# bdsaglam/torch-scae

Measured on AMD Instinct MI355X. Metric: images/sec SCAE fwd+bwd, MNIST 40x40 bs=128, 1/2/4/8 MI355X, higher is better.
Workload: dtype f32

## Files before the change

include/scae_hip.h:

```cpp
#ifndef SCAE_HIP_H
#define SCAE_HIP_H

#include <stdint.h>

#ifdef __cplusplus
extern "C" {
#endif

#define SCAE_ABI_VERSION 3

#define SCAE_OK 0
#define SCAE_ERR_BAD_ARG (-1)
#define SCAE_ERR_UNSUPPORTED (-2)

#define SCAE_MAX_CHANNELS 4
#define SCAE_ATTN_MAX_SET 64
#define SCAE_RENDER_MAX_TEMPLATE_ELEMS 4096

int scae_abi_version(void);
const char *scae_error_string(int code);

void *scae_launch_list_begin(void *stream);
int scae_launch_list_end(void *list);
int scae_launch_list_size(const void *list);
// ... 623 lines not shown
  float *loss;
  const float *g_loss;
  int defer_combine;
  float *out12;
  const scae_train_log_desc *train_log;
} scae_loss_extras;
int scae_loss_tail_supported(int B, int O, int ncls);
int64_t scae_loss_tail_workspace_floats(int B, int O, int ncls);
int scae_loss_tail_fwd_f32(const float *lpp, const float *posterior,
                           const float *caps_presence, const float *cls_w,
                           const float *cls_b, const int64_t *label,
                           const scae_loss_extras *extras, float *out12, float *workspace,
                           int B, int O, int M, int ncls, int n_classes_cfg, int prior_type,
                           int post_type, int sparsity_on, const float *weights5,
                           float within_const, void *stream);
int scae_loss_tail_defer_preferred(int B, int O);
int scae_loss_tail_combine_f32(const float *lpp, const float *posterior,
                               const float *caps_presence, const float *cls_w,
                               const float *cls_b, const int64_t *label,
                               const scae_loss_extras *extras, float *out12, float *workspace,
                               int B, int O, int M, int ncls, int n_classes_cfg, int prior_type,
                               int post_type, int sparsity_on, const float *weights5,
                               float within_const, void *stream);
int scae_loss_tail_fwd_class_probs_f32(
    const float *lpp, const float *posterior, const float *caps_presence, const float *cls_w,
    const float *cls_b, const int64_t *label, const scae_loss_extras *extras, float *out12,
    float *workspace, int B, int O, int M, int ncls, int n_classes_cfg, int prior_type,
    int post_type, int sparsity_on, const float *weights5, float within_const,
    const float *cp_caps_presence, const float *cp_posterior, const float *cp_w,
    const float *cp_bias, float *prior_prob, float *post_prob, int cp_B, int cp_O, int cp_M,
    int cp_ncls, const scae_scaled_sum *extra_sums, int n_extra, void *stream);
int scae_loss_tail_fwd_class_probs_sink_f32(
    const float *lpp, const float *posterior, const float *caps_presence, const float *cls_w,
    const float *cls_b, const int64_t *label, const scae_loss_extras *extras, float *out12,
    float *workspace, int B, int O, int M, int ncls, int n_classes_cfg, int prior_type,
    int post_type, int sparsity_on, const float *weights5, float within_const,
    const float *cp_caps_presence, const float *cp_posterior, const float *cp_w,
    const float *cp_bias, float *prior_prob, float *post_prob, int cp_B, int cp_O, int cp_M,
    int cp_ncls, const scae_scaled_sum *extra_sums, int n_extra, scae_eval_sink *sink,
    void *stream);
int scae_loss_tail_bwd_f32(const float *lpp, const float *posterior,
                           const float *caps_presence, const float *cls_w,
                           const float *cls_b, const int64_t *label,
                           const scae_loss_extras *extras, const float *gout12,
                           const float *workspace, float *g_lpp, float *g_posterior,
                           float *g_caps_presence, float *g_cls_w,
                           float *g_cls_b, int B, int O, int M, int ncls, int n_classes_cfg,
                           int prior_type, int post_type, int sparsity_on,
                           const float *weights5, float within_const, void *stream);

#define SCAE_EVAL_ACC_DOUBLES 17
int scae_eval_tail_f32(const float *lpp, const float *posterior, const float *caps_presence,
                       const float *cls_w, const float *cls_b, const int64_t *label,
                       const scae_loss_extras *extras, float *out12, float *workspace, int B,
                       int O, int M, int ncls, int n_classes_cfg, int prior_type,
                       int post_type, int sparsity_on, const float *weights5,
                       float within_const, const float *prior_prob, const float *post_prob,
                       double *acc, float *batch3, void *stream);
int scae_eval_tail_sink_f32(const float *lpp, const float *posterior, const float *caps_presence,
                            const float *cls_w, const float *cls_b, const int64_t *label,
                            const scae_loss_extras *extras, float *out12, float *workspace,
                            int B, int O, int M, int ncls, int n_classes_cfg, int prior_type,
                            int post_type, int sparsity_on, const float *weights5,
                            float within_const, const float *prior_prob, const float *post_prob,
                            double *acc, float *batch3, scae_eval_sink *sink, void *stream);
int scae_eval_tail_records_f32(const float *lpp, const float *posterior,
                               const float *caps_presence, const float *cls_w,
                               const float *cls_b, const int64_t *label,
                               const scae_loss_extras *extras, float *out12, float *workspace,
                               int B, int O, int M, int ncls, int n_classes_cfg, int prior_type,
                               int post_type, int sparsity_on, const float *weights5,
                               float within_const, const float *prior_prob,
                               const float *post_prob, double *acc, float *batch3,
                               scae_eval_sink *sink, scae_eval_records *records, void *stream);
int scae_eval_records_f32(const float *prior_prob, const float *post_prob, const int64_t *label,
                          const float *lpp, const float *rec_sums, const float *rec_pixels,
                          int B, int ncls, int M, int n_rec, scae_eval_records *records,
                          void *stream);
int scae_eval_accumulate_f32(const float *loss, const float *out12, const float *prior_prob,
                             const float *post_prob, const int64_t *label, int B, int ncls,
                             double *acc, float *batch3, void *stream);
int scae_eval_features_f32(const float *caps_presence, const float *posterior, int B, int O,
                           int M, scae_eval_sink *sink, void *stream);
int scae_train_log_f32(const float *loss, const float *out12, const float *extra2,
                       const scae_train_log_desc *log, int B, void *stream);

typedef struct scae_decoder_desc {
  const float *templates;
  const float *templates_alpha;
  const float *pose;
  const float *presence;
  const float *bg_image;
  const float *bg_value;
  const float *bg_mixing_logit;
  const float *temperature_logit;
  const float *out_scale;
  int B, M, C, th, tw, H, W;
  int template_repeat;
} scae_decoder_desc;

int scae_template_render_fwd_f32(const scae_decoder_desc *d,
                                 float *transformed_templates,
                                 float *mixing_logits, void *stream);

int scae_render_gmm_logprob_fwd_f32(const scae_decoder_desc *d, const float *x,
                                    float *log_prob, float *lse_post,
                                    float *lse_prior, void *stream);

int scae_render_gmm_bwd_f32(const scae_decoder_desc *d, const float *x,
                            const float *lse_post, const float *lse_prior,
                            const float *g_logprob, const float *g_tt,
                            const float *g_ml, float *g_templates,
                            float *g_alpha_partial, float *g_pose,
                            float *g_presence, float *g_bg_image,
                            float *g_scalar_partial, void *stream);
int scae_render_gmm_logprob_tiles(const scae_decoder_desc *d);
int scae_render_gmm_logprob_sums_fwd_f32(const scae_decoder_desc *d, const float *x,
                                         float *tile_sums, float *lse_post, float *lse_prior,
                                         void *stream);
int scae_render_gmm_sums_bwd_f32(const scae_decoder_desc *d, const float *x,
                                 const float *lse_post, const float *lse_prior,
                                 const float *g_tile_sums, float *g_templates,
                                 float *g_alpha_partial, float *g_pose, float *g_presence,
                                 float *g_bg_image, float *g_scalar_partial, void *stream);
#define SCAE_K1_FWD_WAVE 0
#define SCAE_K1_FWD_CLASSIC 1
#define SCAE_K1_RENDER_WAVE 0
#define SCAE_K1_RENDER_CLASSIC 1
#define SCAE_K1_BWD_CELL 0
#define SCAE_K1_BWD_SCATTER 1
#define SCAE_K1_BWD_GATHER 2
int scae_render_gmm_forms(const scae_decoder_desc *d, int fused, const void *tt,
                          const void *ml, int out[12]);


int scae_set_encoder_fwd_logprob_f32(int nseg, const float *const *seg_ptr,
                                     const int *seg_width, const int *seg_row_stride,
                                     const int64_t *seg_batch_stride, const float *presence,
                                     const float *params, float *z, float *hsave, int B, int N,
                                     int D, int Din, int Dout, int L, int layer_norm,
                                     const scae_decoder_desc *d, const float *x,
                                     float *tile_sums, float *lse_post, float *lse_prior,
                                     void *stream);

int scae_set_encoder_fwd_logprob_bf16(int nseg, const float *const *seg_ptr,
                                      const int *seg_width, const int *seg_row_stride,
                                      const int64_t *seg_batch_stride, const float *presence,
                                      const float *params, float *z, float *hsave, int B, int N,
                                      int D, int Din, int Dout, int L, int layer_norm,
                                      const scae_decoder_desc *d, const float *x,
                                      float *tile_sums, float *lse_post, float *lse_prior,
                                      void *stream);

typedef struct scae_likelihood_bwd_desc {
  const float *vote, *scale, *vote_presence, *dummy_vote, *x, *presence, *posterior;
  const int64_t *winner_idx;
  const float *g_lpp, *g_winner, *g_winner_presence, *g_soft_winner, *g_soft_winner_presence,
      *g_posterior, *g_mixing_log_prob, *g_mixing_logit;
  float *gvote, *gscale, *gvote_presence, *gx, *gpresence, *gdummy_partial;
  int B, O, M;
} scae_likelihood_bwd_desc;
int scae_render_gmm_sums_bwd_likelihood_f32(
    const scae_decoder_desc *d, const float *x, const float *lse_post, const float *lse_prior,
    const float *g_tile_sums, float *g_templates, float *g_alpha_partial, float *g_pose,
    float *g_presence, float *g_bg_image, float *g_scalar_partial,
    const scae_likelihood_bwd_desc *k, void *stream);

int scae_gmm_log_prob_fwd_f32(const float *loc, const float *mixing_logits,
                              const float *sigma, const float *x,
                              float *log_prob, int B, int K, int C, int Cm,
                              int64_t P, void *stream);
int scae_gmm_log_prob_bwd_f32(const float *loc, const float *mixing_logits,
                              const float *sigma, const float *x,
                              const float *g_logprob, float *g_loc,
                              float *g_ml, float *g_sigma_partial, float *g_x,
                              int B, int K, int C, int Cm, int64_t P,
                              void *stream);
int scae_gmm_mean_f32(const float *loc, const float *mixing_logits, float *out,
                      int B, int K, int C, int Cm, int64_t P, void *stream);
int scae_gmm_mode_f32(const float *loc, const float *mixing_logits,
                      const float *sigma, float *out, int maximum, int B,
                      int K, int C, int Cm, int64_t P, void *stream);

int scae_render_gmm_mode_f32(const scae_decoder_desc *d, float *out, int what, int first,
                             int count, void *stream);

int scae_render_gmm_parts_f32(const scae_decoder_desc *d, const float *x, const int *part_group,
                              const float *palette, int P, int *part, float *conf, float *mass,
                              float *mass_partial, int *group, float *rgb_part,
                              float *rgb_group, int first, int count, void *stream);
int scae_render_gmm_parts_geometry(const scae_decoder_desc *d, int count, int *out);

int scae_image_sheet_f32(int nsrc, const float *const *src, const int *n, int C, int H, int W,
                         int nrow, int padding, float pad_value, float *sheet, void *stream);

#define SCAE_KMEANS_MAX_K 256
#define SCAE_KMEANS_MAX_F 256
#define SCAE_KMEANS_MAX_KF 16384
#define SCAE_KMEANS_STATE_INTS 4
int scae_kmeans_supported(int k, int F);
int scae_kmeans_groups(int64_t N, int R);
typedef struct scae_kmeans_desc {
  const float *x;
  int64_t N;
  int F, k, R;
  int G;
  int max_iter;
  float *centroids;
  int64_t *labels;
  float *part_sum;
  int *part_count;
  int *part_changed;
  double *part_inertia;
  int *state;
  double *inertia;
} scae_kmeans_desc;
int scae_kmeans_lloyd_f32(const scae_kmeans_desc *d, int n_iters, void *stream);
int scae_kmeans_pp_f32(const float *x, int64_t N, int F, int k, int R, uint32_t seed,
                       float *centroids, float *d2, int64_t *chosen, void *stream);
int scae_kmeans_assign_f32(const float *x, int64_t N, int F, int k, const float *centroids,
                           int64_t *labels, void *stream);
int scae_kmeans_contingency(const int64_t *cluster_ids, const int64_t *labels, int64_t N, int k,
                            int ncls, int *table, int *outside, void *stream);

#define SCAE_PROBE_MAX_F 256
#define SCAE_PROBE_MAX_C 256
#define SCAE_PROBE_MAX_CF 16384
#define SCAE_PROBE_MAX_R 16
#define SCAE_PROBE_STATE_INTS 4
int scae_probe_supported(int F, int C, int R);
int scae_probe_groups(int64_t N, int F);
int scae_probe_predict_blocks(int64_t N);
int scae_probe_moments_f64(const float *x, const int64_t *y, int64_t N, int F, int C,
                           double *part, double *moments, int *outside, void *stream);
typedef struct scae_probe_desc {
  const float *x;
  const int64_t *y;
  int64_t N;
  int F, C, R;
  int G;
  int max_iter;
  const float *mean;
  const float *scale;
  const double *l2;
  const double *step;
  const double *tol;
  float *W, *V;
  float *grad;
  double *t;
  float *part_grad;
  double *part_loss;
  double *history;
  int *state;
} scae_probe_desc;
int scae_probe_fit_f32(const scae_probe_desc *d, int n_iters, void *stream);
int scae_probe_predict_f32(const float *x, int64_t N, int F, int C, const float *weight,
                           const float *bias, const int64_t *y, int64_t *pred, float *log_prob,
                           double *part_ce, double *mean_ce, void *stream);

#define SCAE_TSNE_MAX_N 32768
#define SCAE_TSNE_MAX_F 256
#define SCAE_TSNE_HISTORY_COLS 3
#define SCAE_TSNE_BLOCK_DOUBLES 640
int scae_tsne_supported(int N, int F);
int scae_tsne_groups(int N);
int scae_tsne_affinities_f32(const float *x, int N, int F, float perplexity, float *P,
                             float *beta, double *part, double *plogp, void *stream);
typedef struct scae_tsne_desc {
  int N;
  int G;
  int n_iter;
  int exaggeration_iter;
  int check_every;
  float early_exaggeration;
  float learning_rate;
  const float *P;
  float *Y, *velocity, *gains;
  float *part;
  float *rows;
  double *block;
  const double *plogp;
  double *history;
} scae_tsne_desc;
int scae_tsne_run_f32(const scae_tsne_desc *d, int first_iter, int n, void *stream);

#define SCAE_KNN_MAX_K 64
#define SCAE_KNN_MAX_F 256
#define SCAE_KNN_MAX_KS 8
int scae_knn_supported(int64_t Nq, int64_t Nb, int F, int k);
int scae_knn_groups(int64_t Nq, int64_t Nb);
int scae_knn_f32(const float *q, int64_t Nq, const float *base, int64_t Nb, int F, int k,
                 int self_mode, uint64_t *part, float *d2, int64_t *idx, void *stream);
int scae_knn_vote_f32(const int64_t *idx, const float *d2, int64_t Nq, int k,
                      const int64_t *base_labels, int64_t Nb, const int *ks, int n_ks,
                      int weighted, int64_t *pred, void *stream);
int scae_knn_ranks_f32(const float *x, int64_t N, int F, const int64_t *idx, int k, int *rank,
                       int *part_count, int64_t *part, int64_t *penalty, void *stream);

#define SCAE_TSNE_MAX_NEIGHBORS 128
#define SCAE_TSNE_SPARSE_MAX_N 262144
#define SCAE_TSNE_SPARSE_BLOCK_DOUBLES 5120
int scae_knn_wide_f32(const float *x, int64_t N, int F, int k, uint64_t *part, float *d2,
                      int64_t *idx, void *stream);
int scae_tsne_sparse_supported(int N, int F, int K);
int scae_tsne_sparse_groups(int N);
int scae_tsne_knn_bandwidths_f32(const float *d2, int N, int K, float perplexity, float *cond,
                                 float *beta, void *stream);
typedef struct scae_tsne_sparse_desc {
  int N;
  int G;
  int n_iter;
  int exaggeration_iter;
  int check_every;
// ... 31 lines not shown
```

torch_scae_amd/_lib.py:

```python
import ctypes
import os
from ctypes import (POINTER, Structure, c_char_p, c_double, c_float, c_int,
                    c_int64, c_uint32, c_uint64, c_void_p)

_HERE = os.path.dirname(os.path.abspath(__file__))
LIB_PATH = os.environ.get("SCAE_HIP_LIB") or os.path.join(_HERE, "lib",
                                                        "libscae_hip.so")

P = c_void_p


class DecoderDesc(Structure):
    _fields_ = [("templates", P), ("templates_alpha", P), ("pose", P),
                ("presence", P), ("bg_image", P), ("bg_value", P),
                ("bg_mixing_logit", P), ("temperature_logit", P),
                ("out_scale", P),
                ("B", c_int), ("M", c_int), ("C", c_int), ("th", c_int),
                ("tw", c_int), ("H", c_int), ("W", c_int),
                ("template_repeat", c_int)]


class LikelihoodBwdDesc(Structure):
    _fields_ = [(n, P) for n in (
        "vote", "scale", "vote_presence", "dummy_vote", "x", "presence",
        "posterior", "winner_idx", "g_lpp", "g_winner", "g_winner_presence",
        "g_soft_winner", "g_soft_winner_presence", "g_posterior",
        "g_mixing_log_prob", "g_mixing_logit", "gvote", "gscale",
        "gvote_presence", "gx", "gpresence", "gdummy_partial")] + [
        ("B", c_int), ("O", c_int), ("M", c_int)]


class GemmDesc(Structure):
    _fields_ = [("A", P), ("B", P), ("C", P), ("bias", P), ("mask", P),
                ("asum", P), ("batch", c_int), ("M", c_int), ("N", c_int),
                ("K", c_int), ("a_kcontig", c_int), ("lda", c_int),
                ("a_batch", c_int64), ("b_kcontig", c_int), ("ldb", c_int),
                ("b_batch", c_int64), ("ldc", c_int), ("c_batch", c_int64),
                ("bias_ld", c_int), ("bias_batch", c_int64), ("ldmask", c_int),
                ("mask_batch", c_int64), ("asum_batch", c_int64),
                ("relu", c_int), ("asum_ld", c_int), ("c_nomask", P)]


class MlpChainLayer(Structure):
    _fields_ = [("w", P), ("w_gs", c_int64), ("ldw", c_int), ("K", c_int),
                ("N", c_int), ("bias", P), ("bias_gs", c_int64),
                ("bias_ld", c_int), ("gate", P), ("gate_gs", c_int64),
                ("gate_bs", c_int64), ("out", P), ("out_gs", c_int64),
                ("out_bs", c_int64), ("relu", c_int)]


class MlpChainDesc(Structure):
    _fields_ = [("layer", MlpChainLayer * 4), ("n_layers", c_int), ("in_", P),
                ("in_gs", c_int64), ("in_bs", c_int64), ("in_dim", c_int),
                ("B", c_int), ("G", c_int), ("row_tile", c_int),
                ("bf16", c_int)]


class VotesDesc(Structure):
    _fields_ = [(n, P) for n in ("all_param", "cpr_static", "bias_cvr",
                                 "bias_caps", "bias_vote", "bias_scale",
                                 "noise_caps", "noise_vote")] + \
        [("noise_scale", c_float), ("V", c_int), ("ld_param", c_int),
         ("similarity", c_int), ("learn_vote_scale", c_int),
         ("allow_deformations", c_int)] + \
        [(n, P) for n in ("vote", "scale", "vote_presence", "logit_caps",
                          "logit_vote", "reg_partial", "caps_presence",
                          "caps_arg", "gvote", "gscale", "gvote_presence",
                          "glogit_caps", "glogit_vote", "greg", "gcaps_presence",
                          "gall_param", "gcpr_in", "gall_param_gated")]


class SumSegment(Structure):
    _fields_ = [("dst", P), ("begin", c_int64), ("end", c_int64),
                ("period", c_int64)]


class SumJob(Structure):
    _fields_ = [("src", P), ("rows", c_int64), ("cols", c_int64),
                ("segments", POINTER(SumSegment)), ("n_segments", c_int)]


class ScaledSum(Structure):
    _fields_ = [("src", P), ("n", c_int64), ("scale", c_float), ("dst", P)]


class TrainLogDesc(Structure):
    _fields_ = [("rows", P), ("step", P), ("capacity", c_int), ("acc", P),
                ("prior_prob", P), ("post_prob", P), ("label", P), ("ncls", c_int),
                ("lr", P)]


class LossExtras(Structure):
    _fields_ = [("rec_sums", P), ("n_rec", c_int), ("reg", P),
                ("w_reg", c_float), ("g_rec_sums", P), ("g_reg", P),
                ("loss", P), ("g_loss", P), ("defer_combine", c_int),
                ("out12", P), ("train_log", POINTER(TrainLogDesc))]


class KMeansDesc(Structure):
    _fields_ = [("x", P), ("N", c_int64), ("F", c_int), ("k", c_int), ("R", c_int),
                ("G", c_int), ("max_iter", c_int), ("centroids", P), ("labels", P),
                ("part_sum", P), ("part_count", P), ("part_changed", P),
                ("part_inertia", P), ("state", P), ("inertia", P)]


class ProbeDesc(Structure):
    _fields_ = [("x", P), ("y", P), ("N", c_int64), ("F", c_int), ("C", c_int), ("R", c_int),
                ("G", c_int), ("max_iter", c_int), ("mean", P), ("scale", P), ("l2", P),
                ("step", P), ("tol", P), ("W", P), ("V", P), ("grad", P), ("t", P),
                ("part_grad", P), ("part_loss", P), ("history", P), ("state", P)]


class TsneDesc(Structure):
    _fields_ = [("N", c_int), ("G", c_int), ("n_iter", c_int), ("exaggeration_iter", c_int),
                ("check_every", c_int), ("early_exaggeration", c_float),
                ("learning_rate", c_float), ("P", P), ("Y", P), ("velocity", P), ("gains", P),
                ("part", P), ("rows", P), ("block", P), ("plogp", P), ("history", P)]


class TsneSparseDesc(Structure):
    _fields_ = [("N", c_int), ("G", c_int), ("n_iter", c_int), ("exaggeration_iter", c_int),
                ("check_every", c_int), ("early_exaggeration", c_float),
                ("learning_rate", c_float), ("indptr", P), ("cols", P), ("vals", P),
                ("nnz", c_int64), ("Y", P), ("velocity", P), ("gains", P), ("part", P),
                ("rows", P), ("block", P), ("plogp", P), ("history", P)]


class SeedFoldDesc(Structure):
    _fields_ = [(n, P) for n in (
        "seeds", "wq", "bq", "wk", "bk", "wv", "bv", "wo", "bo", "w2", "b2",
        "q", "wkf", "bkf", "wvf", "bvf", "wv2e", "wowv")] + \
        [("O", c_int), ("C", c_int), ("D", c_int)]


class FirstLayerDesc(Structure):
    _fields_ = [("img", P), ("w", P), ("bias", P), ("out", P)] + \
        [(n, c_int) for n in ("B", "Cin", "IH", "IW", "Cout", "stride",
                              "n_layers")] + \
        [("rw", P * 8), ("rwf", P * 8), ("rwd", P * 8),
         ("rCout", c_int * 8), ("rCin", c_int * 8),
         ("out_h", P), ("rwfh", P * 8), ("rwdh", P * 8)]


class BatchSourceDesc(Structure):
    _fields_ = [("images", P), ("labels", P), ("index", P), ("rows", c_int64),
                ("n", c_int64)] + \
        [(n, c_int) for n in ("image_u8", "label_u8", "C", "h", "w", "H", "W",
                              "shuffle", "translate")] + \
        [("seed", c_uint64), ("epoch", c_int64), ("position", c_int64),
         ("rank", c_int), ("world", c_int), ("wrap", c_int),
         ("affine", P), ("affine_rows", c_int64)]


class SeedFoldGrads(Structure):
    _fields_ = [(n, P) for n in (
        "g_q", "g_wkf", "g_bkf", "g_wvf", "g_bvf", "d_seeds", "d_wq", "d_bq",
        "d_wk", "d_bk", "d_wv", "d_bv", "d_wo", "d_bo", "d_w2", "d_b2",
        "gv2e", "t1")]


SIGNATURES = {
    "scae_abi_version": [],
    "scae_error_string": [c_int],
    "scae_uniform_f32": [P, c_int64, P, P],
    "scae_geometric_transform_fwd_f32": [P, P, c_int64, c_int, c_int, c_int, P],
    "scae_geometric_transform_bwd_f32": [P, P, P, c_int64, c_int, c_int, c_int,
                                         P],
    "scae_mat3_mul_fwd_f32": [P, P, P, c_int64, c_int, P],
    "scae_mat3_mul_bwd_f32": [P, P, P, P, P, c_int64, c_int, P],
    "scae_qkv_attention_fwd_f32": [P, P, P, P, P, P, c_int, c_int, c_int,
                                   c_int, c_int, c_float, P],
    "scae_qkv_attention_fwd_bf16": [P, P, P, P, P, P, c_int, c_int, c_int,
                                    c_int, c_int, c_float, P],
    "scae_qkv_attention_bwd_f32": [P, P, P, P, P, P, P, P, P, c_int, c_int,
                                   c_int, c_int, c_int, c_float, P],
    "scae_set_encoder_param_count": [c_int] * 5,
    "scae_set_encoder_grid": [c_int],
    "scae_set_encoder_supported": [c_int] * 6,
    "scae_set_encoder_fwd_f32": [c_int, P, P, P, P, P, P, P, P] + [c_int] * 7 + [P],
    "scae_set_encoder_bwd_f32": [c_int, P, P, P, P, P, P, P, P, P, P]
                                + [c_int] * 7 + [P],
    "scae_render_gmm_sums_bwd_likelihood_f32": [P] * 13,
    "scae_set_encoder_fwd_logprob_f32": [c_int, P, P, P, P, P, P, P, P] + [c_int] * 7
                                        + [P] * 6,
    "scae_set_encoder_fwd_logprob_bf16": [c_int, P, P, P, P, P, P, P, P] + [c_int] * 7
                                         + [P] * 6,
    "scae_set_encoder_bf16_supported": [c_int] * 6,
    "scae_set_encoder_fwd_bf16": [c_int, P, P, P, P, P, P, P, P] + [c_int] * 7 + [P],
    "scae_set_encoder_bwd_bf16": [c_int, P, P, P, P, P, P, P, P, P, P]
                                 + [c_int] * 7 + [P],
    "scae_seed_attention_splits": [c_int] * 2,
    "scae_seed_attention_grid": [c_int] * 2,
    "scae_seed_attention_supported": [c_int] * 4,
    "scae_seed_attention_fwd_f32": [P] * 9 + [c_int] * 5 + [P],
    "scae_seed_attention_bwd_f32": [P] * 10 + [c_int] * 5 + [P],
    "scae_seed_attention_mfma_supported": [c_int] * 4,
    "scae_seed_attention_mfma_rows": [c_int],
    "scae_seed_attention_mfma_fwd_f32": [P] * 7 + [c_int] * 4 + [P],
    "scae_seed_attention_mfma_bwd_f32": [P] * 8 + [c_int] * 4 + [P],
    "scae_seed_attention_mfma_fwd_bf16": [P] * 7 + [c_int] * 4 + [P],
    "scae_seed_attention_mfma_bwd_bf16": [P] * 8 + [c_int] * 4 + [P],
    "scae_seed_attention_mfma_bwd_gemm_f32": [P] * 8 + [c_int] * 4
    + [POINTER(GemmDesc), c_int, P],
    "scae_seed_attention_mfma_bwd_gemm_bf16": [P] * 8 + [c_int] * 4
    + [POINTER(GemmDesc), c_int, P],
    "scae_object_encoder_bwd_supported": [c_int] * 9,
    "scae_object_encoder_bwd_gemm_f32": [P] * 8 + [c_int] * 4
    + [POINTER(GemmDesc), c_int] + [c_int, P, P, P, P, P, P, P, P, P] + [c_int] * 7 + [P],
    "scae_object_encoder_bwd_gemm_bf16": [P] * 8 + [c_int] * 4
    + [POINTER(GemmDesc), c_int] + [c_int, P, P, P, P, P, P, P, P, P] + [c_int] * 7 + [P],
    "scae_seed_attention_mfma_reduce_f32": [P, c_int] + [P] * 7 + [c_int] * 2 + [P],
    "scae_seed_fold_supported": [c_int] * 3,
    "scae_seed_fold_fwd_f32": [POINTER(SeedFoldDesc), P],
    "scae_seed_fold_bwd_f32": [POINTER(SeedFoldDesc), POINTER(SeedFoldGrads), P],
    "scae_layer_norm_rows": [c_int64],
    "scae_layer_norm_fwd_f32": [P] * 6 + [c_int64, c_int, c_float, P],
    "scae_layer_norm_bwd_f32": [P] * 7 + [c_int64, c_int, P],
    "scae_gemm_f32": [P] * 6 + [c_int] * 6 + [c_int64, c_int, c_int, c_int64,
                                              c_int, c_int64, c_int, c_int64,
                                              c_int, c_int64, c_int64, c_int, c_int,
                                              P],
    "scae_gemm_bf16": [P] * 6 + [c_int] * 6 + [c_int64, c_int, c_int, c_int64,
                                              c_int, c_int64, c_int, c_int64,
                                              c_int, c_int64, c_int64, c_int, c_int,
                                              P],
    "scae_gemm_pair_f32": [POINTER(GemmDesc), POINTER(GemmDesc), P],
    "scae_launch_list_begin": [P],
    "scae_launch_list_end": [P],
    "scae_launch_list_size": [P],
    "scae_launch_list_run": [P, P],
    "scae_launch_list_lane": [P, c_int],
    "scae_launch_list_timeline": [P, P, P, POINTER(c_float), c_int],
    "scae_launch_list_free": [P],
    "scae_gemm_multi_f32": [POINTER(GemmDesc), c_int, P],
    "scae_gemm_multi_bf16": [POINTER(GemmDesc), c_int, P],
    "scae_mlp_chain_max_width": [],
    "scae_mlp_chain_fwd_f32": [POINTER(MlpChainDesc), P],
    "scae_mlp_chain_bwd_f32": [POINTER(MlpChainDesc), P],
    "scae_mlp_chain_votes_fwd_f32": [POINTER(MlpChainDesc), POINTER(VotesDesc), P],
    "scae_mlp_chain_votes_bwd_f32": [POINTER(MlpChainDesc), POINTER(VotesDesc), P],
    "scae_gemm_pair_bf16": [POINTER(GemmDesc), POINTER(GemmDesc), P],
    "scae_conv3x3_wf_floats": [c_int, c_int],
    "scae_conv3x3_relayout_f32": [P, P, P, c_int, c_int, P],
    "scae_conv3x3_bf16r_supported": [c_int] * 6,
    "scae_conv3x3_first_fwd_relayout_bf16": [P] * 4 + [c_int] * 7 + [P] * 8,
    "scae_cvt_bf16_batch": [c_int, P, P, P, P],
    "scae_conv3x3_fwd_bf16r": [P] * 7 + [c_int] * 6 + [P],
    "scae_conv3x3_dgrad_bf16r": [P] * 5 + [c_int] * 6 + [P],
    "scae_conv3x3_wgrad_bf16r_splits": [c_int] * 5,
# ... 291 lines not shown
```

torch_scae_amd/csrc/loss_tail.hip:

```cpp
#include "class_probs_dev.h"
#include "common.h"
#include "loss_tail_dev.h"

namespace {
using namespace scae_tail;
constexpr int MAXCLS = 32;

__device__ __forceinline__ float ent_term_grad(float p, float k) {
  const float q = p * k;
  return q < scae::kLogSafeEps ? 1e8f : -(logf(q) + 1.f);
}

__device__ __forceinline__ float within_term(const float *x, float r, int O, int type,
                                             float cw, int lane) {
  if (type == 0) return (r - cw) * (r - cw);
  const float k = type == 2 ? (float)O : 1.f;
  float w = 0.f;
  for (int o = lane; o < O; o += NTI) w += ent_term(x[o] / (r + 1e-8f), k);
  return scae::wave_sum(w);
}

__device__ __forceinline__ float cls_xe(const TailArgs &a, const float *x, int label, int lane,
                                        float &gl) {
  const bool on = lane < a.ncls;
  float z = -INFINITY;
  if (on) {
    const float *wr = a.cls_w + (size_t)lane * a.O;
    float z0 = a.cls_b[lane], z1 = 0.f, z2 = 0.f, z3 = 0.f;
    int o = 0;
    for (; o + 4 <= a.O; o += 4) {
      const float w0 = wr[o], w1 = wr[o + 1], w2 = wr[o + 2], w3 = wr[o + 3];
      z0 = fmaf(x[o], w0, z0), z1 = fmaf(x[o + 1], w1, z1);
      z2 = fmaf(x[o + 2], w2, z2), z3 = fmaf(x[o + 3], w3, z3);
    }
    for (; o < a.O; ++o) z0 = fmaf(x[o], wr[o], z0);
    z = (z0 + z1) + (z2 + z3);
  }
  const float mx = scae::wave_max(z);
  float p = on ? expf(z - mx) : 0.f;
  p /= scae::wave_sum(p);
  const float mx2 = scae::wave_max(on ? p : -INFINITY);
  const float q = on ? expf(p - mx2) : 0.f;
  const float sum2 = scae::wave_sum(q);
  const float plabel = scae::wave_sum(lane == label ? p : 0.f);
  const float dq = on ? q / sum2 - (lane == label ? 1.f : 0.f) : 0.f;
  const float dot = scae::wave_sum(p * dq);
  gl = p * (dq - dot);
  return mx2 + logf(sum2) - plabel;
}

__global__ __launch_bounds__(NTI) void tail_image_kernel(TailArgs a, Ws ws, scae_cp::Args cpa,
                                                        int n_cp) {
  extern __shared__ __attribute__((aligned(16))) float smem[];
  const int B = a.B, O = a.O, M = a.M, b = blockIdx.x, lane = threadIdx.x;
  if (b >= B) {
    __shared__ scae_cp::Lds s_cpl;
    scae_cp::body(cpa, s_cpl, b - B, lane);
    return;
  }
  float *s_cp = smem, *s_mass = smem + O, *s_raw = smem + 2 * O;
  float rc = 0.f, rm = 0.f;
  for (int o = lane; o < O; o += NTI) {
    const float xc = a.cp[(size_t)b * O + o];
    const float *pr = a.posterior + ((size_t)b * (O + 1) + o) * M;
    float t = 0.f;
    if ((M & 3) == 0) {
      const float4 *p4 = reinterpret_cast<const float4 *>(pr);
      for (int m = 0; m < M / 4; ++m) {
        const float4 v = p4[m];
        t += (v.x + v.y) + (v.z + v.w);
      }
    } else {
      for (int m = 0; m < M; ++m) t += pr[m];
    }
    s_cp[o] = xc;
    s_raw[o] = t;
    s_mass[o] = t / M;
    ws.mass[(size_t)b * O + o] = t;
    rc += xc;
    rm += t / M;
  }
  rc = scae::wave_sum(rc);
  rm = scae::wave_sum(rm);
  float lp = 0.f;
  for (int m = lane; m < M; m += NTI) lp += a.lpp[(size_t)b * M + m];
  lp = scae::wave_sum(lp);
  __syncthreads();
  float wc = 0.f, wm = 0.f;
  if (a.sparsity_on) {
    wc = within_term(s_cp, rc, O, a.prior_type, a.l2_within_const, lane);
    wm = within_term(s_mass, rm, O, a.post_type, a.l2_within_const_post, lane);
  }
  float xe_c = 0.f, xe_m = 0.f;
  if (a.label) {
    const int label = (int)a.label[b];
    float g0, g1;
    xe_c = cls_xe(a, s_cp, label, lane, g0);
    xe_m = cls_xe(a, s_raw, label, lane, g1);
    if (lane < a.ncls) {
      ws.gl[((size_t)b * 2 + 0) * a.ncls + lane] = g0;
      ws.gl[((size_t)b * 2 + 1) * a.ncls + lane] = g1;
    }
  }
  if (lane == 0) {
    float *p = ws.part + (size_t)b * 8;
    p[0] = lp, p[1] = wc, p[2] = wm, p[3] = xe_c, p[4] = xe_m, p[5] = rc, p[6] = rm, p[7] = 0.f;
  }
}

template <int NTC>
__global__ __launch_bounds__(NTC) void tail_combine_kernel(TailArgs a, scae_loss_extras x, Ws ws,
                                                          float *out) {
  extern __shared__ __attribute__((aligned(16))) float smem[];
  combine_body<NTC>(a, x, ws, out, smem);
}

template <int NTC>
__global__ __launch_bounds__(NTC) void tail_combine_log_kernel(TailArgs a, scae_loss_extras x,
                                                              Ws ws, float *out,
                                                              TrainLogArgs g) {
  extern __shared__ __attribute__((aligned(16))) float smem[];
  combine_body<NTC>(a, x, ws, out, smem);
  __syncthreads();
  train_log_epilogue<NTC>(g, out, out, nullptr);
}

__device__ __forceinline__ void sparsity_grad(const float *x, const float *col, float r, int B,
                                              int O, int type, float cw, float cb, float gw,
                                              float gb, float *g, int lane) {
  if (type == 0) {
    for (int o = lane; o < O; o += 64)
      g[o] = gw * 2.f * (r - cw) / B + gb * 2.f * (col[o] - cb) / O;
    return;
  }
  const float k = type == 2 ? (float)O : 1.f;
  float tot = 0.f;
  for (int o = 0; o < O; ++o) tot += col[o];
  const float tinv = 1.f / (tot + 1e-8f), rinv = 1.f / (r + 1e-8f);
  float dot_b = 0.f, dot_w = 0.f;
  for (int o = lane; o < O; o += 64) {
    dot_b += ent_term_grad(col[o] * tinv, k) * col[o] * tinv;
    dot_w += ent_term_grad(x[o] * rinv, k) * x[o] * rinv;
  }
  dot_b = scae::wave_sum(dot_b);
  dot_w = scae::wave_sum(dot_w);
  for (int o = lane; o < O; o += 64) {
    const float dw = (ent_term_grad(x[o] * rinv, k) - dot_w) * rinv / B;
    const float db = -(ent_term_grad(col[o] * tinv, k) - dot_b) * tinv;
    g[o] = gw * dw + gb * db;
  }
}

template <int NT>
__device__ __forceinline__ void tail_bwd_body(const TailArgs &a, const scae_loss_extras &x,
                                              const Ws &ws, const float *gout ,
                                              float *g_lpp, float *g_post, float *g_cp,
                                              float *g_w, float *g_b, float *smem) {
  const int B = a.B, O = a.O, M = a.M, tid = threadIdx.x;
  float go[12];
#pragma unroll
  for (int i = 0; i < 12; ++i) go[i] = gout ? gout[i] : 0.f;
  if (x.g_loss) go[0] += x.g_loss[0];
  const float g0 = go[0];
  if ((int)blockIdx.x >= B) {
    if (!(a.label && g_w)) return;
    const float g_x1 = (g0 + go[6]) / B, g_x2 = (g0 + go[7]) / B;
    const int nout = a.ncls * O + a.ncls;
    const int out = ((int)blockIdx.x - B) * (NT / 4) + (tid >> 2), part = tid & 3;
    float t = 0.f;
    if (out < a.ncls * O) {
      const int cc = out / O, o = out - cc * O;
      float t0 = 0.f, t1 = 0.f, t2 = 0.f, t3 = 0.f;
      int b = part;
      for (; b + 12 < B; b += 16) {
#define SCAE_TERM(bb)                                                                  \
  (ws.gl[((size_t)(bb) * 2) * a.ncls + cc] * g_x1 * a.cp[(size_t)(bb) * O + o] +      \
   ws.gl[((size_t)(bb) * 2 + 1) * a.ncls + cc] * g_x2 * ws.mass[(size_t)(bb) * O + o])
        const float u0 = SCAE_TERM(b), u1 = SCAE_TERM(b + 4), u2 = SCAE_TERM(b + 8),
                    u3 = SCAE_TERM(b + 12);
        t0 += u0, t1 += u1, t2 += u2, t3 += u3;
      }
      for (; b < B; b += 4) t0 += SCAE_TERM(b);
#undef SCAE_TERM
      t = (t0 + t1) + (t2 + t3);
    } else if (out < nout) {
      const int cc = out - a.ncls * O;
#pragma unroll 4
      for (int b = part; b < B; b += 4)
        t += ws.gl[((size_t)b * 2) * a.ncls + cc] * g_x1 +
             ws.gl[((size_t)b * 2 + 1) * a.ncls + cc] * g_x2;
    }
    t += scae::xor1_f(t);
    t += scae::xor2_f(t);
    if (part == 0 && out < nout) {
      if (out < a.ncls * O)
        g_w[out] = t;
      else
        g_b[out - a.ncls * O] = t;
    }
    return;
  }
  const int b = blockIdx.x;
  const float g_lp = (-a.w_ll * g0 + go[1] - go[10]) / B;
  for (int m = tid; m < M; m += NT) g_lpp[(size_t)b * M + m] = g_lp;
  if (x.g_rec_sums) {
    const float gr = (-g0 + go[8] - go[9]) / B;
    const int per = (x.n_rec + B - 1) / B, i1 = min(x.n_rec, (b + 1) * per);
    for (int i = b * per + tid; i < i1; i += NT) x.g_rec_sums[i] = gr;
  }
  if (x.g_reg && b == 0 && tid == 0) x.g_reg[0] = x.w_reg * g0 + go[11];
  float *s_cp = smem, *s_mass = s_cp + O, *col = s_mass + O, *gc = col + 2 * O, *gm = gc + O;
  for (int o = tid; o < O; o += NT) {
    s_cp[o] = a.cp[(size_t)b * O + o];
    s_mass[o] = ws.mass[(size_t)b * O + o] / M;
    if (!x.defer_combine) {
      col[o] = ws.col[o];
      col[O + o] = ws.col[O + o];
    }
    gc[o] = gm[o] = 0.f;
  }
  if (x.defer_combine) column_sums<NT>(a, ws, col, tid, false);
  __syncthreads();
  if (a.sparsity_on && tid < 64) {
    const float *p = ws.part + (size_t)b * 8;
    sparsity_grad(s_cp, col, p[5], B, O, a.prior_type, a.l2_within_const, a.l2_between_const,
                  a.w_pw * g0 + go[2], a.w_pb * g0 + go[3], gc, tid);
    sparsity_grad(s_mass, col + O, p[6], B, O, a.post_type, a.l2_within_const_post,
                  a.l2_between_const_post, a.w_qw * g0 + go[4], a.w_qb * g0 + go[5], gm, tid);
  }
  __syncthreads();
  for (int o = tid; o < O; o += NT) g_cp[(size_t)b * O + o] = gc[o];
  float *gp = g_post + (size_t)b * (O + 1) * M;
  if ((M & 3) == 0) {
    const int M4 = M / 4;
    for (int e = tid; e < (O + 1) * M4; e += NT) {
      const int o = e / M4;
      const float v = o < O ? gm[o] / M : 0.f;
      reinterpret_cast<float4 *>(gp)[e] = make_float4(v, v, v, v);
    }
  } else {
    for (int e = tid; e < (O + 1) * M; e += NT) {
      const int o = e / M;
      gp[e] = o < O ? gm[o] / M : 0.f;
    }
  }
}

template <int NT>
__global__ __launch_bounds__(NT) void tail_bwd_kernel(TailArgs a, scae_loss_extras x, Ws ws,
                                                      const float *gout , float *g_lpp,
                                                      float *g_post, float *g_cp, float *g_w,
                                                      float *g_b) {
  extern __shared__ __attribute__((aligned(16))) float smem[];
  if (x.defer_combine && blockIdx.x + 1 == gridDim.x) {
    combine_body<NT>(a, x, ws, x.out12, smem);
    return;
  }
  tail_bwd_body<NT>(a, x, ws, gout, g_lpp, g_post, g_cp, g_w, g_b, smem);
}

template <int NT>
__global__ __launch_bounds__(NT) void tail_bwd_log_kernel(TailArgs a, scae_loss_extras x, Ws ws,
                                                          const float *gout ,
                                                          float *g_lpp, float *g_post,
                                                          float *g_cp, float *g_w, float *g_b,
                                                          TrainLogArgs g) {
  extern __shared__ __attribute__((aligned(16))) float smem[];
  if (blockIdx.x + 1 == gridDim.x) {
    combine_body<NT>(a, x, ws, x.out12, smem);
    __syncthreads();
    train_log_epilogue<NT>(g, x.out12, x.out12, nullptr);
    return;
  }
  tail_bwd_body<NT>(a, x, ws, gout, g_lpp, g_post, g_cp, g_w, g_b, smem);
}
}

extern "C" int scae_loss_tail_supported(int B, int O, int ncls) {
  return (B > 0 && O > 0 && O <= 4096 && ncls <= MAXCLS) ? 1 : 0;
}

extern "C" int64_t scae_loss_tail_workspace_floats(int B, int O, int ncls) {
  if (B <= 0 || O <= 0 || ncls < 0) return 0;
  return (int64_t)ws_floats(B, O, ncls);
}

int scae_tail::fill_train_log(TrainLogArgs &g, const scae_train_log_desc &d, int B) {
  if (!d.rows || !d.step || d.capacity <= 0 || B <= 0 || d.ncls < 0) return SCAE_ERR_BAD_ARG;
  if (d.label && (d.ncls <= 0 || !d.prior_prob || !d.post_prob)) return SCAE_ERR_BAD_ARG;
  g = TrainLogArgs{d.rows, d.step, d.acc, d.prior_prob, d.post_prob, d.label, d.lr,
                   d.capacity, B, d.ncls};
  return SCAE_OK;
}

static int launch_combine(const TailArgs &a, const scae_loss_extras &x, const Ws &ws,
                          float *out12, hipStream_t st) {
  const bool small = scae_loss_tail_defer_preferred(a.B, a.O);
  if (x.train_log) {
    TrainLogArgs g;
    const int rc = fill_train_log(g, *x.train_log, a.B);
    if (rc) return rc;
    if (small)
      scae::launch(tail_combine_log_kernel<NT_SMALL>, dim3(1), dim3(NT_SMALL), combine_lds(a.O),
                   st, a, x, ws, out12, g);
    else
      scae::launch(tail_combine_log_kernel<NTC_LARGE>, dim3(1), dim3(NTC_LARGE),
                   combine_lds(a.O), st, a, x, ws, out12, g);
    return SCAE_OK;
  }
  if (small)
    scae::launch(tail_combine_kernel<NT_SMALL>, dim3(1), dim3(NT_SMALL), combine_lds(a.O), st,
                       a, x, ws, out12);
  else
    scae::launch(tail_combine_kernel<NTC_LARGE>, dim3(1), dim3(NTC_LARGE), combine_lds(a.O),
                       st, a, x, ws, out12);
  return SCAE_OK;
}

int scae_tail::fill_tail(TailArgs &a, const float *lpp, const float *posterior, const float *cp,
                          const float *cls_w, const float *cls_b, const int64_t *label, int B,
                          int O, int M, int ncls, int n_classes_cfg, int prior_type,
                          int post_type, int sparsity_on, const float *weights ,
                          float within_const) {
  if (!lpp || !posterior || !cp || !weights || B <= 0 || O <= 0 || M <= 0)
    return SCAE_ERR_BAD_ARG;
  if (label && (!cls_w || !cls_b || ncls <= 0)) return SCAE_ERR_BAD_ARG;
  if (prior_type < 0 || prior_type > 2 || post_type < 0 || post_type > 2) return SCAE_ERR_BAD_ARG;
  if (!scae_loss_tail_supported(B, O, ncls)) return SCAE_ERR_UNSUPPORTED;
  a = TailArgs{lpp, posterior, cp, cls_w, cls_b, label, B, O, M, ncls, prior_type, post_type,
               sparsity_on, weights[0], weights[1], weights[2], weights[3], weights[4],
               0.f, 0.f, 0.f, 0.f};
  const float nc = n_classes_cfg > 0 ? (float)n_classes_cfg : 1.f;
  a.l2_within_const = within_const == within_const ? within_const : (float)O / nc;
  a.l2_between_const = (float)B / nc;
  a.l2_within_const_post = (float)O / nc;
  a.l2_between_const_post = (float)B / nc;
  return SCAE_OK;
}

static int tail_fwd(const float *lpp, const float *posterior, const float *caps_presence,
                    const float *cls_w, const float *cls_b, const int64_t *label,
                    const scae_loss_extras *extras, float *out12, float *workspace, int B, int O,
                    int M, int ncls, int n_classes_cfg, int prior_type, int post_type,
                    int sparsity_on, const float *weights5, float within_const,
                    const scae_cp::Args *cpa, void *stream) {
  TailArgs a;
  int rc = fill_tail(a, lpp, posterior, caps_presence, cls_w, cls_b, label, B, O, M, ncls,
                     n_classes_cfg, prior_type, post_type, sparsity_on, weights5, within_const);
  if (rc) return rc;
  SCAE_REQUIRE(out12 && workspace);
  scae_loss_extras x{};
  if (extras) x = *extras;
  if (x.rec_sums && x.n_rec <= 0) return SCAE_ERR_BAD_ARG;
  const Ws ws = carve_ws(workspace, B, O, ncls);
  hipStream_t st = (hipStream_t)stream;
  const int n_cp = cpa ? cpa->B + cpa->extra.n : 0;
  scae::launch(tail_image_kernel, dim3(B + n_cp), dim3(NTI), 3 * O * sizeof(float), st, a,
                     ws, cpa ? *cpa : scae_cp::Args{}, n_cp);
  if (!x.defer_combine) {
    rc = launch_combine(a, x, ws, out12, st);
    if (rc) return rc;
  }
  return scae_launch_status();
}

extern "C" int scae_loss_tail_defer_preferred(int B, int O) {
  return B > 0 && O > 0 && (long)B * B * 2 * O * (long)sizeof(float) <= (8l << 20);
}

extern "C" int scae_loss_tail_combine_f32(const float *lpp, const float *posterior,
                                          const float *caps_presence, const float *cls_w,
                                          const float *cls_b, const int64_t *label,
                                          const scae_loss_extras *extras, float *out12,
                                          float *workspace, int B, int O, int M, int ncls,
                                          int n_classes_cfg, int prior_type, int post_type,
                                          int sparsity_on, const float *weights5,
                                          float within_const, void *stream) {
  TailArgs a;
  int rc = fill_tail(a, lpp, posterior, caps_presence, cls_w, cls_b, label, B, O, M, ncls,
                     n_classes_cfg, prior_type, post_type, sparsity_on, weights5, within_const);
  if (rc) return rc;
  SCAE_REQUIRE(out12 && workspace);
  scae_loss_extras x{};
  if (extras) x = *extras;
  if (x.rec_sums && x.n_rec <= 0) return SCAE_ERR_BAD_ARG;
  rc = launch_combine(a, x, carve_ws(workspace, B, O, ncls), out12, (hipStream_t)stream);
  if (rc) return rc;
  return scae_launch_status();
}

extern "C" int scae_loss_tail_fwd_f32(const float *lpp, const float *posterior,
                                      const float *caps_presence, const float *cls_w,
                                      const float *cls_b, const int64_t *label,
                                      const scae_loss_extras *extras, float *out12,
                                      float *workspace, int B, int O, int M, int ncls,
                                      int n_classes_cfg, int prior_type, int post_type,
                                      int sparsity_on, const float *weights5,
                                      float within_const, void *stream) {
  return tail_fwd(lpp, posterior, caps_presence, cls_w, cls_b, label, extras, out12, workspace,
                  B, O, M, ncls, n_classes_cfg, prior_type, post_type, sparsity_on, weights5,
                  within_const, nullptr, stream);
}

extern "C" int scae_loss_tail_fwd_class_probs_sink_f32(
    const float *lpp, const float *posterior, const float *caps_presence, const float *cls_w,
    const float *cls_b, const int64_t *label, const scae_loss_extras *extras, float *out12,
    float *workspace, int B, int O, int M, int ncls, int n_classes_cfg, int prior_type,
    int post_type, int sparsity_on, const float *weights5, float within_const,
    const float *cp_caps_presence, const float *cp_posterior, const float *cp_w,
    const float *cp_bias, float *prior_prob, float *post_prob, int cp_B, int cp_O, int cp_M,
    int cp_ncls, const scae_scaled_sum *extra_sums, int n_extra, scae_eval_sink *sink,
    void *stream) {
  scae_cp::Args cpa;
  int rc = scae_cp::fill(cpa, cp_caps_presence, cp_posterior, cp_w, cp_bias, prior_prob,
                         post_prob, cp_B, cp_O, cp_M, cp_ncls, extra_sums, n_extra);
  if (rc) return rc;
  cpa.sink = sink;
  return tail_fwd(lpp, posterior, caps_presence, cls_w, cls_b, label, extras, out12, workspace,
                  B, O, M, ncls, n_classes_cfg, prior_type, post_type, sparsity_on, weights5,
                  within_const, &cpa, stream);
}

extern "C" int scae_loss_tail_fwd_class_probs_f32(
    const float *lpp, const float *posterior, const float *caps_presence, const float *cls_w,
    const float *cls_b, const int64_t *label, const scae_loss_extras *extras, float *out12,
    float *workspace, int B, int O, int M, int ncls, int n_classes_cfg, int prior_type,
    int post_type, int sparsity_on, const float *weights5, float within_const,
    const float *cp_caps_presence, const float *cp_posterior, const float *cp_w,
    const float *cp_bias, float *prior_prob, float *post_prob, int cp_B, int cp_O, int cp_M,
    int cp_ncls, const scae_scaled_sum *extra_sums, int n_extra, void *stream) {
  return scae_loss_tail_fwd_class_probs_sink_f32(
      lpp, posterior, caps_presence, cls_w, cls_b, label, extras, out12, workspace, B, O, M,
      ncls, n_classes_cfg, prior_type, post_type, sparsity_on, weights5, within_const,
      cp_caps_presence, cp_posterior, cp_w, cp_bias, prior_prob, post_prob, cp_B, cp_O, cp_M,
      cp_ncls, extra_sums, n_extra, nullptr, stream);
}

extern "C" int scae_loss_tail_bwd_f32(const float *lpp, const float *posterior,
                                      const float *caps_presence, const float *cls_w,
                                      const float *cls_b, const int64_t *label,
                                      const scae_loss_extras *extras, const float *gout12,
                                      const float *workspace, float *g_lpp, float *g_posterior,
                                      float *g_caps_presence, float *g_cls_w, float *g_cls_b,
                                      int B, int O, int M, int ncls, int n_classes_cfg,
                                      int prior_type, int post_type, int sparsity_on,
                                      const float *weights5, float within_const, void *stream) {
  TailArgs a;
  int rc = fill_tail(a, lpp, posterior, caps_presence, cls_w, cls_b, label, B, O, M, ncls,
                     n_classes_cfg, prior_type, post_type, sparsity_on, weights5, within_const);
  if (rc) return rc;
  SCAE_REQUIRE(g_lpp && g_posterior && g_caps_presence && workspace);
  if (!gout12 && !(extras && extras->g_loss)) return SCAE_ERR_BAD_ARG;
  scae_loss_extras x{};
  if (extras) x = *extras;
  if (x.rec_sums && (x.n_rec <= 0 || !x.g_rec_sums)) return SCAE_ERR_BAD_ARG;
  if (x.reg && !x.g_reg) return SCAE_ERR_BAD_ARG;
  if (label) SCAE_REQUIRE(g_cls_w && g_cls_b);
  const Ws ws = carve_ws(const_cast<float *>(workspace), B, O, ncls);
  if (x.defer_combine) SCAE_REQUIRE(x.out12);
  const size_t lds = 6 * O * sizeof(float) > combine_lds(O) ? 6 * O * sizeof(float) : combine_lds(O);
  if (x.defer_combine && x.train_log) {
    TrainLogArgs g;
    rc = fill_train_log(g, *x.train_log, B);
    if (rc) return rc;
    const int cls_blocks = label ? (ncls * O + ncls + NT_SMALL / 4 - 1) / (NT_SMALL / 4) : 0;
    scae::launch(tail_bwd_log_kernel<NT_SMALL>, dim3(B + cls_blocks + 1), dim3(NT_SMALL), lds,
                 (hipStream_t)stream, a, x, ws, gout12, g_lpp, g_posterior, g_caps_presence,
                 g_cls_w, g_cls_b, g);
    return scae_launch_status();
  }
#define SCAE_TAIL_BWD(NTH)                                                                       \
  do {                                                                                           \
    const int cls_blocks = label ? (ncls * O + ncls + NTH / 4 - 1) / (NTH / 4) : 0;              \
    scae::launch(tail_bwd_kernel<NTH>, dim3(B + cls_blocks + (x.defer_combine ? 1 : 0)),   \
                       dim3(NTH), lds, (hipStream_t)stream, a, x, ws, gout12, g_lpp, g_posterior, \
                       g_caps_presence, g_cls_w, g_cls_b);                                       \
  } while (0)
  if (x.defer_combine || scae_loss_tail_defer_preferred(B, O))
    SCAE_TAIL_BWD(NT_SMALL);
  else
    SCAE_TAIL_BWD(NTB_LARGE);
#undef SCAE_TAIL_BWD
  return scae_launch_status();
}
```

torch_scae_amd/csrc/loss_tail_dev.h:

```cpp
#pragma once
#include "common.h"

namespace scae_tail {
constexpr int NTI = 64;
constexpr int NT_SMALL = 512, NTC_LARGE = 1024, NTB_LARGE = 256;

struct TailArgs {
  const float *lpp;
  const float *posterior;
  const float *cp;
  const float *cls_w;
  const float *cls_b;
  const int64_t *label;
  int B, O, M, ncls;
  int prior_type, post_type;
  int sparsity_on;
  float w_ll, w_pw, w_pb, w_qw, w_qb;
  float l2_within_const, l2_between_const, l2_within_const_post, l2_between_const_post;
};

struct Ws {
  float *part, *mass, *gl, *col;
};
__host__ __device__ inline Ws carve_ws(float *w, int B, int O, int ncls) {
  Ws s;
  s.part = w;
  s.mass = s.part + (size_t)B * 8;
  s.gl = s.mass + (size_t)B * O;
  s.col = s.gl + (size_t)B * 2 * (ncls > 0 ? ncls : 1);
  return s;
}
inline size_t ws_floats(int B, int O, int ncls) {
  return (size_t)B * 8 + (size_t)B * O + (size_t)B * 2 * (ncls > 0 ? ncls : 1) + 2 * (size_t)O;
}

__device__ __forceinline__ float ent_term(float p, float k) {
  return -p * scae::log_safe(p * k);
}
__device__ __forceinline__ float between_term(const float *col, int O, int type, float cb,
                                              int lane) {
  float t = 0.f;
  if (type == 0) {
    for (int o = lane; o < O; o += 64) t += (col[o] - cb) * (col[o] - cb);
    return scae::wave_sum(t) / O;
  }
  const float k = type == 2 ? (float)O : 1.f;
  float tot = 0.f;
  for (int o = 0; o < O; ++o) tot += col[o];
  for (int o = lane; o < O; o += 64) t += ent_term(col[o] / (tot + 1e-8f), k);
  return -scae::wave_sum(t);
}

template <int NTC>
__device__ __forceinline__ void column_sums(const TailArgs &a, const Ws &ws, float *col, int tid,
                                            bool publish) {
  const int B = a.B, O = a.O;
  for (int e = tid; e < ((2 * O * 16 + NTC - 1) / NTC) * NTC; e += NTC) {
    const int c = e >> 4, l = e & 15, which = c / O, o = c - which * O;
    float t = 0.f;
    if (c < 2 * O) {
      auto at = [&](int b) {
        return which == 0 ? a.cp[(size_t)b * O + o] : ws.mass[(size_t)b * O + o] / a.M;
      };
      float t0 = 0.f, t1 = 0.f, t2 = 0.f, t3 = 0.f;
      int b = l;
      for (; b + 48 < B; b += 64) {
        const float u0 = at(b), u1 = at(b + 16), u2 = at(b + 32), u3 = at(b + 48);
        t0 += u0, t1 += u1, t2 += u2, t3 += u3;
      }
      for (; b < B; b += 16) t0 += at(b);
      t = (t0 + t1) + (t2 + t3);
    }
    t = scae::row_sum16(t);
    if (c < 2 * O && l == 0) {
      col[c] = t;
      if (publish) ws.col[c] = t;
    }
  }
}

template <int NTC>
__device__ __forceinline__ void combine_body(const TailArgs &a, const scae_loss_extras &x,
                                             const Ws &ws, float *out, float *smem) {
  const int B = a.B, O = a.O, tid = threadIdx.x;
  float *col = smem, *red = smem + 2 * O;
  float v[6] = {0.f, 0.f, 0.f, 0.f, 0.f, 0.f};
  for (int b = tid; b < B; b += NTC) {
    const float4 p = *reinterpret_cast<const float4 *>(ws.part + (size_t)b * 8);
    v[0] += p.x, v[1] += p.y, v[2] += p.z, v[3] += p.w;
    v[4] += ws.part[(size_t)b * 8 + 4];
  }
  if (x.rec_sums)
    for (int i = tid; i < x.n_rec; i += NTC) v[5] += x.rec_sums[i];
  column_sums<NTC>(a, ws, col, tid, true);
  scae::block_sum<6, NTC>(v, red);
  if (tid >= 64) return;
  float pb = 0.f, qb = 0.f;
  if (a.sparsity_on) {
    pb = between_term(col, O, a.prior_type, a.l2_between_const, tid);
    qb = between_term(col + O, O, a.post_type, a.l2_between_const_post, tid);
  }
  if (tid != 0) return;
  const float log_prob = v[0] / B, pw = v[1] / B, qw = v[2] / B, xe1 = v[3] / B, xe2 = v[4] / B;
  const float rec = x.rec_sums ? v[5] / B : 0.f, reg = x.reg ? x.reg[0] : 0.f;
  out[1] = log_prob, out[2] = pw, out[3] = pb, out[4] = qw, out[5] = qb;
  out[6] = xe1, out[7] = xe2, out[8] = rec, out[9] = -rec, out[10] = -log_prob, out[11] = reg;
  const float loss = -a.w_ll * log_prob + a.w_pw * pw + a.w_pb * pb + a.w_qw * qw +
                     a.w_qb * qb + xe1 + xe2 - rec + x.w_reg * reg;
  out[0] = loss;
  if (x.loss) x.loss[0] = loss;
}


__device__ __forceinline__ int row_argmax(const float *p, int n) {
  float v = 0.f;
  int best = 0;
  for (int c0 = 0; c0 < n; c0 += 16) {
    float x[16];
#pragma unroll
    for (int j = 0; j < 16; ++j) x[j] = c0 + j < n ? p[c0 + j] : 0.f;
#pragma unroll
    for (int j = 0; j < 16; ++j) {
      const int c = c0 + j;
      if (c >= n) break;
      if (x[j] != x[j]) return c;
      if (c == 0 || x[j] > v) v = x[j], best = c;
    }
  }
  return best;
}

template <int NT>
__device__ __forceinline__ void accuracy_counts(const float *prior_prob, const float *post_prob,
                                                const int64_t *label, int B, int ncls,
                                                float &n_prior, float &n_post) {
  __shared__ float red[2][NT / 64];
  float cp = 0.f, cq = 0.f;
  if (label && ncls > 0) {
    for (int b = threadIdx.x; b < B; b += NT) {
      const int64_t l = label[b];
      cp += row_argmax(prior_prob + (size_t)b * ncls, ncls) == l ? 1.f : 0.f;
      cq += row_argmax(post_prob + (size_t)b * ncls, ncls) == l ? 1.f : 0.f;
    }
  }
  cp = scae::wave_sum(cp);
  cq = scae::wave_sum(cq);
  const int w = threadIdx.x / 64;
  if ((threadIdx.x & 63) == 0) red[0][w] = cp, red[1][w] = cq;
  __syncthreads();
  n_prior = n_post = 0.f;
  if (threadIdx.x == 0)
    for (int i = 0; i < NT / 64; ++i) n_prior += red[0][i], n_post += red[1][i];
}

__device__ __forceinline__ void batch_accuracies(bool labelled, int B, float n_prior,
                                                 float n_post, float acc3[3]) {
  float pa = 0.f, qa = 0.f;
  if (labelled) pa = n_prior / (float)B, qa = n_post / (float)B;
  acc3[0] = qa > pa ? qa : pa, acc3[1] = pa, acc3[2] = qa;
}

__device__ __forceinline__ void accumulate_batch(double *A, float loss, const float *out12,
                                                 const float acc3[3]) {
  A[0] += 1.0;
  A[1] += (double)loss;
  A[2] += (double)acc3[0];
  A[3] += (double)acc3[1];
  A[4] += (double)acc3[2];
  if (out12)
    for (int i = 0; i < 12; ++i) A[5 + i] += (double)out12[i];
}

struct TrainLogArgs {
  float *rows;
  int64_t *step;
  double *acc;
  const float *prior_prob, *post_prob;
  const int64_t *label;
  const float *lr;
  int capacity, B, ncls;
};

template <int NT>
__device__ __forceinline__ void train_log_epilogue(const TrainLogArgs &g, const float *loss,
                                                   const float *out12, const float *extra) {
  float n_prior, n_post;
  accuracy_counts<NT>(g.prior_prob, g.post_prob, g.label, g.B, g.ncls, n_prior, n_post);
  if (threadIdx.x >= 64) return;
  const int lane = threadIdx.x;
  n_prior = __shfl(n_prior, 0), n_post = __shfl(n_post, 0);
  float acc3[3];
  batch_accuracies(g.label && g.ncls > 0, g.B, n_prior, n_post, acc3);
  const int64_t s = g.step[0];
  const float l = loss[0];
  const float o = out12 && lane >= 4 && lane < 16 ? out12[lane - 4] : 0.f;
  const float lr = g.lr ? g.lr[0] : __builtin_nanf("");
  const float e = extra && lane >= 17 && lane < 19 ? extra[lane - 17] : 0.f;
  const double a = g.acc && lane < SCAE_EVAL_ACC_DOUBLES ? g.acc[lane] : 0.0;
  const float v = lane == 0 ? l : lane == 1 ? acc3[0] : lane == 2 ? acc3[1]
                : lane == 3 ? acc3[2] : lane < 16 ? o : lane == 16 ? lr : e;
  float *r = g.rows + (size_t)((uint64_t)s % (uint64_t)g.capacity) * SCAE_TRAIN_LOG_ROW;
  if (lane < SCAE_TRAIN_LOG_ROW) r[lane] = v;
  const float u = __shfl(v, lane > 0 ? lane - 1 : 0);
  if (g.acc && lane < SCAE_EVAL_ACC_DOUBLES && (lane < 5 || out12))
    g.acc[lane] = a + (lane == 0 ? 1.0 : (double)u);
  if (lane == 0) g.step[0] = s + 1;
}

inline size_t combine_lds(int O) { return (2 * O + 6 * (NTC_LARGE / 64)) * sizeof(float); }

int fill_tail(TailArgs &a, const float *lpp, const float *posterior, const float *cp,
              const float *cls_w, const float *cls_b, const int64_t *label, int B, int O, int M,
              int ncls, int n_classes_cfg, int prior_type, int post_type, int sparsity_on,
              const float *weights , float within_const);
int fill_train_log(TrainLogArgs &g, const scae_train_log_desc &d, int B);
}
```

torch_scae_amd/csrc/render_bwd_likelihood.hip:

```cpp
#include "common.h"
#include "capsule_likelihood_dev.h"
#include "render_gmm_wave_dev.h"

namespace {
struct LkBwd {
  scae_lk::LkArgs a;
  const int64_t *winner_idx;
  const float *g_lpp, *g_winner, *g_winner_presence, *g_soft_winner, *g_soft_winner_presence,
      *g_posterior, *g_mlp, *g_mlogit;
  float *gvote, *gscale, *gvp, *gx, *gpresence, *gdummy;
};

template <int C>
__global__ __launch_bounds__(256, 5) void bwd_cell_likelihood_kernel(
    scae_decoder_desc d, const float *__restrict__ x, const float *__restrict__ lse_post,
    const float *__restrict__ lse_prior, const float *__restrict__ g_tile, int lp_tiles,
    int lp_ppb, float *__restrict__ g_templates, float *__restrict__ g_alpha_partial,
    float *__restrict__ g_pose, float *__restrict__ g_presence, float *__restrict__ g_bg_image,
    float *__restrict__ g_scalar_partial, int chunk_rows, int max_items, int item_budget,
    LkBwd lk, int n_lk) {
  extern __shared__ __attribute__((aligned(16))) float smem[];
  if ((int)blockIdx.x < n_lk) {
    scae_lk::likelihood_bwd_body<false, 256>(
        lk.a, lk.winner_idx, lk.g_lpp, lk.g_winner, lk.g_winner_presence, lk.g_soft_winner,
        lk.g_soft_winner_presence, lk.g_posterior, lk.g_mlp, lk.g_mlogit, lk.gvote, lk.gscale,
        lk.gvp, lk.gx, lk.gpresence, lk.gdummy, smem, blockIdx.x, n_lk);
    return;
  }
  const int id = (int)blockIdx.x - n_lk, K = d.M + 1, b = id / K, k = id - b * K;
  scae_k1::bwd_cell_body<C, 256>(d, x, lse_post, lse_prior, nullptr, g_tile, lp_tiles, lp_ppb,
                                 g_templates, g_alpha_partial, g_pose, g_presence, g_bg_image,
                                 g_scalar_partial, chunk_rows, max_items, item_budget, smem, k, b);
}

template <int C>
int launch(const scae_decoder_desc *d, const scae_k1::CellGeom &g, const scae_k1::LpTiling &lt,
           const float *x, const float *lse_post, const float *lse_prior, const float *g_tile,
           float *g_templates, float *g_alpha_partial, float *g_pose, float *g_presence,
           float *g_bg_image, float *g_scalar_partial, const LkBwd &lk, hipStream_t st) {
  const size_t lds_k = scae_lk::lk_lds(lk.a.O, lk.a.M, true);
  const size_t lds = g.lds > lds_k ? g.lds : lds_k;
  if (lds > 48 * 1024) {
    hipError_t e =
        hipFuncSetAttribute(reinterpret_cast<const void *>(bwd_cell_likelihood_kernel<C>),
                            hipFuncAttributeMaxDynamicSharedMemorySize, (int)lds);
    if (e != hipSuccess) return (int)e;
  }
  const int n_lk = lk.a.B < 1024 ? lk.a.B : 1024;
  scae::launch((bwd_cell_likelihood_kernel<C>), dim3(n_lk + (d->M + 1) * d->B), dim3(256),
                     lds, st, *d, x, lse_post, lse_prior, g_tile, lt.tiles, lt.ppb, g_templates,
                     g_alpha_partial, g_pose, g_presence, g_bg_image, g_scalar_partial,
                     g.chunk_rows, g.max_items, g.item_budget, lk, n_lk);
  return scae_launch_status();
}
}

extern "C" int scae_render_gmm_sums_bwd_likelihood_f32(
    const scae_decoder_desc *d, const float *x, const float *lse_post, const float *lse_prior,
    const float *g_tile_sums, float *g_templates, float *g_alpha_partial, float *g_pose,
    float *g_presence, float *g_bg_image, float *g_scalar_partial,
    const scae_likelihood_bwd_desc *k, void *stream) {
  SCAE_REQUIRE(d && k);
  const char *e = getenv("SCAE_FUSE_K1_K4_BWD");
  const scae_k1::CellGeom g = scae_k1::cell_geom(d);
  const bool fits = !(e && *e == '0') && g.lds && (d->C == 1 || d->C == 3) && k->O <= 64 &&
                    scae_lk::lk_lds(k->O, k->M, true) <= g.lds && k->B > 0 && k->O > 0 &&
                    k->M > 0 && d->template_repeat <= 1;
  if (!fits) {
    int rc = scae_render_gmm_sums_bwd_f32(d, x, lse_post, lse_prior, g_tile_sums, g_templates,
                                          g_alpha_partial, g_pose, g_presence, g_bg_image,
                                          g_scalar_partial, stream);
    if (rc) return rc;
    return scae_capsule_likelihood_bwd_f32(
        k->vote, k->scale, k->vote_presence, k->dummy_vote, k->x, k->presence, k->posterior,
        k->winner_idx, k->g_lpp, k->g_winner, k->g_winner_presence, k->g_soft_winner,
        k->g_soft_winner_presence, k->g_posterior, k->g_mixing_log_prob, k->g_mixing_logit,
        k->gvote, k->gscale, k->gvote_presence, k->gx, k->gpresence, k->gdummy_partial, k->B,
        k->O, k->M, stream);
  }
  SCAE_REQUIRE(x && lse_post && lse_prior && g_tile_sums && g_templates && g_alpha_partial &&
               g_pose && g_scalar_partial);
  SCAE_REQUIRE(k->vote && k->scale && k->vote_presence && k->dummy_vote && k->x &&
               k->posterior && k->winner_idx && k->gvote && k->gscale && k->gvote_presence &&
               k->gx && k->gdummy_partial);
  const scae_k1::LpTiling lt = scae_k1::lp_tiling(d);
  LkBwd lk{{k->vote, k->scale, k->vote_presence, k->dummy_vote, k->x, k->presence, k->B, k->O,
            k->M},
           k->winner_idx,
           k->g_lpp,
           k->g_winner,
           k->g_winner_presence,
           k->g_soft_winner,
           k->g_soft_winner_presence,
           k->g_posterior,
           k->g_mixing_log_prob,
           k->g_mixing_logit,
           k->gvote,
           k->gscale,
           k->gvote_presence,
           k->gx,
           k->gpresence,
           k->gdummy_partial};
  hipStream_t st = (hipStream_t)stream;
  return d->C == 1 ? launch<1>(d, g, lt, x, lse_post, lse_prior, g_tile_sums, g_templates,
                               g_alpha_partial, g_pose, g_presence, g_bg_image, g_scalar_partial,
                               lk, st)
                   : launch<3>(d, g, lt, x, lse_post, lse_prior, g_tile_sums, g_templates,
                               g_alpha_partial, g_pose, g_presence, g_bg_image, g_scalar_partial,
                               lk, st);
}
```

torch_scae_amd/csrc/render_gmm_wave_dev.h:

```cpp
#pragma once
#include "common.h"
#include "render_gmm_dev.h"

namespace scae_k1 {
namespace {
constexpr float kLog2e = 1.44269504088896340736f, kLn2 = 0.69314718055994530942f;
constexpr int KC = 8;
constexpr float kMasked = -3.0e38f;

constexpr int kLogprobPadLow = 1;
template <int C> struct TexelOf { static constexpr int TX = C == 1 ? 2 : (C <= 3 ? 4 : 8); };

__device__ __forceinline__ float ex2(float v) { return __builtin_amdgcn_exp2f(v); }
__device__ __forceinline__ float lg2(float v) { return __builtin_amdgcn_logf(v); }

__host__ __device__ inline int plane_w(int tw, int PL) { return tw + PL + 2; }
__host__ __device__ inline int plane_elems(int th, int tw, int PL) {
  return (th + PL + 2) * (tw + PL + 2);
}
template <int C, int PL = 2>
__device__ __forceinline__ void stage_planes(float *s_pl, const scae_decoder_desc &d, int b, int k0,
                                             int nk, float alpha_scale, int tid, int nthr) {
  constexpr int TX = TexelOf<C>::TX;
  const int M = d.M, th = d.th, tw = d.tw, tsz = th * tw;
// ... 51 lines not shown
        const float *a = d.pose + ((size_t)b * M + k) * 6;
        const float hx = 0.5f * (float)tw, hy = 0.5f * (float)th;
        co[0] = hx * a[0], co[1] = hx * a[1], co[2] = hx * (a[2] + 1.f) - 0.5f;
        co[3] = hy * a[3], co[4] = hy * a[4], co[5] = hy * (a[5] + 1.f) - 0.5f;
        co[6] = d.presence ? kLog2e * log_safe(d.presence[b * M + k]) : 0.f;
      }
#pragma unroll
      for (int i = 0; i < 8; ++i) s_coef[k * 8 + i] = co[i];
    }
  }
  __syncthreads();

  const int p = tile * ppb + tid;
  const bool live = p < HW && tid < ppb;
  const int pc = live ? p : HW - 1;
  const float inv_w = 1.f / (float)W;
  const int pi = (int)(((float)pc + 0.5f) * inv_w), pj = pc - pi * W;
  const float xn = (float)(2 * pj + 1) * inv_w - 1.f;
  const float yn = (float)(2 * pi + 1) * (1.f / (float)d.H) - 1.f;
  const float txf = (float)tw, tyf = (float)th, pwf = (float)pw;
  const float c2 = kLog2e * 0.5f * sc.inv_var;

  float xv[C], mpost[C], spost[C];
  const float u_bg = kLog2e * sc.bg_ml;
  float mprior = u_bg, sprior = 1.f;
#pragma unroll
  for (int c = 0; c < C; ++c) {
    xv[c] = x[((size_t)b * C + c) * HW + pc];
    const float bgv = d.bg_image ? d.bg_image[((size_t)b * C + c) * HW + pc] : sc.bg_val;
    const float df = xv[c] - bgv;
    mpost[c] = fmaf(df * df, -c2, u_bg);
    spost[c] = 1.f;
  }

  const float *s_tap = s_pl + (size_t)(PL * pw + PL) * TX;
  for (int k0 = 0; k0 < M; k0 += KC) {
    float uv[KC], pv[KC][C];
#pragma unroll
    for (int q = 0; q < KC; ++q) {
      const int k = k0 + q, kp = k < M ? k : M - 1;
      const float4 ca = *reinterpret_cast<const float4 *>(s_coef + k * 8);
      const float4 cb = *reinterpret_cast<const float4 *>(s_coef + k * 8 + 4);
      float ix = fmaf(ca.x, xn, fmaf(ca.y, yn, ca.z));
      float iy = fmaf(ca.w, xn, fmaf(cb.x, yn, cb.y));
      ix = fminf(fmaxf(ix, -(float)PL), txf);
      iy = fminf(fmaxf(iy, -(float)PL), tyf);
      const float x0f = floorf(ix), y0f = floorf(iy);
      const float fx = ix - x0f, fy = iy - y0f;
      const int idx = (int)fmaf(y0f, pwf, x0f);
      const float *q0 = s_tap + ((size_t)kp * psz + idx) * TX;
      const float *q1 = q0 + pw * TX;
      float v[TX];
      if (TX == 2) {
        const float2 v00 = *reinterpret_cast<const float2 *>(q0);
        const float2 v01 = *reinterpret_cast<const float2 *>(q0 + 2);
        const float2 v10 = *reinterpret_cast<const float2 *>(q1);
        const float2 v11 = *reinterpret_cast<const float2 *>(q1 + 2);
        const float t0 = fmaf(fx, v01.x - v00.x, v00.x), a0 = fmaf(fx, v01.y - v00.y, v00.y);
        const float t1 = fmaf(fx, v11.x - v10.x, v10.x), a1 = fmaf(fx, v11.y - v10.y, v10.y);
        v[0] = fmaf(fy, t1 - t0, t0);
        v[1] = fmaf(fy, a1 - a0, a0);
      } else {
#pragma unroll
        for (int c4 = 0; c4 < TX; c4 += 4) {
          const float4 v00 = *reinterpret_cast<const float4 *>(q0 + c4);
          const float4 v01 = *reinterpret_cast<const float4 *>(q0 + TX + c4);
          const float4 v10 = *reinterpret_cast<const float4 *>(q1 + c4);
          const float4 v11 = *reinterpret_cast<const float4 *>(q1 + TX + c4);
          const float e00[4] = {v00.x, v00.y, v00.z, v00.w}, e01[4] = {v01.x, v01.y, v01.z, v01.w};
          const float e10[4] = {v10.x, v10.y, v10.z, v10.w}, e11[4] = {v11.x, v11.y, v11.z, v11.w};
#pragma unroll
          for (int e = 0; e < 4; ++e) {
            if (c4 + e > C) continue;
            const float t0 = fmaf(fx, e01[e] - e00[e], e00[e]);
            const float t1 = fmaf(fx, e11[e] - e10[e], e10[e]);
            v[c4 + e] = fmaf(fy, t1 - t0, t0);
          }
        }
      }
      const float u = v[C] + cb.z;
      uv[q] = u;
#pragma unroll
      for (int c = 0; c < C; ++c) {
        const float df = xv[c] - v[c];
        pv[q][c] = fmaf(df * df, -c2, u);
      }
    }
    {
      float cm = uv[0];
#pragma unroll
      for (int q = 1; q < KC; ++q) cm = fmaxf(cm, uv[q]);
      const float mn = fmaxf(mprior, cm);
      float s = sprior * ex2(mprior - mn);
#pragma unroll
      for (int q = 0; q < KC; ++q) s += ex2(uv[q] - mn);
      mprior = mn, sprior = s;
    }
#pragma unroll
    for (int c = 0; c < C; ++c) {
      float cm = pv[0][c];
#pragma unroll
      for (int q = 1; q < KC; ++q) cm = fmaxf(cm, pv[q][c]);
      const float mn = fmaxf(mpost[c], cm);
      float s = spost[c] * ex2(mpost[c] - mn);
#pragma unroll
      for (int q = 0; q < KC; ++q) s += ex2(pv[q][c] - mn);
      mpost[c] = mn, spost[c] = s;
    }
  }

  const float knorm = -sc.log_sigma - scae::kHalfLog2Pi;
  const float lprior = kLn2 * (mprior + lg2(sprior));
  float lp_sum = 0.f;
#pragma unroll
  for (int c = 0; c < C; ++c) {
    const float lpost = fmaf(kLn2, mpost[c] + lg2(spost[c]), knorm);
    if (live) {
      const size_t o = ((size_t)b * C + c) * HW + p;
      if (log_prob) log_prob[o] = lpost - lprior;
      lse_post[o] = lpost;
      lp_sum += lpost - lprior;
    }
  }
  if (live) lse_prior[(size_t)b * HW + p] = lprior;

  if (block_sums) {
    const float ws = scae::wave_sum(lp_sum);
    const int wid = tid >> 6, nw = nthr >> 6;
    if ((tid & 63) == 0) s_red[wid] = ws;
    __syncthreads();
    if (tid == 0) {
      float s = 0.f;
      for (int w = 0; w < nw; ++w) s += s_red[w];
      block_sums[(size_t)b * n_tiles + tile] = s;
    }
  }
}
#ifndef SCAE_CELL_ABL
#define SCAE_CELL_ABL 0
#endif
#ifndef SCAE_CELL_NT320
#define SCAE_CELL_NT320 0
#endif
#ifndef SCAE_CELL_REC_KB
#define SCAE_CELL_REC_KB 16
#endif
#ifndef SCAE_CELL_ITEMS
#define SCAE_CELL_ITEMS 256
#endif
template <int C> struct RecOf { static constexpr int RS = C == 1 ? 4 : ((C + 4) & ~1); };

__device__ __forceinline__ int fdiv(int n, float inv) { return (int)(((float)n + 0.5f) * inv); }

template <int C, int NTB>
__device__ __forceinline__ void bwd_cell_body(
    const scae_decoder_desc &d, const float *__restrict__ x, const float *__restrict__ lse_post,
    const float *__restrict__ lse_prior, const float *__restrict__ g_logprob,
    const float *__restrict__ g_tile, int lp_tiles, int lp_ppb,
    float *__restrict__ g_templates, float *__restrict__ g_alpha_partial,
    float *__restrict__ g_pose, float *__restrict__ g_presence,
    float *__restrict__ g_bg_image, float *__restrict__ g_scalar_partial, int chunk_rows,
    int max_items, int item_budget, float *smem, int k, int b) {
  constexpr int TX = TexelOf<C>::TX, NV = C + 1, RS = RecOf<C>::RS, NM = 4 * NV;
  const int tid = threadIdx.x;
  const int M = d.M, K = M + 1, W = d.W, H = d.H, HW = H * W, tw = d.tw, th = d.th;
  const int tsz = th * tw, psz = pad_elems(th, tw), pw = pad_w(tw);
  const bool has_scale = d.out_scale != nullptr;
  const float sigma = has_scale ? softplusf_(d.out_scale[0]) + 1e-4f : 1.f;
  const float inv_sigma = has_scale ? 1.f / sigma : 1.f, inv_var = inv_sigma * inv_sigma;
  const float knorm = (has_scale ? -logf(sigma) : 0.f) - scae::kHalfLog2Pi, hvar = 0.5f * inv_var;
  const float inv_wf = 1.f / (float)W, inv_hf = 1.f / (float)H;
  const float inv_ppb = __builtin_amdgcn_rcpf((float)lp_ppb);
  const int chunk_px = chunk_rows * W;

  float *s_pl = smem;
  float *s_rec = s_pl + ((psz * TX + 3) & ~3);
  int *s_id = reinterpret_cast<int *>(s_rec + (((size_t)chunk_px * RS + 3) & ~(size_t)3));
  float *s_part = reinterpret_cast<float *>(s_id + ((chunk_px + 3) & ~3));
  float *s_tex = s_part + (size_t)max_items * NM;
  float *s_red = s_tex + ((NV * tsz + 3) & ~3);

  if (k == M) {
    struct { float bg_ml, bg_val, inv_var; } sc = {softplusf_(d.bg_mixing_logit[0]),
                                                  d.bg_image ? 0.f : sigmoidf_(d.bg_value[0]), inv_var};
    float acc[3] = {0.f, 0.f, 0.f};
    for (int p = tid; p < HW; p += NTB) {
      const float sp = __expf(sc.bg_ml - lse_prior[(size_t)b * HW + p]);
      float gml = 0.f;
#pragma unroll
      for (int c = 0; c < C; ++c) {
        const size_t o = ((size_t)b * C + c) * HW + p;
        const float gc = g_tile ? g_tile[b * lp_tiles + fdiv(p, inv_ppb)] : g_logprob[o];
        const float tv = d.bg_image ? d.bg_image[o] : sc.bg_val;
        const float diff = x[o] - tv;
        const float w = __expf(fmaf(diff * diff, -hvar, knorm) + sc.bg_ml - lse_post[o]);
        const float gtt = gc * w * diff * sc.inv_var;
        gml += gc * (w - sp);
        acc[2] += gc * w * (diff * diff * sc.inv_var - 1.f) * inv_sigma;
        if (d.bg_image) {
          if (g_bg_image) g_bg_image[o] = gtt;
        } else {
          acc[0] += gtt;
        }
      }
      acc[1] += gml;
    }
    scae::block_sum<3, NTB>(acc, s_red);
    if (tid == 0) {
      float *sp = g_scalar_partial + ((size_t)b * K + k) * 4;
      sp[0] = d.bg_image ? 0.f : acc[0] * sc.bg_val * (1.f - sc.bg_val);
      sp[1] = acc[1] * scae::softplus_grad(d.bg_mixing_logit[0]);
      sp[2] = 0.f;
      sp[3] = has_scale ? acc[2] * scae::softplus_grad(d.out_scale[0]) : 0.f;
    }
    return;
  }

  if (d.presence && d.presence[b * M + k] < scae::kLogSafeEps) {
    float *o_t = g_templates + ((size_t)b * M + k) * C * tsz;
    for (int e = tid; e < C * tsz; e += NTB) o_t[e] = 0.f;
    float *o_a = g_alpha_partial + ((size_t)b * M + k) * tsz;
    for (int e = tid; e < tsz; e += NTB) o_a[e] = 0.f;
    if (tid < 6) g_pose[((size_t)b * M + k) * 6 + tid] = 0.f;
    if (tid == 0) {
      if (g_presence) g_presence[b * M + k] = 0.f;
      float *sp = g_scalar_partial + ((size_t)b * K + k) * 4;
      sp[0] = sp[1] = sp[2] = sp[3] = 0.f;
    }
    return;
  }
  {
    const float *ts = d.templates + ((size_t)tb(d, b) * M + k) * C * tsz;
    const float *as = d.templates_alpha + (size_t)k * tsz;
    const float inv_pw = __builtin_amdgcn_rcpf((float)pw);
    for (int e = tid; e < psz; e += NTB) {
      const int yp = fdiv(e, inv_pw), y = yp - 2, xx = e - yp * pw - 2;
      const bool in = y >= 0 && y < th && xx >= 0 && xx < tw;
#pragma unroll
      for (int c = 0; c < TX; ++c)
        s_pl[e * TX + c] = !in || c > C ? 0.f : (c < C ? ts[c * tsz + y * tw + xx] : as[y * tw + xx]);
    }
    for (int e = tid; e < NV * tsz; e += NTB) s_tex[e] = 0.f;
  }
  const float *pa = d.pose + ((size_t)b * M + k) * 6;
  const float pa6[6] = {pa[0], pa[1], pa[2], pa[3], pa[4], pa[5]};
  const float hx = 0.5f * (float)tw, hy = 0.5f * (float)th;
  const float A0 = hx * pa[0], A1 = hx * pa[1], A2 = hx * (pa[2] + 1.f) - 0.5f;
  const float A3 = hy * pa[3], A4 = hy * pa[4], A5 = hy * (pa[5] + 1.f) - 0.5f;
  const float lsp = d.presence ? log_safe(d.presence[b * M + k]) : 0.f;
  const float txf = (float)tw, tyf = (float)th, pwf = (float)pw;
  const float *s_tap = s_pl + (size_t)(2 * pw + 2) * TX;
  const float ax = A0 * 2.f * inv_wf, bx = A1 * 2.f * inv_hf;
  const float c0x = fmaf(A0, inv_wf - 1.f, fmaf(A1, inv_hf - 1.f, A2));
  const float ay = A3 * 2.f * inv_wf, by = A4 * 2.f * inv_hf;
  const float c0y = fmaf(A3, inv_wf - 1.f, fmaf(A4, inv_hf - 1.f, A5));
  const float det = ax * by - bx * ay;
  const float span = fabsf(ax) + fabsf(ay) + fabsf(bx) + fabsf(by);
  const bool det_ok = fabsf(det) > 1e-3f * span && fabsf(det) < 1e30f;
  const float inv_det = det_ok ? __builtin_amdgcn_rcpf(det) : 0.f;
  const bool ax_ok = fabsf(ax) > 1e-3f && fabsf(ax) < 1e30f, ay_ok = fabsf(ay) > 1e-3f && fabsf(ay) < 1e30f;
  constexpr float kSlack = 0.02f;
  const float inv_ax = ax_ok ? __builtin_amdgcn_rcpf(ax) : 0.f, inv_ay = ay_ok ? __builtin_amdgcn_rcpf(ay) : 0.f;
  const float dix = -ay * inv_det, diy = ax * inv_det;
  const float hvar2 = kLog2e * hvar, knorm2 = kLog2e * knorm;
  __syncthreads();

  float acc[8];
#pragma unroll
  for (int i = 0; i < 8; ++i) acc[i] = 0.f;

  for (int r0 = 0; r0 < H; r0 += chunk_rows) {
    const int r1 = min(H, r0 + chunk_rows), p0 = r0 * W, np = (r1 - r0) * W;
    for (int pl = tid; pl < np; pl += NTB) {
      const int p = p0 + pl;
      const int pi = fdiv(p, inv_wf), pj = p - pi * W;
      const float xn = (float)(2 * pj + 1) * inv_wf - 1.f, yn = (float)(2 * pi + 1) * inv_hf - 1.f;
      float ix, iy;
      tex_pos(pa6, xn, yn, tw, th, ix, iy);
      ix = fminf(fmaxf(ix, -2.f), txf);
      iy = fminf(fmaxf(iy, -2.f), tyf);
      const float x0f = floorf(ix), y0f = floorf(iy), fx = ix - x0f, fy = iy - y0f;
      const int idx = (int)fmaf(y0f, pwf, x0f);
      const float *q0 = s_tap + (size_t)idx * TX, *q1 = q0 + pw * TX;
      float v[NV], vdx[NV], vdy[NV];
#pragma unroll
      for (int e = 0; e < NV; ++e) {
        const float v00 = q0[e], v01 = q0[TX + e], v10 = q1[e], v11 = q1[TX + e];
        const float d0 = v01 - v00, d1 = v11 - v10;
        const float t0 = fmaf(fx, d0, v00), t1 = fmaf(fx, d1, v10);
        vdy[e] = t1 - t0;
        v[e] = fmaf(fy, vdy[e], t0);
        vdx[e] = fmaf(fy, d1 - d0, d0);
      }
      const float mlv2 = kLog2e * (v[C] + lsp);
      const float sp = ex2(fmaf(-kLog2e, lse_prior[(size_t)b * HW + p], mlv2));
      const float gct = g_tile ? g_tile[b * lp_tiles + fdiv(p, inv_ppb)] : 0.f;
      float gtt[C], gml = 0.f;
#pragma unroll
      for (int c = 0; c < C; ++c) {
        const size_t o = ((size_t)b * C + c) * HW + p;
        const float gc = g_tile ? gct : g_logprob[o];
        const float diff = x[o] - v[c];
        const float w = ex2(fmaf(diff * diff, -hvar2, fmaf(-kLog2e, lse_post[o], mlv2 + knorm2)));
        const float gw = gc * w;
        gtt[c] = gw * diff * inv_var;
        gml += gc * (w - sp);
        if (has_scale) acc[7] += gw * (diff * diff * inv_var - 1.f) * inv_sigma;
      }
      float gix = gml * vdx[C], giy = gml * vdy[C];
#pragma unroll
      for (int c = 0; c < C; ++c) {
        gix = fmaf(gtt[c], vdx[c], gix);
        giy = fmaf(gtt[c], vdy[c], giy);
      }
      acc[0] = fmaf(gix, xn, acc[0]);
      acc[1] = fmaf(gix, yn, acc[1]);
      acc[2] += gix;
      acc[3] = fmaf(giy, xn, acc[3]);
      acc[4] = fmaf(giy, yn, acc[4]);
      acc[5] += giy;
      acc[6] += gml;
      float *rec = s_rec + (size_t)pl * RS;
      if (C == 1) {
        *reinterpret_cast<float4 *>(rec) = make_float4(gtt[0], gml, fx, fy);
      } else {
#pragma unroll
        for (int c = 0; c < C; ++c) rec[c] = gtt[c];
        rec[C] = gml, rec[C + 1] = fx, rec[C + 2] = fy;
      }
      s_id[pl] = idx;
    }
    __syncthreads();

#if SCAE_CELL_ABL != 1
    int cxlo, cylo, ncx, ncy;
    {
      const float jx = ax * (float)(W - 1), jy = ay * (float)(W - 1);
      const float xa = fmaf(bx, (float)r0, c0x), xb = fmaf(bx, (float)(r1 - 1), c0x);
      const float ya = fmaf(by, (float)r0, c0y), yb = fmaf(by, (float)(r1 - 1), c0y);
      const float xmin = fminf(xa, xb) + fminf(jx, 0.f), xmax = fmaxf(xa, xb) + fmaxf(jx, 0.f);
      const float ymin = fminf(ya, yb) + fminf(jy, 0.f), ymax = fmaxf(ya, yb) + fmaxf(jy, 0.f);
      cxlo = (int)fminf(fmaxf(floorf(xmin - 0.01f), -1.f), txf);
      cylo = (int)fminf(fmaxf(floorf(ymin - 0.01f), -1.f), tyf);
      const int cxhi = (int)fmaxf(fminf(floorf(xmax + 0.01f), txf - 1.f), -2.f);
      const int cyhi = (int)fmaxf(fminf(floorf(ymax + 0.01f), tyf - 1.f), -2.f);
      ncx = max(cxhi - cxlo + 1, 0), ncy = max(cyhi - cylo + 1, 0);
    }
    const int ncells = ncx * ncy;
    int S = 1, G = 1;
    if (ncells > 0) {
      const int L = max(item_budget / ncells, 1);
      const int rows_cell = det_ok ? min(r1 - r0, (int)fminf(fabsf(dix) + fabsf(diy), 1e4f) + 2)
                                   : r1 - r0;
      S = min(min(L, rows_cell), 64);
      const float run = fminf(ax_ok ? fabsf(inv_ax) : 1e4f, ay_ok ? fabsf(inv_ay) : 1e4f);
      const int jspan = min(W, (int)fminf(run, 1e4f) + 2);
      G = max(1, min(L / S, jspan >> 2));
      const int nparts = S * G, nitems = ncells * nparts;
      const float inv_nc = __builtin_amdgcn_rcpf((float)ncells), inv_ncx = __builtin_amdgcn_rcpf((float)ncx);
      const float inv_G = __builtin_amdgcn_rcpf((float)G);
      for (int item = tid; item < nitems; item += NTB) {
        const int part = fdiv(item, inv_nc), cell = item - part * ncells;
        const int sl = fdiv(part, inv_G), seg = part - sl * G;
        const int cyi = fdiv(cell, inv_ncx), cxi = cell - cyi * ncx;
        const float cxf = (float)(cxlo + cxi), cyf = (float)(cylo + cyi);
        const int myid = (int)fmaf(cyf, pwf, cxf);
        const float ux = cxf - c0x, uy = cyf - c0y;
        int ilo = r0, ihi = r1 - 1;
        if (det_ok) {
          const float i00 = (ax * uy - ay * ux) * inv_det;
          const float imin = i00 + fminf(dix, 0.f) + fminf(diy, 0.f);
          const float imax = i00 + fmaxf(dix, 0.f) + fmaxf(diy, 0.f);
          ilo = max(ilo, (int)fminf(fmaxf(ceilf(imin - kSlack), -1.f), (float)H));
          ihi = min(ihi, (int)fmaxf(fminf(floorf(imax + kSlack), (float)H), -1.f));
        }
        float m[NM];
#pragma unroll
        for (int q = 0; q < NM; ++q) m[q] = 0.f;
        for (int i = ilo + sl; i <= ihi; i += S) {
          const float rx = fmaf(-bx, (float)i, ux), ry = fmaf(-by, (float)i, uy);
          float lo = 0.f, hi = (float)(W - 1);
          if (ax_ok) {
            const float t0 = rx * inv_ax, t1 = t0 + inv_ax;
            lo = fmaxf(lo, ceilf(fminf(t0, t1) - kSlack));
            hi = fminf(hi, floorf(fmaxf(t0, t1) + kSlack));
          }
          if (ay_ok) {
            const float t0 = ry * inv_ay, t1 = t0 + inv_ay;
            lo = fmaxf(lo, ceilf(fminf(t0, t1) - kSlack));
            hi = fminf(hi, floorf(fmaxf(t0, t1) + kSlack));
          }
          if (!(lo <= hi)) continue;
          int jl = (int)lo, jh = (int)hi;
          if (G > 1) {
            const int len = fdiv(jh - jl + G, inv_G);
            jl += seg * len;
            jh = min(jh, jl + len - 1);
          }
          const int base = (i - r0) * W;
#if SCAE_CELL_ABL == 2
          if (jl > 10000)
#endif
          for (int pl = base + jl; pl <= base + jh; ++pl) {
            if (s_id[pl] != myid) continue;
            const float *rec = s_rec + (size_t)pl * RS;
            float g[NV], fx, fy;
            if (C == 1) {
              const float4 r4 = *reinterpret_cast<const float4 *>(rec);
              g[0] = r4.x, g[1] = r4.y, fx = r4.z, fy = r4.w;
            } else {
#pragma unroll
              for (int e = 0; e < NV; ++e) g[e] = rec[e];
              fx = rec[NV], fy = rec[NV + 1];
            }
            const float fxy = fx * fy;
#pragma unroll
            for (int e = 0; e < NV; ++e) {
              m[4 * e] += g[e];
              m[4 * e + 1] = fmaf(g[e], fx, m[4 * e + 1]);
              m[4 * e + 2] = fmaf(g[e], fy, m[4 * e + 2]);
              m[4 * e + 3] = fmaf(g[e], fxy, m[4 * e + 3]);
            }
          }
        }
        float *mp = s_part + (size_t)item * NM;
#pragma unroll
        for (int q = 0; q < NM; q += 4)
          *reinterpret_cast<float4 *>(mp + q) = make_float4(m[q], m[q + 1], m[q + 2], m[q + 3]);
      }
    }
    __syncthreads();
    int P = S * G;
    while (P > 6) {
      const int q = (P + 3) >> 2, stride = q * ncells * (NM / 4);
      float4 *dst = reinterpret_cast<float4 *>(s_part);
      for (int t = tid; t < stride; t += NTB) {
        float4 a4 = dst[t];
#pragma unroll
        for (int j = 1; j < 4; ++j)
          if (t + j * stride < P * ncells * (NM / 4)) {
            const float4 b4 = dst[t + j * stride];
            a4 = make_float4(a4.x + b4.x, a4.y + b4.y, a4.z + b4.z, a4.w + b4.w);
          }
        dst[t] = a4;
      }
      __syncthreads();
      P = q;
    }

    if (ncells > 0) {
      const float inv_tw = __builtin_amdgcn_rcpf((float)tw);
      for (int e = tid; e < tsz; e += NTB) {
        const int ty = fdiv(e, inv_tw), tx = e - ty * tw;
        float g[NV];
// ... 71 lines not shown
```

torch_scae_amd/ops.py:

```python
import collections
import ctypes
import functools

import numpy as np
import torch

from . import _lib, step_plan
from ._lib import DecoderDesc, ScaeHipError
from .step_plan import StepPlan, current as _plan

__all__ = ["geometric_transform", "qkv_attention", "set_encoder", "grouped_mlp", "seed_attention", "seed_attention_supported", "seed_fold", "seed_fold_supported", "loss_tail", "loss_tail_scalar", "loss_tail_supported", "capsule_votes",
           "capsule_likelihood", "colored_templates", "template_color_supported", "attention_conv_pool", "attention_pool_supported", "capsule_head", "part_encoder", "conv_stack", "conv_stack_supported",
           "uniform", "reset_noise", "pack_params", "render_templates", "render_gmm_log_prob", "render_gmm_log_prob_sums",
           "gmm_log_prob", "gmm_mean", "gmm_mode", "render_gmm_mode", "render_gmm_parts", "GmmParts", "image_sheet", "ScaeHipError"]


def _need_hip(*tensors):
    for t in tensors:
        if t is None:
            continue
        if not t.is_cuda:
            raise ScaeHipError(
                "torch_scae_amd ops run only on a HIP device (got a "
                f"{t.device} tensor); there is no CPU path.")
        if t.dtype != torch.float32:
            raise ScaeHipError(f"float32 expected, got {t.dtype}")


def _c(t):
    return None if t is None else t.contiguous()


def _p(t):
    return None if t is None else ctypes.c_void_p(t.data_ptr())


def _stream(ref):
    return ctypes.c_void_p(torch.cuda.current_stream(ref.device).cuda_stream)


def _detached(t):
    return None if t is None else t.detach()


def _fwd(f):
    node = f.__qualname__

    @functools.wraps(f)
    def forward(ctx, *args):
        ctx.plan = plan = _plan()
        plan.enter(node)
        return f(ctx, *args)
    return staticmethod(forward)


def _bwd(f):
    node = f.__qualname__

    @functools.wraps(f)
    def backward(ctx, *grads):
        with step_plan.running(ctx.plan, node):
            return f(ctx, *grads)
    return staticmethod(backward)


def _slot(t, ctx=None):
    return getattr(t, "_scae_grad_slot", None) if t is not None else None


def _grad_out(slot, like, shape=None):
    shape = tuple(like.shape if shape is None else shape)
    if slot is not None and tuple(slot.shape) == shape:
        v = slot.take()
        if v is not None:
            v._scae_in_slot = True
            return v
        flush_param_sums()
        flush_pending_backward()
    return torch.empty(shape, device=like.device, dtype=like.dtype)


def _in_slot(t):
    return t is not None and getattr(t, "_scae_in_slot", False)


def _sum_jobs(jobs):
    arr = (_lib.ScaledSum * max(1, len(jobs)))()
    for a, (src, scale, dst) in zip(arr, jobs):
        assert src.is_contiguous() and dst.numel() == 1
        a.src, a.n, a.scale, a.dst = src.data_ptr(), src.numel(), scale, \
            dst.data_ptr()
    return arr


def scaled_sums(jobs):
    _lib.call("scae_scaled_sums_f32", _sum_jobs(jobs), len(jobs),
              _stream(jobs[0][0]))


def mfma_bf16(enabled=True):
    return _plan().precision(enabled)


def _bf16():
    return _plan().bf16


def _prec(name):
    return name.replace("_f32", "_bf16") if _plan().bf16 else name


_FOLD_RIDES = __import__("os").environ.get("SCAE_FOLD_RIDES", "conv")


class StepPrologue:

    def __init__(self):
        self.noise = self.noise_state = None
        self.fold_inputs = self.fold_outs = self.fold_dims = None
        self.first_inputs = self.first_outs = None
        self.first_half = None
        self.noise_fresh = self.fold_fresh = self.first_fresh = False
        self.fold_rides_conv = False
        self.fold_conv_ok = False if _FOLD_RIDES == "prologue" else None

    def _first_desc(self, image):
        _, weights, biases, strides = self.first_inputs
        act, wfs, wds = self.first_outs
        d = _lib.FirstLayerDesc()
        d.img, d.w, d.bias, d.out = image.data_ptr(), weights[0].data_ptr(), \
            biases[0].data_ptr(), act.data_ptr()
        d.B, d.Cin, d.IH, d.IW = image.shape
        d.Cout, d.stride, d.n_layers = weights[0].shape[0], strides[0], len(wfs)
        for i, (w, wf, wd) in enumerate(zip(weights[1:], wfs, wds)):
            d.rw[i], d.rwf[i], d.rwd[i] = w.data_ptr(), wf.data_ptr(), \
                wd.data_ptr()
            d.rCout[i], d.rCin[i] = w.shape[0], w.shape[1]
        if self.first_half is not None:
            act_h, wfh, wdh = self.first_half
            d.out_h = act_h.data_ptr()
            for i, (a, b) in enumerate(zip(wfh, wdh)):
                d.rwfh[i], d.rwdh[i] = a.data_ptr(), b.data_ptr()
        return d

    def launch(self, dst_image=None, src_image=None, dst_label=None,
               src_label=None, stream_ref=None, source=None):
        stage = dst_image is not None
        n_noise = 0 if self.noise is None else self.noise.numel()
        first = self.first_outs is not None and (
            not stage or (dst_image.data_ptr() == self.first_inputs[0].data_ptr()
                          and dst_image.shape == self.first_inputs[0].shape))
        if not (stage or n_noise or self.fold_outs is not None or first):
            return
        ref = dst_image if stage else (
            self.noise if n_noise else (self.fold_outs[0] if self.fold_outs
                                        is not None else self.first_outs[0]))
        _need_hip(ref)
        P = ctypes.c_void_p
        desc = fdesc = None
        fold_here = self.fold_outs is not None and not self.fold_rides_conv
        if fold_here:
            desc = ctypes.byref(_fold_desc(self.fold_inputs, self.fold_outs,
                                           *self.fold_dims))
        if first:
            fdesc = ctypes.byref(self._first_desc(
                src_image if stage and source is None else
                dst_image if stage else self.first_inputs[0]))
        if source is not None:
            _lib.call("scae_step_prologue_source_f32", _p(dst_image),
                      _p(dst_label), dst_image.shape[0], ctypes.byref(source),
                      _p(self.noise), n_noise, _p(self.noise_state), desc, fdesc,
                      _stream(ref))
        else:
            _lib.call("scae_step_prologue_first_f32",
                      _p(dst_image), _p(src_image),
                      dst_image.numel() if stage else 0,
                      P(dst_label.data_ptr()) if stage else None,
                      P(src_label.data_ptr()) if stage else None,
                      dst_label.numel() if stage else 0,
                      _p(self.noise), n_noise, _p(self.noise_state), desc, fdesc,
                      _stream(ref))
        self.noise_fresh = self.noise is not None
        self.fold_fresh = fold_here
        self.first_fresh = first


def step_prologue(pro):
    return _plan().with_prologue(pro)


def reset_noise():
    for plan in step_plan.live_plans():
        for key, (seed, state) in list(plan.noise.items()):
            fresh = (int(torch.initial_seed()) ^ plan.noise_salt) & ((1 << 63) - 1)
            state.copy_(torch.tensor([fresh, 0, 0], dtype=torch.int64))
            plan.noise[key] = (fresh, state)


def uniform(n, ref):
    _need_hip(ref)
    plan = _plan()
    seed = (int(torch.initial_seed()) ^ plan.noise_salt) & ((1 << 63) - 1)
    key = (ref.device, torch.cuda.current_stream(ref.device).cuda_stream)
    state = plan.noise.get(key)
    if state is None or (state[0] != seed and
                         not torch.cuda.is_current_stream_capturing()):
        state = plan.noise[key] = (seed, torch.tensor(
            [seed, 0, 0], dtype=torch.int64).to(ref.device))
    pro = plan.prologue
    if pro is not None:
        if pro.noise is not None and pro.noise.numel() == int(n) \
                and pro.noise_state is state[1] and pro.noise_fresh:
            pro.noise_fresh = False
            return pro.noise
        pro.noise = torch.empty(int(n), device=ref.device, dtype=torch.float32)
        pro.noise_state, pro.noise_fresh = state[1], False
# ... 127 lines not shown
                  V, _stream(right))
        ctx.save_for_backward(left, right)
        return out

    @_bwd
    def backward(ctx, gout):
        left, right = ctx.saved_tensors
        V = right.shape[-3]
        n_caps = right.numel() // (9 * V)
        gright = torch.empty_like(right)
        gleft = torch.empty_like(left) if ctx.needs_input_grad[0] else None
        _lib.call("scae_mat3_mul_bwd_f32", _p(left), _p(right),
                  _p(gout.contiguous()), _p(gleft), _p(gright), n_caps, V,
                  _stream(right))
        return gleft, gright


def mat3_mul(left, right):
    return _Mat3Mul.apply(left, right)


class _QKVAttention(torch.autograd.Function):

    @_fwd
    def forward(ctx, q, k, v, presence):
        bf16 = q.dtype == torch.bfloat16
        if bf16:
            if not (k.dtype == v.dtype == torch.bfloat16 and q.is_cuda):
                raise ScaeHipError("bf16 attention wants q, k and v in bf16 "
                                   "on a HIP device")
            presence = None if presence is None else presence.float()
            _need_hip(presence)
        else:
            _need_hip(q, k, v, presence)
        q, k, v, presence = _c(q), _c(k), _c(v), _c(presence)
        HB, N, dk = q.shape
        M, dv = v.shape[1], v.shape[2]
        out = torch.empty(HB, N, dv, device=q.device, dtype=q.dtype)
        probs = torch.empty(HB, N, M, device=q.device, dtype=torch.float32)
        sqrt_dk = float(np.float32(np.sqrt(dk)))
        if bf16 and (N > 64 or M > 64):
            q32, k32, v32 = q.float(), k.float(), v.float()
            out32 = torch.empty(HB, N, dv, device=q.device, dtype=torch.float32)
            _lib.call("scae_qkv_attention_fwd_f32", _p(q32), _p(k32), _p(v32),
                      _p(presence), _p(out32), _p(probs), HB, N, M, dk, dv,
                      sqrt_dk, _stream(q))
            out.copy_(out32)
        else:
            _lib.call("scae_qkv_attention_fwd_bf16" if bf16 else
                      "scae_qkv_attention_fwd_f32", _p(q), _p(k), _p(v),
                      _p(presence), _p(out), _p(probs), HB, N, M, dk, dv,
                      sqrt_dk, _stream(q))
        ctx.save_for_backward(q, k, v, probs)
        ctx.has_presence = presence is not None
        ctx.sqrt_dk = sqrt_dk
        return out

    @_bwd
    def backward(ctx, gout):
        q, k, v, probs = ctx.saved_tensors
        dtype = q.dtype
        if dtype != torch.float32:
            q, k, v = q.float(), k.float(), v.float()
        HB, N, dk = q.shape
        M, dv = v.shape[1], v.shape[2]
        gout = gout.float().contiguous()
        gq, gk, gv = torch.empty_like(q), torch.empty_like(k), torch.empty_like(v)
        gp = None
        if ctx.has_presence and ctx.needs_input_grad[3]:
            gp = torch.empty(HB, M, device=q.device, dtype=q.dtype)
        _lib.call("scae_qkv_attention_bwd_f32", _p(q), _p(k), _p(v), _p(probs),
                  _p(gout), _p(gq), _p(gk), _p(gv), _p(gp), HB, N, M, dk, dv,
                  ctx.sqrt_dk, _stream(q))
        if dtype != torch.float32:
            gq, gk, gv = gq.to(dtype), gk.to(dtype), gv.to(dtype)
        return gq, gk, gv, gp


def qkv_attention(queries, keys, values, presence=None):
    return _QKVAttention.apply(queries, keys, values, presence)


def _seg_arrays(segs):
    n = len(segs)
    ptrs = (ctypes.c_void_p * n)(*[t.data_ptr() for t in segs])
    widths = (ctypes.c_int * n)(*[t.shape[2] for t in segs])
    rs = (ctypes.c_int * n)(*[t.stride(1) for t in segs])
    bs = (ctypes.c_int64 * n)(*[t.stride(0) for t in segs])
    return ptrs, widths, rs, bs


def step_fusion(target):
    return _plan().fusing(target)


def fusion_target():
    return _plan().target


class LogProbRider:

    def __init__(self, inputs, x):
        t = _prep_decoder(inputs.tensors())
        _need_hip(x)
        self.x = x.detach().contiguous()
        self.desc, (B, M, C, th, tw, H, W) = _make_desc(t, inputs.output_size)
        self._keep = t
        dev, dt = t[0].device, t[0].dtype
        tiles = _lib.load().scae_render_gmm_logprob_tiles(ctypes.byref(self.desc))
        self.sums = torch.empty(B, tiles, device=dev, dtype=dt)
        self.lse_post = torch.empty(B, C, H, W, device=dev, dtype=dt)
        self.lse_prior = torch.empty(B, 1 if t[1] is not None else C, H, W,
                                     device=dev, dtype=dt)
        self.key = self.key_of(inputs, x)
        self.launched = False

    @staticmethod
    def key_of(inputs, x):
        return (x.data_ptr(), tuple(x.shape), tuple(inputs.output_size)) + tuple(
            None if v is None else (v.data_ptr(), tuple(v.shape))
            for v in inputs.tensors())


def offer_log_prob_rider(inputs, x):
    plan = _plan()
    plan.rider = LogProbRider(inputs, x)
    return plan.rider


def evaluating():
    return _plan().evaluation is not None


def withdraw_log_prob_rider():
    plan = _plan()
    if plan.rider is not None and not plan.rider.launched:
        plan.rider = None


class _PendingK1Backward:

    def __init__(self, desc, keep, inputs, outputs, stream_ref):
        self.desc, self.keep, self.ref = desc, (keep, inputs), stream_ref
        self.ptrs = [ctypes.c_void_p(t.data_ptr()) if t is not None else None
                     for t in inputs] + \
                    [None if t is None else ctypes.c_void_p(
                        t if isinstance(t, int) else t.data_ptr())
                     for t in outputs]
        self.keep_out = [t for t in outputs if not isinstance(t, int)]

    def launch_alone(self):
        _lib.call("scae_render_gmm_sums_bwd_f32", ctypes.byref(self.desc),
                  *self.ptrs, _stream(self.ref))


class _PendingWeightGemms:

    def __init__(self, descs, n, keep, stream_ref):
        self.descs, self.n, self.keep, self.ref = descs, n, keep, stream_ref

    def launch_alone(self):
        _lib.call("scae_gemm_multi_f32", self.descs, self.n, _stream(self.ref))


class _PendingTcBackward:

    def __init__(self, ptrs, bm, dims, keep, gf_ptr, stream_ref):
        self.ptrs, self.bm, self.dims = ptrs, bm, dims
        self.keep, self.gf_ptr, self.ref = keep, gf_ptr, stream_ref

    def launch_alone(self):
        _lib.call("scae_template_color_bwd_f32", *self.ptrs, *self.bm,
                  *self.dims, _stream(self.ref))


class _PendingReduce:

    def __init__(self, args, keep, stream_ref):
        self.args, self.keep, self.ref = args, keep, stream_ref

    def launch_alone(self):
        _lib.call("scae_seed_attention_mfma_reduce_f32", *self.args,
                  _stream(self.ref))


class _PendingFoldBackward:

    def __init__(self, desc, grads, keep, stream_ref):
        self.desc, self.grads, self.keep, self.ref = desc, grads, keep, stream_ref

    def launch_alone(self):
        _lib.call("scae_seed_fold_bwd_f32", ctypes.byref(self.desc),
                  ctypes.byref(self.grads), _stream(self.ref))


class _TrunkBackwardOffer:

    def __init__(self, node, z):
        self.node, self.z_ptr, self.shape = node, z.data_ptr(), tuple(z.shape)

    def carry(self, plan, lib, h, args, O, C, parked, gh):
        t = self.node
        B, N, D, Din, Dout, L, ln = t.dims
        if not (plan.parking and plan.carry_trunk_bwd
                and h.data_ptr() == self.z_ptr and tuple(h.shape) == self.shape
                and t.bf16 == plan.bf16
                and lib.scae_object_encoder_bwd_supported(B, N, O, C, D, Din,
                                                          Dout, L, ln)):
            return False
        packed, hsave = t.saved_tensors[:2]
        segs = list(t.saved_tensors[2:2 + t.nseg])
        presence = t.saved_tensors[2 + t.nseg] if t.has_presence else None
        partial, gsegs, gptrs = _trunk_bwd_outputs(t, packed, segs)
        ptrs, widths, rs, bs = _seg_arrays(segs)
        rc = getattr(lib, _prec("scae_object_encoder_bwd_gemm_f32"))(
            *args, parked.descs, parked.n, len(segs), ptrs, widths, rs, bs,
            gptrs, _p(presence), _p(packed), _p(hsave), _p(partial), B, N, D,
            Din, Dout, L, ln, _stream(h))
        if rc == _lib.ERR_UNSUPPORTED:
            return False
        _lib.check(rc, "scae_object_encoder_bwd_gemm")
        t.carried = (gh, partial, gsegs)
        return True


def _trunk_bwd_outputs(ctx, packed, segs):
    B, N = ctx.dims[:2]
    grid = _lib.load().scae_set_encoder_grid(B)
    partial = torch.empty(grid, packed.numel(), device=packed.device,
                          dtype=packed.dtype)
    gsegs = [torch.empty(B, N, t.shape[2], device=t.device, dtype=t.dtype)
             if ctx.needs_input_grad[3 + i] else None
             for i, t in enumerate(segs)]
    gptrs = (ctypes.c_void_p * len(segs))(
        *[None if g is None else g.data_ptr() for g in gsegs])
    return partial, gsegs, gptrs


def flush_pending_backward():
    _plan().flush_scope("deferring")


class _SetEncoder(torch.autograd.Function):
    @_fwd
    def forward(ctx, presence, packed, meta, *segs):
        D, Dout, L, layer_norm = meta
        _need_hip(presence, packed, *segs)
        segs = [t if t.stride(2) == 1 else t.contiguous() for t in segs]
        presence, packed = _c(presence), packed.contiguous()
        B, N = segs[0].shape[:2]
        Din = sum(t.shape[2] for t in segs)
        lib = _lib.load()
        assert packed.numel() == lib.scae_set_encoder_param_count(
            D, Din, Dout, L, int(layer_norm))
        z = torch.empty(B, N, Dout if Dout else D, device=packed.device,
                        dtype=packed.dtype)
        hsave = torch.empty(B, L + 1, N, D, device=packed.device,
                            dtype=packed.dtype)
        ptrs, widths, rs, bs = _seg_arrays(segs)
        ctx.bf16 = bool(_bf16() and lib.scae_set_encoder_bf16_supported(
            N, D, Din, Dout, L, int(layer_norm)))
        rider = ctx.plan.rider
        if rider is not None and not rider.launched \
                and rider.x.device == packed.device:
            _lib.call("scae_set_encoder_fwd_logprob_bf16" if ctx.bf16 else
                      "scae_set_encoder_fwd_logprob_f32", len(segs), ptrs,
                      widths, rs, bs, _p(presence), _p(packed), _p(z),
                      _p(hsave), B, N, D, Din, Dout, L, int(layer_norm),
                      ctypes.byref(rider.desc), _p(rider.x), _p(rider.sums),
                      _p(rider.lse_post), _p(rider.lse_prior), _stream(packed))
            rider.launched = True
        else:
            _lib.call("scae_set_encoder_fwd_bf16" if ctx.bf16 else
                      "scae_set_encoder_fwd_f32", len(segs), ptrs, widths, rs,
                      bs, _p(presence), _p(packed), _p(z), _p(hsave), B, N, D,
                      Din, Dout, L, int(layer_norm), _stream(packed))
        ctx.save_for_backward(packed, hsave, *segs,
                              *([presence] if presence is not None else []))
        ctx.has_presence = presence is not None
        ctx.nseg = len(segs)
        ctx.dims = (B, N, D, Din, Dout, L, int(layer_norm))
        ctx.slot = _slot(packed, ctx)
        ctx.carried = None
        if ctx.plan.fused and ctx.plan.carry_trunk_bwd and Dout == 0 and \
                any(ctx.needs_input_grad) and \
                lib.scae_set_encoder_bf16_supported(N, D, Din, Dout, L,
                                                    int(layer_norm)):
            ctx.plan.offer("trunk_bwd", _TrunkBackwardOffer(ctx, z))
        return z

    @_bwd
    def backward(ctx, gz):
        packed, hsave = ctx.saved_tensors[:2]
        segs = list(ctx.saved_tensors[2:2 + ctx.nseg])
        presence = ctx.saved_tensors[2 + ctx.nseg] if ctx.has_presence else None
        B, N, D, Din, Dout, L, ln = ctx.dims
        gz = gz.contiguous()
        carried, ctx.carried = ctx.carried, None
        if carried is not None and carried[0].data_ptr() == gz.data_ptr():
            _, partial, gsegs = carried
        else:
            partial, gsegs, gptrs = _trunk_bwd_outputs(ctx, packed, segs)
            ptrs, widths, rs, bs = _seg_arrays(segs)
            _lib.call("scae_set_encoder_bwd_bf16" if ctx.bf16 else
                      "scae_set_encoder_bwd_f32", len(segs), ptrs, widths, rs,
                      bs, gptrs, _p(presence), _p(packed), _p(hsave), _p(gz),
# ... 1529 lines not shown
        x, tuple(bool(o) for _, _, o in layers),
        (bool(similarity), bool(learn_vote_scale), bool(allow_deformations),
         bool(defer_reg)), float(noise_scale), cpr_static, bias_cvr, bias_caps,
        bias_vote, bias_scale, noise_caps, noise_vote, *ws, *bs)


def mlp_chain(x, layers, x_is_relu=False):
    ws = [w for w, _, _ in layers]
    bs = [b for _, b, _ in layers]
    return _MLPChain.apply(x, tuple(bool(o) for _, _, o in layers),
                           bool(x_is_relu), *ws, *bs)


def grouped_mlp(x, weights, biases, ones_input=False, grad_pregated=False,
                x_is_relu=False, pad_out=False):
    biases = list(biases) if biases is not None else [None] * len(weights)
    return _GroupedMLP.apply(x, ones_input, len(weights), grad_pregated,
                             x_is_relu, pad_out, *weights, *biases)


class _CapsuleVotes(torch.autograd.Function):
    @_fwd
    def forward(ctx, all_param, cpr_static, b_cvr, b_caps, b_vote, b_scale,
                noise_caps, noise_vote, noise_scale, similarity,
                learn_vote_scale, allow_deformations, param_is_relu,
                defer_reg):
        _need_hip(all_param, cpr_static, b_cvr, b_caps, b_vote, b_scale,
                  noise_caps, noise_vote)
        B, O, A = all_param.shape
        V = (A - 7) // 8
        ldp = all_param.stride(1)
        if not (all_param.stride(2) == 1 and ldp >= A
                and all_param.stride(0) == O * ldp):
            all_param, ldp = all_param.contiguous(), A
        args = [all_param] + [_c(t) for t in (cpr_static, b_cvr, b_caps, b_vote,
                                              b_scale, noise_caps, noise_vote)]
        dev, dt = all_param.device, all_param.dtype
        vote = torch.empty(B, O, V, 6, device=dev, dtype=dt)
        scale = torch.empty(B, O, V, device=dev, dtype=dt)
        vp = torch.empty(B, O, V, device=dev, dtype=dt)
        lc = torch.empty(B, O, 1, device=dev, dtype=dt)
        lv = torch.empty(B, O, V, device=dev, dtype=dt)
        reg = torch.empty(B, O, device=dev, dtype=dt)
        reg_loss = torch.empty((), device=dev, dtype=dt)
        caps_presence = torch.empty(B, O, device=dev, dtype=dt)
        caps_arg = torch.empty(B, O, device=dev, dtype=torch.int32)
        flags = (B, O, V, ldp, int(similarity), int(learn_vote_scale),
                 int(allow_deformations))
        _lib.call("scae_capsule_votes_fwd_f32", *[_p(t) for t in args],
                  float(noise_scale), _p(vote), _p(scale), _p(vp), _p(lc),
                  _p(lv), _p(reg), _p(caps_presence), _p(caps_arg), *flags,
                  _stream(all_param))
        if not defer_reg:
            scaled_sums([(reg, 0.5 / B, reg_loss)])
        ctx.save_for_backward(caps_arg, *[t for t in args if t is not None])
        ctx.has_noise = (args[6] is not None, args[7] is not None)
        ctx.noise_scale = float(noise_scale)
        ctx.flags = flags
        ctx.param_is_relu = bool(param_is_relu)
        ctx.slots = [_slot(t, ctx) for t in (cpr_static, b_cvr, b_caps, b_vote,
                                        b_scale)]
        ctx.set_materialize_grads(False)
        ctx.mark_non_differentiable(reg)
        return vote, scale, vp, lc, lv, reg_loss, caps_presence, reg

    @_bwd
    def backward(ctx, gvote, gscale, gvp, glc, glv, greg, gcp, _greg_partial):
        saved = list(ctx.saved_tensors)
        caps_arg = saved.pop(0)
        args = saved[:6]
        args.append(saved.pop(6) if ctx.has_noise[0] else None)
        args.append(saved[6] if ctx.has_noise[1] else None)
        all_param = args[0]
        B, O, V, ldp = ctx.flags[:4]
        A = all_param.shape[2]
        padded = lambda: torch.empty(B, O, ldp, device=all_param.device,
                                     dtype=all_param.dtype)[:, :, :A]
        gall = padded()
        ggated = padded() if ctx.param_is_relu else None
        gin = torch.empty(B, O, V, 6, device=all_param.device,
                          dtype=all_param.dtype)
        grads = [_c(g) for g in (gvote, gscale, gvp, glc, glv, greg, gcp)]
        _lib.call("scae_capsule_votes_bwd_f32", *[_p(t) for t in args],
                  ctx.noise_scale, *[_p(g) for g in grads], _p(caps_arg),
                  _p(gall), _p(gin), _p(ggated), *ctx.flags,
                  _stream(all_param))
        outs = [_grad_out(sl, t) for sl, t in zip(ctx.slots, args[1:6])]
        gall_rows = torch.as_strided(gall, (B, O * ldp), (O * ldp, 1))
        (g_static,), (g_cvr, g_caps, g_vote, g_scale) = _sum_rows_multi([
            dict(partial=gin.view(B, -1), shapes=[args[1].shape],
                 outs=outs[:1], defer=ctx.slots[0] is not None),
            dict(partial=gall_rows,
                 shapes=[t.shape for t in args[2:6]],
                 starts=[6 * V, 6 * V + 6, 6 * V + 7, 7 * V + 7], period=ldp,
                 outs=outs[1:],
                 defer=all(sl is not None for sl in ctx.slots[1:5]))])
        return (gall if ggated is None else ggated, g_static, g_cvr, g_caps,
                g_vote, g_scale, None, None, None, None, None, None, None, None)


def capsule_votes(all_param, cpr_static, bias_cvr, bias_caps, bias_vote,
                  bias_scale, noise_caps=None, noise_vote=None, noise_scale=0.,
                  similarity=False, learn_vote_scale=True,
                  allow_deformations=True, param_is_relu=False,
                  defer_reg=False):
    return _CapsuleVotes.apply(all_param, cpr_static, bias_cvr, bias_caps,
                               bias_vote, bias_scale, noise_caps, noise_vote,
                               noise_scale, similarity, learn_vote_scale,
                               allow_deformations, param_is_relu, defer_reg)


class _CapsuleLikelihood(torch.autograd.Function):
    @_fwd
    def forward(ctx, vote, scale, vp, dummy_vote, x, presence, defer_sum):
        _need_hip(vote, scale, vp, dummy_vote, x, presence)
        vote, scale, vp, dummy_vote, x, presence = (
            _c(t) for t in (vote, scale, vp, dummy_vote, x, presence))
        B, O, M, _ = vote.shape
        dev, dt = vote.device, vote.dtype
        f = lambda *s: torch.empty(*s, device=dev, dtype=dt)
        lpp, binary = f(B, M), f(B, O, M)
        winner, winner_p = f(B, M, 6), f(B, M)
        widx = torch.empty(B, M, device=dev, dtype=torch.int64)
        from_caps = torch.empty(B, M, device=dev, dtype=torch.int64)
        soft, soft_p = f(B, M, 6), f(B, M)
        post, mlp, mlogit = f(B, O + 1, M), f(B, O + 1, M), f(B, O + 1, M)
        log_prob = torch.empty((), device=dev, dtype=dt)
        _lib.call("scae_capsule_likelihood_fwd_f32", _p(vote), _p(scale),
                  _p(vp), _p(dummy_vote), _p(x), _p(presence), _p(lpp),
                  _p(binary), _p(winner), _p(winner_p), _p(widx),
                  _p(from_caps), _p(soft), _p(soft_p), _p(post), _p(mlp),
                  _p(mlogit), B, O, M, _stream(vote))
        if not defer_sum:
            scaled_sums([(lpp, 1.0 / B, log_prob)])
        saved = [vote, scale, vp, dummy_vote, x, post, widx]
        if presence is not None:
            saved.append(presence)
        ctx.save_for_backward(*saved)
        ctx.has_presence = presence is not None
        ctx.dims = (B, O, M)
        ctx.dummy_shape = dummy_vote.shape
        ctx.mark_non_differentiable(binary, widx, from_caps)
        ctx.set_materialize_grads(False)
        return (lpp, binary, winner, winner_p, widx, from_caps, soft, soft_p,
                post, mlp, mlogit, log_prob)

    @_bwd
    def backward(ctx, g_lpp, _gb, g_w, g_wp, _gi, _gf, g_s, g_sp, g_post,
                 g_mlp, g_mlogit, g_log_prob):
        saved = ctx.saved_tensors
        vote, scale, vp, dummy_vote, x, post, widx = saved[:7]
        presence = saved[7] if ctx.has_presence else None
        B, O, M = ctx.dims
        if g_log_prob is not None:
            spread = (g_log_prob / B).expand(B, M)
            g_lpp = spread if g_lpp is None else g_lpp + spread
        gvote, gscale, gvp = (torch.empty_like(t) for t in (vote, scale, vp))
        gx = torch.empty_like(x)
        gpres = torch.empty(B, M, device=x.device, dtype=x.dtype) \
            if presence is not None else None
        gdummy = torch.empty(B, M, 6, device=x.device, dtype=x.dtype)
        gin = [_c(g) for g in (g_lpp, g_w, g_wp, g_s, g_sp, g_post, g_mlp,
                               g_mlogit)]
        pending = ctx.plan.take("k1_bwd")
        if pending is not None and any(
                g is not None for g in (g_w, g_wp, g_s, g_sp)):
            pending.launch_alone()
            pending = None
        if pending is not None and pending.ref.device == vote.device:
            k = _lib.LikelihoodBwdDesc()
            for name, t in zip(
                    ("vote", "scale", "vote_presence", "dummy_vote", "x",
                     "presence", "posterior", "winner_idx", "g_lpp",
                     "g_winner", "g_winner_presence", "g_soft_winner",
                     "g_soft_winner_presence", "g_posterior",
                     "g_mixing_log_prob", "g_mixing_logit", "gvote", "gscale",
                     "gvote_presence", "gx", "gpresence", "gdummy_partial"),
                    (vote, scale, vp, dummy_vote, x, presence, post, widx,
                     *gin, gvote, gscale, gvp, gx, gpres, gdummy)):
                setattr(k, name, None if t is None else t.data_ptr())
            k.B, k.O, k.M = B, O, M
            _lib.call("scae_render_gmm_sums_bwd_likelihood_f32",
                      ctypes.byref(pending.desc), *pending.ptrs,
                      ctypes.byref(k), _stream(vote))
        else:
            if pending is not None:
                pending.launch_alone()
            _lib.call("scae_capsule_likelihood_bwd_f32", _p(vote), _p(scale),
                      _p(vp), _p(dummy_vote), _p(x), _p(presence), _p(post),
                      _p(widx), *[_p(g) for g in gin], _p(gvote), _p(gscale),
                      _p(gvp), _p(gx), _p(gpres), _p(gdummy), B, O, M,
                      _stream(vote))
        g_dummy = None
        if g_w is not None or g_s is not None:
            g_dummy = _sum_rows(gdummy.view(B, -1), [ctx.dummy_shape])[0]
        return gvote, gscale, gvp, g_dummy, gx, gpres, None


def capsule_likelihood(vote, scale, vote_presence, dummy_vote, x,
                       presence=None, defer_sum=False):
    return _CapsuleLikelihood.apply(vote, scale, vote_presence, dummy_vote, x,
                                    presence, defer_sum)


_SPARSITY_TYPES = {"l2": 0, "entropy": 1, "kl": 2}


def loss_tail_supported(B, O, n_classes):
    return bool(_lib.load().scae_loss_tail_supported(B, O, n_classes or 0))


class _LossTail(torch.autograd.Function):
    @_fwd
    def forward(ctx, lpp, posterior, caps_presence, cls_w, cls_b, label,
                rec_sums, reg, cfg):
        _need_hip(lpp, posterior, caps_presence, cls_w, cls_b, rec_sums, reg)
        ctx.slots = (_slot(cls_w, ctx), _slot(cls_b, ctx))
        lpp, posterior, caps_presence = _c(lpp), _c(posterior), _c(caps_presence)
        cls_w, cls_b, label = _c(cls_w), _c(cls_b), _c(label)
        rec_sums, reg = _c(rec_sums), _c(reg)
        B, O1, M = posterior.shape
        O = O1 - 1
        ncls = 0 if cls_w is None else cls_w.shape[0]
        (n_classes_cfg, prior_type, post_type, sparsity_on, weights,
         within_const, w_reg) = cfg
        w5 = (ctypes.c_float * 5)(*weights)
        ints = (B, O, M, ncls, int(n_classes_cfg or 0), prior_type, post_type,
                int(sparsity_on))
        both = torch.empty(16, device=lpp.device, dtype=lpp.dtype)
        out = both[:12]
        wc = float("nan") if within_const is None else float(within_const)
        lab = None if label is None else ctypes.c_void_p(label.data_ptr())
        ex = _lib.LossExtras()
        if rec_sums is not None:
            ex.rec_sums, ex.n_rec = rec_sums.data_ptr(), rec_sums.numel()
        if reg is not None:
            ex.reg, ex.w_reg = reg.data_ptr(), float(w_reg)
        loss = both[12]
        ex.loss = loss.data_ptr()
        defer = ctx.plan.fused and rec_sums is not None and \
            any(ctx.needs_input_grad) and \
            bool(_lib.load().scae_loss_tail_defer_preferred(B, O))
        ev = ctx.plan.evaluation if ctx.plan.fused and rec_sums is not None else None
        if ev is not None and label is not None and not ctx.plan.holds("class_probs"):
            ev = None
        defer = defer and ev is None
        tl = ctx.plan.train_log if ctx.plan.fused and rec_sums is not None and ev is None \
            else None
        if tl is not None and label is not None and not ctx.plan.holds("class_probs"):
            tl = None
        ex.defer_combine = int(defer or ev is not None)
        ws = torch.empty(_lib.load().scae_loss_tail_workspace_floats(
            ints[0], ints[1], ints[3]), device=lpp.device, dtype=lpp.dtype)
        tail = (_p(lpp), _p(posterior), _p(caps_presence), _p(cls_w), _p(cls_b),
                lab, ctypes.byref(ex), _p(out), _p(ws), *ints, w5, wc)
        parked = ctx.plan.take("class_probs")
        if tl is not None:
            probs = (None, None) if label is None else parked.keep[4:6]
            ex.train_log = ctypes.pointer(tl.fused_desc(*probs, label))
        if ev is not None and parked is not None and ev.sink is not None:
            ev.sink_written = True
            _lib.call("scae_loss_tail_fwd_class_probs_sink_f32", *tail, *parked.args,
                      ctypes.c_void_p(ev.sink.ptr), _stream(lpp))
        elif parked is not None:
            _lib.call("scae_loss_tail_fwd_class_probs_f32", *tail, *parked.args,
                      _stream(lpp))
        else:
            _lib.call("scae_loss_tail_fwd_f32", *tail, _stream(lpp))
        if ev is not None:
            probs = (None, None) if label is None else parked.keep[4:6]
            ev.fused_launch(tail, *probs, keep=(ws, both, ex, w5), stream_ref=lpp)
        ctx.save_for_backward(lpp, posterior, caps_presence, ws,
                              *([cls_w, cls_b, label] if label is not None
                                else []),
                              *([rec_sums] if rec_sums is not None else []),
                              *([reg] if reg is not None else []))
        ctx.has = (label is not None, rec_sums is not None, reg is not None)
        ctx.call = (ints, tuple(weights), wc, float(w_reg))
        ctx.set_materialize_grads(False)
        ctx.deferred = None
        if defer:
            ctx.deferred = _PendingCombine(
                tail, (lpp, posterior, caps_presence, cls_w, cls_b, label,
                       rec_sums, reg, ws, w5, both, ex), loss.data_ptr(),
                out.data_ptr(), lpp)
            ctx.plan.park("combine", ctx.deferred)
        return loss, out

    @_bwd
    def backward(ctx, g_loss, gout):
        saved = list(ctx.saved_tensors)
        lpp, posterior, cp, ws = saved[:4]
        rest = saved[4:]
        has_label, has_rec, has_reg = ctx.has
        cls_w = cls_b = label = rec_sums = reg = None
        if has_label:
            cls_w, cls_b, label = rest[:3]
            rest = rest[3:]
        if has_rec:
            rec_sums, rest = rest[0], rest[1:]
        if has_reg:
            reg = rest[0]
        ints, weights, wc, w_reg = ctx.call
        g_lpp, g_post, g_cp = (torch.empty_like(t) for t in (lpp, posterior, cp))
        g_w = _grad_out(ctx.slots[0], cls_w) if cls_w is not None else None
        g_b = _grad_out(ctx.slots[1], cls_b) if cls_b is not None else None
        g_rec = torch.empty_like(rec_sums) if has_rec else None
        g_reg = torch.empty_like(reg) if has_reg else None
        ex = _lib.LossExtras()
        if has_rec:
            ex.rec_sums, ex.n_rec = rec_sums.data_ptr(), rec_sums.numel()
            ex.g_rec_sums = g_rec.data_ptr()
        if has_reg:
            ex.reg, ex.w_reg, ex.g_reg = reg.data_ptr(), w_reg, g_reg.data_ptr()
        if g_loss is None and gout is None:
            gout = torch.zeros(12, device=lpp.device, dtype=lpp.dtype)
        if g_loss is not None:
            g_loss = g_loss.contiguous()
            ex.g_loss = g_loss.data_ptr()
        pend = ctx.deferred
        if pend is not None and ctx.plan.holds("combine", pend):
            ctx.plan.take("combine")
            ex.defer_combine, ex.loss, ex.out12 = 1, pend.loss_ptr, pend.out_ptr
            ex.train_log = pend.keep[-1].train_log
        w5 = (ctypes.c_float * 5)(*weights)
        lab = None if label is None else ctypes.c_void_p(label.data_ptr())
        _lib.call("scae_loss_tail_bwd_f32", _p(lpp), _p(posterior), _p(cp),
                  _p(cls_w), _p(cls_b), lab, ctypes.byref(ex),
                  _p(_c(gout)), _p(ws), _p(g_lpp), _p(g_post), _p(g_cp),
                  _p(g_w), _p(g_b), *ints, w5, wc, _stream(lpp))
        return g_lpp, g_post, g_cp, g_w, g_b, None, g_rec, g_reg, None


def loss_tail_scalar(lpp, posterior, caps_presence, cls_w, cls_b, label,
                     n_classes, prior_type, post_type, sparsity_on, weights,
                     within_const=None, rec_sums=None, reg=None, w_reg=0.):
    if label is None:
        cls_w = cls_b = None
    cfg = (n_classes, _SPARSITY_TYPES[prior_type], _SPARSITY_TYPES[post_type],
           bool(sparsity_on), [float(w) for w in weights], within_const,
           float(w_reg))
    return _LossTail.apply(lpp, posterior, caps_presence, cls_w, cls_b, label,
                           rec_sums, reg, cfg)


class EvalEpilogue:

    def __init__(self, device):
        self.acc = torch.zeros(_lib.EVAL_ACC_DOUBLES, device=device, dtype=torch.float64)
        self.batch3 = torch.zeros(3, device=device, dtype=torch.float32)
        self.fused = False
        self._keep = None
        self.sink = None
        self.sink_written = False
        self.records = None
        self.records_alone = False

    def fused_launch(self, tail, prior, post, keep, stream_ref):
        _need_hip(prior, post)
        if self.records is not None:
            sink = ctypes.c_void_p(self.sink.ptr) if self.sink_written else None
            _lib.call("scae_eval_tail_records_f32", *tail, _p(prior), _p(post), _p(self.acc),
                      _p(self.batch3), sink, ctypes.c_void_p(self.records.ptr),
                      _stream(stream_ref))
            self.records_alone = False
        elif self.sink_written:
            _lib.call("scae_eval_tail_sink_f32", *tail, _p(prior), _p(post), _p(self.acc),
                      _p(self.batch3), ctypes.c_void_p(self.sink.ptr), _stream(stream_ref))
        else:
            _lib.call("scae_eval_tail_f32", *tail, _p(prior), _p(post), _p(self.acc),
                      _p(self.batch3), _stream(stream_ref))
        self.fused, self._keep = True, (keep, prior, post)

    def accumulate(self, loss, out12, prior, post, label):
        _need_hip(loss, out12, prior, post)
        B = 1 if label is None else label.shape[0]
        ncls = 0 if prior is None else prior.shape[-1]
        loss, out12, prior, post = _c(loss), _c(out12), _c(prior), _c(post)
        lab = None if label is None else ctypes.c_void_p(_c(label).data_ptr())
        _lib.call("scae_eval_accumulate_f32", _p(loss), _p(out12), _p(prior), _p(post), lab,
                  B, ncls, _p(self.acc), _p(self.batch3), _stream(loss))
        self._keep = (loss, out12, prior, post, label)


class EvalSink:

    def __init__(self, device):
        self.desc = torch.zeros(_lib.EVAL_SINK_INT64S, device=device, dtype=torch.int64)
        self.ptr = self.desc.data_ptr()
        self.rows = None

    def point(self, rows):
        if rows is not None:
            if rows.dtype != torch.float32 or rows.dim() != 3 or rows.shape[1] != 2 \
                    or not rows.is_contiguous() or rows.device != self.desc.device:
                raise ValueError("sink rows must be a contiguous (N, 2, O) fp32 tensor on "
                                 "the sink's device")
        self.rows = rows
        n = 0 if rows is None else rows.shape[0]
        self.desc.copy_(torch.tensor([0 if rows is None else rows.data_ptr(), n, 0, 0],
                                     dtype=torch.int64))

    def off(self):
        self.point(None)

    def status(self):
        v = self.desc[2:4].cpu()
        return int(v[0]), bool(v[1])

    def launch_alone(self, caps_presence, posterior):
        _need_hip(caps_presence, posterior)
        cp, post = _c(caps_presence.detach()), _c(posterior.detach())
        B, O1, M = post.shape
        _lib.call("scae_eval_features_f32", _p(cp), _p(post), B, O1 - 1, M,
                  ctypes.c_void_p(self.ptr), _stream(cp))
        self._keep = (cp, post)


class EvalRecords:

    def __init__(self, device):
        self.desc = torch.zeros(_lib.EVAL_RECORDS_INT64S, device=device, dtype=torch.int64)
        self.ptr = self.desc.data_ptr()
        self.rows = self.confusion = None

    def point(self, rows, confusion=None, labelled=True):
        R = _lib.EVAL_RECORD_FLOATS
        dev = self.desc.device
        if rows is not None:
            if rows.dtype != torch.float32 or rows.dim() != 2 or rows.shape[1] != R \
                    or not rows.is_contiguous() or rows.device != dev:
                raise ValueError(f"records rows must be a contiguous (N, {R}) fp32 tensor on "
                                 "the records' device")
            if confusion is not None and (
                    confusion.dtype != torch.int64 or confusion.dim() != 3
                    or confusion.shape[0] != 2 or confusion.shape[1] != confusion.shape[2]
                    or not confusion.is_contiguous() or confusion.device != dev):
                raise ValueError("confusion must be a contiguous (2, ncls, ncls) int64 tensor "
                                 "on the records' device")
        else:
            confusion = None
        self.rows, self.confusion = rows, confusion
        self.desc.copy_(torch.tensor(
            [0 if rows is None else rows.data_ptr(), 0 if rows is None else rows.shape[0], 0, 0,
             0 if confusion is None else confusion.data_ptr(),
             0 if confusion is None else confusion.shape[1], int(bool(labelled))],
            dtype=torch.int64))

    def off(self):
        self.point(None)

    def status(self):
        v = self.desc[2:4].cpu()
        return int(v[0]), bool(v[1])

    def launch_alone(self, prior, post, label, lpp, rec_sums=None, rec_pixels=None):
        _need_hip(prior, post, lpp, rec_sums, rec_pixels)
        prior, post, label, lpp = (_c(t.detach()) if t is not None else None
                                   for t in (prior, post, label, lpp))
        rec = rec_sums if rec_sums is not None else rec_pixels
        rec = _c(rec.detach()).flatten(1) if rec is not None else None
        B, M = lpp.shape
        ncls = 0 if prior is None else prior.shape[-1]
        lab = None if label is None else ctypes.c_void_p(label.data_ptr())
        _lib.call("scae_eval_records_f32", _p(prior), _p(post), lab, _p(lpp),
                  _p(rec if rec_sums is not None else None),
                  _p(rec if rec_sums is None else None), B, ncls, M,
                  0 if rec is None else rec.shape[1], ctypes.c_void_p(self.ptr), _stream(lpp))
        self._keep = (prior, post, label, lpp, rec)


TRAIN_LOG_INDEX = {"loss": 0, "accuracy": 1, "prior_accuracy": 2, "posterior_accuracy": 3,
                   "log_prob": 5, "prior_within_sparsity_loss": 6,
                   "prior_between_sparsity_loss": 7, "posterior_within_sparsity_loss": 8,
                   "posterior_between_sparsity_loss": 9, "prior_cls_xe": 10,
                   "posterior_cls_xe": 11, "rec_ll": 12, "rec_ll_loss": 13,
                   "log_prob_loss": 14, "cpr_dynamic_reg_loss": 15, "learning_rate": 16,
                   "mse": 17, "part_caps_loss": 18}


def ring_order(count, capacity):
    k = min(count, capacity)
    steps = list(range(count - k, count))
    return [s % capacity for s in steps], steps


class TrainLog:

    def __init__(self, capacity, device, lr=None):
        self.capacity = int(capacity)
        self.rows = torch.zeros(self.capacity, _lib.TRAIN_LOG_ROW, device=device,
                                dtype=torch.float32)
        self.step = torch.zeros(1, device=device, dtype=torch.int64)
        self.acc = torch.zeros(_lib.EVAL_ACC_DOUBLES, device=device, dtype=torch.float64)
        self.lr = lr
        self.count = 0
        self.fused = False
        self._keep = None

    def _desc(self, prior, post, label):
        d = _lib.TrainLogDesc()
        d.rows, d.step, d.acc = self.rows.data_ptr(), self.step.data_ptr(), \
            self.acc.data_ptr()
        d.capacity = self.capacity
        d.lr = None if self.lr is None else self.lr.data_ptr()
        if label is not None:
            d.prior_prob, d.post_prob, d.label = prior.data_ptr(), post.data_ptr(), \
                label.data_ptr()
            d.ncls = prior.shape[-1]
        return d

    def fused_desc(self, prior, post, label):
        _need_hip(prior, post)
        d = self._desc(prior, post, label)
        self.fused, self._keep = True, (d, prior, post, label)
        return d

    def log_alone(self, loss, out12, extra2, prior, post, label):
        _need_hip(loss, out12, extra2, prior, post)
        loss, out12, extra2 = _c(loss), _c(out12), _c(extra2)
        prior, post, label = _c(prior), _c(post), _c(label)
        B = 1 if label is None else label.shape[0]
        d = self._desc(prior, post, label)
        _lib.call("scae_train_log_f32", _p(loss), _p(out12), _p(extra2), ctypes.byref(d), B,
                  _stream(loss))
        self._keep = (d, loss, out12, extra2, prior, post, label)

    def reset(self):
        self.rows.zero_()
        self.step.zero_()
        self.acc.zero_()
        self.count = 0


def loss_tail(*args, **kwargs):
    return loss_tail_scalar(*args, **kwargs)[1]


class DecoderInputs:

    FIELDS = ("templates", "templates_alpha", "pose", "presence", "bg_image",
              "bg_value", "bg_mixing_logit", "temperature_logit", "out_scale")

    def __init__(self, output_size, **tensors):
        self.output_size = tuple(output_size)
        for f in self.FIELDS:
            setattr(self, f, tensors.get(f))

    def tensors(self):
        return [getattr(self, f) for f in self.FIELDS]


def _make_desc(tensors, output_size):
    (templates, alpha, pose, presence, bg_image, bg_value, bg_ml, temp,
     out_scale) = tensors
    B0, M, C, th, tw = templates.shape
    B = pose.shape[0]
    if B % B0:
        raise ValueError(f"{B} poses cannot share {B0} template sets")
    H, W = output_size
    d = DecoderDesc(_p(templates), _p(alpha), _p(pose), _p(presence),
                    _p(bg_image), _p(bg_value), _p(bg_ml), _p(temp),
                    _p(out_scale), B, M, C, th, tw, H, W, B // B0)
    return d, (B, M, C, th, tw, H, W)


def _decoder_backward(ctx_tensors, output_size, needs, x, lse_post, lse_prior,
                      g_lp, g_tt, g_ml, g_tile=None, slots=None,
                      alpha_shape=None, park=False):
    (templates, alpha, pose, presence, bg_image, bg_value, bg_ml, temp,
     out_scale) = ctx_tensors
    d, (B, M, C, th, tw, H, W) = _make_desc(ctx_tensors, output_size)
    dev, dt = templates.device, templates.dtype
    g_templates = torch.empty_like(templates)
    g_alpha_p = torch.empty(B, M, th, tw, device=dev, dtype=dt) \
        if alpha is not None else None
    g_pose = torch.empty_like(pose)
    g_presence = torch.empty_like(presence) if presence is not None else None
    g_bg_image = torch.empty_like(bg_image) if bg_image is not None else None
    g_scal = torch.empty(B, M + 1, 4, device=dev, dtype=dt)
    slots = slots or [None] * 9
    jobs, g_alpha, gs = [], None, [None] * 4
    if alpha is not None:
        ashape = tuple(alpha_shape or alpha.shape)
        jobs.append(dict(partial=g_alpha_p.view(B, -1), shapes=[ashape],
                         outs=[_grad_out(slots[1], alpha, ashape)],
                         defer=slots[1] is not None))
    scal = [(i, t) for i, t in enumerate((bg_value, bg_ml, temp, out_scale))
            if t is not None]
    if scal:
        jobs.append(dict(partial=g_scal.view(-1, 4),
                         shapes=[t.shape for _, t in scal],
                         starts=[i for i, _ in scal],
                         outs=[_grad_out(slots[5 + i], t) for i, t in scal],
                         defer=all(slots[5 + i] is not None
                                   for i, _ in scal)))
    if park:
        plan = _plan()
        park = plan.deferred is not None and all(
            job["defer"] and all(_in_slot(o) for o in job["outs"])
            for job in jobs)
    if g_tile is not None and park:
        plan.flush_scope("deferring")
        addr = lambda t: None if t is None else t.data_ptr()
        plan.park("k1_bwd", _PendingK1Backward(
            d, ctx_tensors, (x, lse_post, lse_prior, g_tile),
            (addr(g_templates), g_alpha_p, addr(g_pose), addr(g_presence),
             addr(g_bg_image), g_scal), templates))
    elif g_tile is not None:
        _lib.call("scae_render_gmm_sums_bwd_f32", ctypes.byref(d), _p(x),
                  _p(lse_post), _p(lse_prior), _p(g_tile), _p(g_templates),
                  _p(g_alpha_p), _p(g_pose), _p(g_presence), _p(g_bg_image),
                  _p(g_scal), _stream(templates))
    else:
        _lib.call("scae_render_gmm_bwd_f32", ctypes.byref(d), _p(x),
                  _p(lse_post), _p(lse_prior), _p(g_lp), _p(g_tt), _p(g_ml),
                  _p(g_templates), _p(g_alpha_p), _p(g_pose), _p(g_presence),
                  _p(g_bg_image), _p(g_scal), _stream(templates))
    res = _sum_rows_multi(jobs) if jobs else []
    if alpha is not None:
        g_alpha = res[0][0]
    if scal:
        for (i, _), o in zip(scal, res[-1]):
            gs[i] = o
    return (g_templates, g_alpha, g_pose, g_presence, g_bg_image, *gs)


def _prep_decoder(tensors):
    _need_hip(*tensors)
    tensors = [_c(_detached(t)) for t in tensors]
    if tensors[1] is not None:
        tensors[1] = tensors[1].reshape(-1, *tensors[1].shape[-2:])
    return tensors


class _RenderTemplates(torch.autograd.Function):

    @_fwd
    def forward(ctx, output_size, *tensors):
        t = _prep_decoder(tensors)
        d, (B, M, C, th, tw, H, W) = _make_desc(t, output_size)
        dev, dt = t[0].device, t[0].dtype
        Cm = 1 if t[1] is not None else C
        tt = torch.empty(B, M + 1, C, H, W, device=dev, dtype=dt)
        ml = torch.empty(B, M + 1, Cm, H, W, device=dev, dtype=dt)
        _lib.call("scae_template_render_fwd_f32", ctypes.byref(d), _p(tt),
                  _p(ml), _stream(t[0]))
        ctx.save_for_backward(*[x for x in t if x is not None])
        ctx.present = [x is not None for x in t]
        ctx.output_size = output_size
        ctx.alpha_shape = None if tensors[1] is None else tensors[1].shape
        ctx.slots = [_slot(v, ctx) for v in tensors]
        ctx.set_materialize_grads(False)
        return tt, ml

    @_bwd
    def backward(ctx, g_tt, g_ml):
        if g_tt is None and g_ml is None:
            return (None,) * 10
        it = iter(ctx.saved_tensors)
        t = [next(it) if p else None for p in ctx.present]
        grads = _decoder_backward(t, ctx.output_size, ctx.needs_input_grad,
                                  None, None, None, None, _c(g_tt), _c(g_ml),
                                  slots=ctx.slots, alpha_shape=ctx.alpha_shape)
        grads = list(grads)
        if grads[1] is not None:
            grads[1] = grads[1].view(ctx.alpha_shape)
        return (None, *grads)


class _RenderGmmLogProb(torch.autograd.Function):

    @_fwd
    def forward(ctx, output_size, x, *tensors):
        t = _prep_decoder(tensors)
        _need_hip(x)
        x = x.detach().contiguous()
        d, (B, M, C, th, tw, H, W) = _make_desc(t, output_size)
        dev, dt = t[0].device, t[0].dtype
        Cm = 1 if t[1] is not None else C
        lp = torch.empty(B, C, H, W, device=dev, dtype=dt)
        lse_post = torch.empty(B, C, H, W, device=dev, dtype=dt)
        lse_prior = torch.empty(B, Cm, H, W, device=dev, dtype=dt)
        _lib.call("scae_render_gmm_logprob_fwd_f32", ctypes.byref(d), _p(x),
                  _p(lp), _p(lse_post), _p(lse_prior), _stream(x))
        ctx.save_for_backward(x, lse_post, lse_prior,
                              *[v for v in t if v is not None])
        ctx.present = [v is not None for v in t]
        ctx.output_size = output_size
        ctx.alpha_shape = None if tensors[1] is None else tensors[1].shape
        ctx.slots = [_slot(v, ctx) for v in tensors]
        return lp

    @_bwd
    def backward(ctx, g_lp):
        x, lse_post, lse_prior = ctx.saved_tensors[:3]
        it = iter(ctx.saved_tensors[3:])
        t = [next(it) if p else None for p in ctx.present]
        grads = list(_decoder_backward(t, ctx.output_size, ctx.needs_input_grad,
                                       x, lse_post, lse_prior,
                                       g_lp.contiguous(), None, None,
                                       slots=ctx.slots,
                                       alpha_shape=ctx.alpha_shape))
        if grads[1] is not None:
            grads[1] = grads[1].view(ctx.alpha_shape)
        return (None, None, *grads)


class _RenderGmmLogProbSums(torch.autograd.Function):

    @_fwd
    def forward(ctx, output_size, x, rider, parkable, *tensors):
        ctx.parkable = bool(parkable)
        t = _prep_decoder(tensors)
        _need_hip(x)
        x = x.detach().contiguous()
        if rider is not None:
            sums, lse_post, lse_prior = rider.sums, rider.lse_post, \
                rider.lse_prior
        else:
            d, (B, M, C, th, tw, H, W) = _make_desc(t, output_size)
            dev, dt = t[0].device, t[0].dtype
            Cm = 1 if t[1] is not None else C
            tiles = _lib.load().scae_render_gmm_logprob_tiles(ctypes.byref(d))
            sums = torch.empty(B, tiles, device=dev, dtype=dt)
            lse_post = torch.empty(B, C, H, W, device=dev, dtype=dt)
            lse_prior = torch.empty(B, Cm, H, W, device=dev, dtype=dt)
            _lib.call("scae_render_gmm_logprob_sums_fwd_f32", ctypes.byref(d),
                      _p(x), _p(sums), _p(lse_post), _p(lse_prior), _stream(x))
        ctx.save_for_backward(x, lse_post, lse_prior,
                              *[v for v in t if v is not None])
        ctx.present = [v is not None for v in t]
        ctx.output_size = output_size
        ctx.alpha_shape = None if tensors[1] is None else tensors[1].shape
        ctx.slots = [_slot(v, ctx) for v in tensors]
        return sums

    @_bwd
    def backward(ctx, g_sums):
        x, lse_post, lse_prior = ctx.saved_tensors[:3]
        it = iter(ctx.saved_tensors[3:])
        t = [next(it) if p else None for p in ctx.present]
        grads = list(_decoder_backward(t, ctx.output_size, ctx.needs_input_grad,
                                       x, lse_post, lse_prior, None, None, None,
                                       g_tile=g_sums.contiguous(),
                                       slots=ctx.slots,
                                       alpha_shape=ctx.alpha_shape,
                                       park=ctx.plan.parking
                                       and ctx.parkable))
        if grads[1] is not None:
            grads[1] = grads[1].view(ctx.alpha_shape)
        return (None, None, None, None, *grads)


_K1_GRADIENT_READERS = ("_ColoredTemplatesBackward", "_PartEncoderBackward",
                        "_CapsuleHeadBackward")


def render_gmm_log_prob_sums(inputs: "DecoderInputs", x):
    M, C = inputs.templates.shape[1:3]
    B = inputs.pose.shape[0]
    if tuple(x.shape) != (B, C, *inputs.output_size):
# ... 271 lines not shown
```

torch_scae_amd/step_plan.py:

```python
import collections
import contextlib
import contextvars
import weakref

ANY = "*"
_LIVE = weakref.WeakSet()


class Ride:

    __slots__ = ("carriers", "readers", "scope", "abi", "what")

    def __init__(self, what, carriers, readers=(), scope="deferring", abi=""):
        self.what, self.carriers, self.readers = what, tuple(carriers), readers
        self.scope, self.abi = scope, abi


RIDES = collections.OrderedDict([
    ("tc_fwd", Ride(
        "the colour MLP's forward (K10)",
        carriers=("_PartEncoder.forward",), scope="offer",
        abi="scae_capsule_head_conv_fwd_tc_f32")),
    ("logprob_fwd", Ride(
        "the reconstruction likelihood's forward (K1)",
        carriers=("_SetEncoder.forward",), scope="offer",
        abi="scae_set_encoder_fwd_logprob_f32")),
    ("trunk_bwd", Ride(
        "the object encoder trunk's backward (K2b), set by set behind the "
        "output attention's",
        carriers=("_SeedAttention.backward",), scope="offer",
        abi="scae_object_encoder_bwd_gemm_f32")),
    ("class_probs", Ride(
        "SCAE.forward's two classifier heads (one wave per image)",
        carriers=("_LossTail.forward",), scope="fusing",
        abi="scae_loss_tail_fwd_class_probs_f32")),
    ("combine", Ride(
        "the loss tail's batch combine (one workgroup)",
        carriers=("_LossTail.backward",), scope="fusing",
        abi="scae_loss_tail_bwd_f32 (scae_loss_extras.defer_combine)")),
    ("k1_bwd", Ride(
        "the reconstruction likelihood's backward (K1)",
        carriers=("_CapsuleLikelihood.backward",), readers=ANY,
        abi="scae_render_gmm_sums_bwd_likelihood_f32")),
    ("wgrads", Ride(
        "the capsule MLPs' four weight-gradient GEMMs",
        carriers=("_SeedAttention.backward",),
        abi="scae_seed_attention_mfma_bwd_gemm_f32")),
    ("tc_bwd", Ride(
        "the colour MLP's backward (K10)",
        carriers=("_PartEncoder.backward",),
        readers=("_CapsuleHead.backward",),
        abi="scae_capsule_head_bwd_tc_f32")),
    ("reduce", Ride(
        "the output attention's partial-row reduction",
        carriers=("_PartEncoder.backward", "_ConvStack.backward"),
        abi="scae_conv3x3_bwd_pair_reduce_f32")),
    ("fold_bwd", Ride(
        "the folding products' backward (K2d)",
        carriers=("_PartEncoder.backward", "_ConvStack.backward"),
        abi="scae_conv3x3_bwd_pair_fold_f32")),
])


class StepPlan:
    def __init__(self, name="step", prologue=None):
        _LIVE.add(self)
        self.name = name
        self.target = None
        self.rider = None
        self.offers = {}
        self.parked = {}
        self.deferred = None
        self.sums_to_optimizer = False
        self.held_sums = []
        self.prologue = prologue
        self.bf16 = False
        self.carry_trunk_bwd = True
        self.noise = {}
        self.noise_salt = 0
        self.side_stream = None
        self.evaluation = None
        self.train_log = None

    @contextlib.contextmanager
    def active(self):
        token = _CURRENT.set(self)
        try:
            yield self
        finally:
            _CURRENT.reset(token)

    @property
    def fused(self):
        return self.target is not None

    @property
    def parking(self):
        return self.target is not None and self.deferred is not None

    def offer(self, kind, work):
        assert RIDES[kind].scope == "offer", kind
        self.offers[kind] = work

    def claim(self, kind):
        return self.offers.pop(kind, None)

    def park(self, kind, work):
        assert kind in RIDES and RIDES[kind].scope != "offer", kind
        stale = self.parked.pop(kind, None)
        if stale is not None:
            stale.launch_alone()
        self.parked[kind] = work

    def take(self, kind):
        return self.parked.pop(kind, None)

    def holds(self, kind, work=None):
        held = self.parked.get(kind)
        return held is not None and (work is None or held is work)

    def flush(self, *kinds):
        for kind in RIDES:
            if (not kinds or kind in kinds) and kind in self.parked:
                self.parked.pop(kind).launch_alone()

    def flush_scope(self, scope):
        self.flush(*[k for k, r in RIDES.items() if r.scope == scope])

    def enter(self, node):
        if not self.parked:
            return
        for kind in RIDES:
            if kind not in self.parked:
                continue
            ride = RIDES[kind]
            if node in ride.carriers:
                continue
            if ride.readers == ANY or node in ride.readers:
                self.parked.pop(kind).launch_alone()

    def flush_sums(self):
        if self.deferred:
            units = list(self.deferred)
            del self.deferred[:]
            from . import ops
            ops._launch_sum_units(units)

    def take_held_sums(self):
        units, self.held_sums = self.held_sums, []
        return units

    @contextlib.contextmanager
    def fusing(self, target):
        prev = (self.target, self.rider)
        self.target, self.rider = target, None
        self.parked.clear()
        self.offers.clear()
        ok = False
        try:
            yield self
            ok = True
        finally:
            self.target, self.rider = prev
            self.offers.clear()
            if ok:
                self.flush_scope("fusing")

    @contextlib.contextmanager
    def deferring(self):
        outer = self.deferred
        if outer is None:
            self.deferred = []
        ok = False
        try:
            yield self
            ok = True
        finally:
            if outer is None:
                try:
                    if ok:
                        self.flush_scope("deferring")
                        if self.sums_to_optimizer:
                            self.held_sums.extend(self.deferred)
                            del self.deferred[:]
                        else:
                            self.flush_sums()
                finally:
                    self.deferred = None

    @contextlib.contextmanager
    def with_prologue(self, pro):
        prev, self.prologue = self.prologue, pro
        try:
            yield pro
        finally:
            self.prologue = prev

    @contextlib.contextmanager
    def evaluating(self, epilogue):
        prev, self.evaluation = self.evaluation, epilogue
        try:
            yield self
        finally:
            self.evaluation = prev

    @contextlib.contextmanager
    def logging(self, train_log):
        prev, self.train_log = self.train_log, train_log
        try:
            yield self
        finally:
            self.train_log = prev

    @contextlib.contextmanager
    def precision(self, bf16):
        prev, self.bf16 = self.bf16, bool(bf16)
        try:
            yield self
        finally:
            self.bf16 = prev


def live_plans():
    return list(_LIVE)


_CURRENT = contextvars.ContextVar("scae_step_plan", default=None)
ambient = StepPlan("ambient")


# ... 14 lines not shown
```

Before: 271,300.

## Park the loss-tail backward and ride it inside the fused likelihood/render backward launch

Instead of launching the loss tail's backward kernel on its own, the autograd step parks it in the step plan. It is then carried into the combined render-GMM/likelihood backward kernel through a new tail descriptor pointer, which removes one kernel launch and its serialization point per step. The tail body and combine are refactored into shared device code, and the combine can now run with fewer threads per wave. Safety checks fall back to a standalone launch when pointers, devices or gradient readers don't match, which adds host-side bookkeeping and a larger combined kernel.

```diff
diff --git a/include/scae_hip.h b/include/scae_hip.h
--- a/include/scae_hip.h
+++ b/include/scae_hip.h
@@ -799,6 +799,15 @@
                                       float *tile_sums, float *lse_post, float *lse_prior,
                                       void *stream);
 
+typedef struct scae_loss_tail_ride_desc {
+  const float *lpp, *posterior, *caps_presence, *cls_w, *cls_b;
+  const int64_t *label;
+  scae_loss_extras extras;
+  const float *gout12, *workspace;
+  float *g_lpp, *g_posterior, *g_caps_presence, *g_cls_w, *g_cls_b;
+  int B, O, M, ncls, n_classes_cfg, prior_type, post_type, sparsity_on;
+  float weights5[5], within_const;
+} scae_loss_tail_ride_desc;
 typedef struct scae_likelihood_bwd_desc {
   const float *vote, *scale, *vote_presence, *dummy_vote, *x, *presence, *posterior;
   const int64_t *winner_idx;
@@ -806,6 +815,7 @@
       *g_posterior, *g_mixing_log_prob, *g_mixing_logit;
   float *gvote, *gscale, *gvote_presence, *gx, *gpresence, *gdummy_partial;
   int B, O, M;
+  const scae_loss_tail_ride_desc *tail;
 } scae_likelihood_bwd_desc;
 int scae_render_gmm_sums_bwd_likelihood_f32(
     const scae_decoder_desc *d, const float *x, const float *lse_post, const float *lse_prior,
diff --git a/torch_scae_amd/_lib.py b/torch_scae_amd/_lib.py
--- a/torch_scae_amd/_lib.py
+++ b/torch_scae_amd/_lib.py
@@ -18,16 +18,6 @@
                 ("B", c_int), ("M", c_int), ("C", c_int), ("th", c_int),
                 ("tw", c_int), ("H", c_int), ("W", c_int),
                 ("template_repeat", c_int)]
-
-
-class LikelihoodBwdDesc(Structure):
-    _fields_ = [(n, P) for n in (
-        "vote", "scale", "vote_presence", "dummy_vote", "x", "presence",
-        "posterior", "winner_idx", "g_lpp", "g_winner", "g_winner_presence",
-        "g_soft_winner", "g_soft_winner_presence", "g_posterior",
-        "g_mixing_log_prob", "g_mixing_logit", "gvote", "gscale",
-        "gvote_presence", "gx", "gpresence", "gdummy_partial")] + [
-        ("B", c_int), ("O", c_int), ("M", c_int)]
 
 
 class GemmDesc(Structure):
@@ -95,6 +85,28 @@
                 ("w_reg", c_float), ("g_rec_sums", P), ("g_reg", P),
                 ("loss", P), ("g_loss", P), ("defer_combine", c_int),
                 ("out12", P), ("train_log", POINTER(TrainLogDesc))]
+
+
+class LossTailRideDesc(Structure):
+    _fields_ = [(n, P) for n in ("lpp", "posterior", "caps_presence", "cls_w",
+                                 "cls_b", "label")] + \
+        [("extras", LossExtras), ("gout12", P), ("workspace", P)] + \
+        [(n, P) for n in ("g_lpp", "g_posterior", "g_caps_presence", "g_cls_w",
+                          "g_cls_b")] + \
+        [(n, c_int) for n in ("B", "O", "M", "ncls", "n_classes_cfg",
+                              "prior_type", "post_type", "sparsity_on")] + \
+        [("weights5", c_float * 5), ("within_const", c_float)]
+
+
+class LikelihoodBwdDesc(Structure):
+    _fields_ = [(n, P) for n in (
+        "vote", "scale", "vote_presence", "dummy_vote", "x", "presence",
+        "posterior", "winner_idx", "g_lpp", "g_winner", "g_winner_presence",
+        "g_soft_winner", "g_soft_winner_presence", "g_posterior",
+        "g_mixing_log_prob", "g_mixing_logit", "gvote", "gscale",
+        "gvote_presence", "gx", "gpresence", "gdummy_partial")] + [
+        ("B", c_int), ("O", c_int), ("M", c_int),
+        ("tail", POINTER(LossTailRideDesc))]
 
 
 class KMeansDesc(Structure):
diff --git a/torch_scae_amd/csrc/loss_tail.hip b/torch_scae_amd/csrc/loss_tail.hip
--- a/torch_scae_amd/csrc/loss_tail.hip
+++ b/torch_scae_amd/csrc/loss_tail.hip
@@ -5,11 +5,6 @@
 namespace {
 using namespace scae_tail;
 constexpr int MAXCLS = 32;
-
-__device__ __forceinline__ float ent_term_grad(float p, float k) {
-  const float q = p * k;
-  return q < scae::kLogSafeEps ? 1e8f : -(logf(q) + 1.f);
-}
 
 __device__ __forceinline__ float within_term(const float *x, float r, int O, int type,
                                              float cw, int lane) {
@@ -125,127 +120,6 @@
   train_log_epilogue<NTC>(g, out, out, nullptr);
 }
 
-__device__ __forceinline__ void sparsity_grad(const float *x, const float *col, float r, int B,
-                                              int O, int type, float cw, float cb, float gw,
-                                              float gb, float *g, int lane) {
-  if (type == 0) {
-    for (int o = lane; o < O; o += 64)
-      g[o] = gw * 2.f * (r - cw) / B + gb * 2.f * (col[o] - cb) / O;
-    return;
-  }
-  const float k = type == 2 ? (float)O : 1.f;
-  float tot = 0.f;
-  for (int o = 0; o < O; ++o) tot += col[o];
-  const float tinv = 1.f / (tot + 1e-8f), rinv = 1.f / (r + 1e-8f);
-  float dot_b = 0.f, dot_w = 0.f;
-  for (int o = lane; o < O; o += 64) {
-    dot_b += ent_term_grad(col[o] * tinv, k) * col[o] * tinv;
-    dot_w += ent_term_grad(x[o] * rinv, k) * x[o] * rinv;
-  }
-  dot_b = scae::wave_sum(dot_b);
-  dot_w = scae::wave_sum(dot_w);
-  for (int o = lane; o < O; o += 64) {
-    const float dw = (ent_term_grad(x[o] * rinv, k) - dot_w) * rinv / B;
-    const float db = -(ent_term_grad(col[o] * tinv, k) - dot_b) * tinv;
-    g[o] = gw * dw + gb * db;
-  }
-}
-
-template <int NT>
-__device__ __forceinline__ void tail_bwd_body(const TailArgs &a, const scae_loss_extras &x,
-                                              const Ws &ws, const float *gout ,
-                                              float *g_lpp, float *g_post, float *g_cp,
-                                              float *g_w, float *g_b, float *smem) {
-  const int B = a.B, O = a.O, M = a.M, tid = threadIdx.x;
-  float go[12];
-#pragma unroll
-  for (int i = 0; i < 12; ++i) go[i] = gout ? gout[i] : 0.f;
-  if (x.g_loss) go[0] += x.g_loss[0];
-  const float g0 = go[0];
-  if ((int)blockIdx.x >= B) {
-    if (!(a.label && g_w)) return;
-    const float g_x1 = (g0 + go[6]) / B, g_x2 = (g0 + go[7]) / B;
-    const int nout = a.ncls * O + a.ncls;
-    const int out = ((int)blockIdx.x - B) * (NT / 4) + (tid >> 2), part = tid & 3;
-    float t = 0.f;
-    if (out < a.ncls * O) {
-      const int cc = out / O, o = out - cc * O;
-      float t0 = 0.f, t1 = 0.f, t2 = 0.f, t3 = 0.f;
-      int b = part;
-      for (; b + 12 < B; b += 16) {
-#define SCAE_TERM(bb)                                                                  \
-  (ws.gl[((size_t)(bb) * 2) * a.ncls + cc] * g_x1 * a.cp[(size_t)(bb) * O + o] +      \
-   ws.gl[((size_t)(bb) * 2 + 1) * a.ncls + cc] * g_x2 * ws.mass[(size_t)(bb) * O + o])
-        const float u0 = SCAE_TERM(b), u1 = SCAE_TERM(b + 4), u2 = SCAE_TERM(b + 8),
-                    u3 = SCAE_TERM(b + 12);
-        t0 += u0, t1 += u1, t2 += u2, t3 += u3;
-      }
-      for (; b < B; b += 4) t0 += SCAE_TERM(b);
-#undef SCAE_TERM
-      t = (t0 + t1) + (t2 + t3);
-    } else if (out < nout) {
-      const int cc = out - a.ncls * O;
-#pragma unroll 4
-      for (int b = part; b < B; b += 4)
-        t += ws.gl[((size_t)b * 2) * a.ncls + cc] * g_x1 +
-             ws.gl[((size_t)b * 2 + 1) * a.ncls + cc] * g_x2;
-    }
-    t += scae::xor1_f(t);
-    t += scae::xor2_f(t);
-    if (part == 0 && out < nout) {
-      if (out < a.ncls * O)
-        g_w[out] = t;
-      else
-        g_b[out - a.ncls * O] = t;
-    }
-    return;
-  }
-  const int b = blockIdx.x;
-  const float g_lp = (-a.w_ll * g0 + go[1] - go[10]) / B;
-  for (int m = tid; m < M; m += NT) g_lpp[(size_t)b * M + m] = g_lp;
-  if (x.g_rec_sums) {
-    const float gr = (-g0 + go[8] - go[9]) / B;
-    const int per = (x.n_rec + B - 1) / B, i1 = min(x.n_rec, (b + 1) * per);
-    for (int i = b * per + tid; i < i1; i += NT) x.g_rec_sums[i] = gr;
-  }
-  if (x.g_reg && b == 0 && tid == 0) x.g_reg[0] = x.w_reg * g0 + go[11];
-  float *s_cp = smem, *s_mass = s_cp + O, *col = s_mass + O, *gc = col + 2 * O, *gm = gc + O;
-  for (int o = tid; o < O; o += NT) {
-    s_cp[o] = a.cp[(size_t)b * O + o];
-    s_mass[o] = ws.mass[(size_t)b * O + o] / M;
-    if (!x.defer_combine) {
-      col[o] = ws.col[o];
-      col[O + o] = ws.col[O + o];
-    }
-    gc[o] = gm[o] = 0.f;
-  }
-  if (x.defer_combine) column_sums<NT>(a, ws, col, tid, false);
-  __syncthreads();
-  if (a.sparsity_on && tid < 64) {
-    const float *p = ws.part + (size_t)b * 8;
-    sparsity_grad(s_cp, col, p[5], B, O, a.prior_type, a.l2_within_const, a.l2_between_const,
-                  a.w_pw * g0 + go[2], a.w_pb * g0 + go[3], gc, tid);
-    sparsity_grad(s_mass, col + O, p[6], B, O, a.post_type, a.l2_within_const_post,
-                  a.l2_between_const_post, a.w_qw * g0 + go[4], a.w_qb * g0 + go[5], gm, tid);
-  }
-  __syncthreads();
-  for (int o = tid; o < O; o += NT) g_cp[(size_t)b * O + o] = gc[o];
-  float *gp = g_post + (size_t)b * (O + 1) * M;
-  if ((M & 3) == 0) {
-    const int M4 = M / 4;
-    for (int e = tid; e < (O + 1) * M4; e += NT) {
-      const int o = e / M4;
-      const float v = o < O ? gm[o] / M : 0.f;
-      reinterpret_cast<float4 *>(gp)[e] = make_float4(v, v, v, v);
-    }
-  } else {
-    for (int e = tid; e < (O + 1) * M; e += NT) {
-      const int o = e / M;
-      gp[e] = o < O ? gm[o] / M : 0.f;
-    }
-  }
-}
-
 template <int NT>
 __global__ __launch_bounds__(NT) void tail_bwd_kernel(TailArgs a, scae_loss_extras x, Ws ws,
                                                       const float *gout , float *g_lpp,
@@ -445,41 +319,68 @@
                                       int B, int O, int M, int ncls, int n_classes_cfg,
                                       int prior_type, int post_type, int sparsity_on,
                                       const float *weights5, float within_const, void *stream) {
-  TailArgs a;
-  int rc = fill_tail(a, lpp, posterior, caps_presence, cls_w, cls_b, label, B, O, M, ncls,
-                     n_classes_cfg, prior_type, post_type, sparsity_on, weights5, within_const);
-  if (rc) return rc;
-  SCAE_REQUIRE(g_lpp && g_posterior && g_caps_presence && workspace);
-  if (!gout12 && !(extras && extras->g_loss)) return SCAE_ERR_BAD_ARG;
-  scae_loss_extras x{};
-  if (extras) x = *extras;
+  if (!weights5) return SCAE_ERR_BAD_ARG;
+  scae_loss_tail_ride_desc t{lpp, posterior, caps_presence, cls_w, cls_b, label,
+                             extras ? *extras : scae_loss_extras{}, gout12, workspace, g_lpp,
+                             g_posterior, g_caps_presence, g_cls_w, g_cls_b, B, O, M, ncls,
+                             n_classes_cfg, prior_type, post_type, sparsity_on,
+                             {weights5[0], weights5[1], weights5[2], weights5[3], weights5[4]},
+                             within_const};
+  return launch_ride_alone(t, stream);
+}
+
+int scae_tail::fill_ride(TailRide &r, const scae_loss_tail_ride_desc &t, bool &rides) {
+  rides = false;
+  int rc = fill_tail(r.a, t.lpp, t.posterior, t.caps_presence, t.cls_w, t.cls_b, t.label, t.B,
+                     t.O, t.M, t.ncls, t.n_classes_cfg, t.prior_type, t.post_type,
+                     t.sparsity_on, t.weights5, t.within_const);
+  if (rc) return rc;
+  SCAE_REQUIRE(t.g_lpp && t.g_posterior && t.g_caps_presence && t.workspace);
+  const scae_loss_extras &x = t.extras;
+  if (!t.gout12 && !x.g_loss) return SCAE_ERR_BAD_ARG;
   if (x.rec_sums && (x.n_rec <= 0 || !x.g_rec_sums)) return SCAE_ERR_BAD_ARG;
   if (x.reg && !x.g_reg) return SCAE_ERR_BAD_ARG;
-  if (label) SCAE_REQUIRE(g_cls_w && g_cls_b);
-  const Ws ws = carve_ws(const_cast<float *>(workspace), B, O, ncls);
+  if (t.label) SCAE_REQUIRE(t.g_cls_w && t.g_cls_b);
   if (x.defer_combine) SCAE_REQUIRE(x.out12);
-  const size_t lds = 6 * O * sizeof(float) > combine_lds(O) ? 6 * O * sizeof(float) : combine_lds(O);
+  r.x = x;
+  r.ws = carve_ws(const_cast<float *>(t.workspace), t.B, t.O, t.ncls);
+  r.gout = t.gout12;
+  r.g_lpp = t.g_lpp, r.g_post = t.g_posterior, r.g_cp = t.g_caps_presence;
+  r.g_w = t.g_cls_w, r.g_b = t.g_cls_b;
+  r.n_cls = cls_blocks(r.a, NTRIDE);
+  r.has_log = 0;
+  r.log = TrainLogArgs{};
   if (x.defer_combine && x.train_log) {
-    TrainLogArgs g;
-    rc = fill_train_log(g, *x.train_log, B);
+    rc = fill_train_log(r.log, *x.train_log, t.B);
     if (rc) return rc;
-    const int cls_blocks = label ? (ncls * O + ncls + NT_SMALL / 4 - 1) / (NT_SMALL / 4) : 0;
-    scae::launch(tail_bwd_log_kernel<NT_SMALL>, dim3(B + cls_blocks + 1), dim3(NT_SMALL), lds,
-                 (hipStream_t)stream, a, x, ws, gout12, g_lpp, g_posterior, g_caps_presence,
-                 g_cls_w, g_cls_b, g);
+    r.has_log = 1;
+  }
+  rides = x.defer_combine && scae_loss_tail_defer_preferred(t.B, t.O) && t.B <= 1024 &&
+          x.rec_sums;
+  return SCAE_OK;
+}
+
+int scae_tail::launch_ride_alone(const scae_loss_tail_ride_desc &t, void *stream) {
+  TailRide r;
+  bool rides;
+  const int rc = fill_ride(r, t, rides);
+  if (rc) return rc;
+  const size_t lds = ride_lds(t.O);
+  hipStream_t st = (hipStream_t)stream;
+  if (r.has_log) {
+    scae::launch(tail_bwd_log_kernel<NT_SMALL>, dim3(t.B + cls_blocks(r.a, NT_SMALL) + 1),
+                 dim3(NT_SMALL), lds, st, r.a, r.x, r.ws, r.gout, r.g_lpp, r.g_post, r.g_cp,
+                 r.g_w, r.g_b, r.log);
     return scae_launch_status();
   }
-#define SCAE_TAIL_BWD(NTH)                                                                       \
-  do {                                                                                           \
-    const int cls_blocks = label ? (ncls * O + ncls + NTH / 4 - 1) / (NTH / 4) : 0;              \
-    scae::launch(tail_bwd_kernel<NTH>, dim3(B + cls_blocks + (x.defer_combine ? 1 : 0)),   \
-                       dim3(NTH), lds, (hipStream_t)stream, a, x, ws, gout12, g_lpp, g_posterior, \
-                       g_caps_presence, g_cls_w, g_cls_b);                                       \
-  } while (0)
-  if (x.defer_combine || scae_loss_tail_defer_preferred(B, O))
-    SCAE_TAIL_BWD(NT_SMALL);
+  const int comb = r.x.defer_combine ? 1 : 0;
+  if (comb || scae_loss_tail_defer_preferred(t.B, t.O))
+    scae::launch(tail_bwd_kernel<NT_SMALL>, dim3(t.B + cls_blocks(r.a, NT_SMALL) + comb),
+                 dim3(NT_SMALL), lds, st, r.a, r.x, r.ws, r.gout, r.g_lpp, r.g_post, r.g_cp,
+                 r.g_w, r.g_b);
   else
-    SCAE_TAIL_BWD(NTB_LARGE);
-#undef SCAE_TAIL_BWD
+    scae::launch(tail_bwd_kernel<NTB_LARGE>, dim3(t.B + cls_blocks(r.a, NTB_LARGE)),
+                 dim3(NTB_LARGE), lds, st, r.a, r.x, r.ws, r.gout, r.g_lpp, r.g_post, r.g_cp,
+                 r.g_w, r.g_b);
   return scae_launch_status();
 }
diff --git a/torch_scae_amd/csrc/loss_tail_dev.h b/torch_scae_amd/csrc/loss_tail_dev.h
--- a/torch_scae_amd/csrc/loss_tail_dev.h
+++ b/torch_scae_amd/csrc/loss_tail_dev.h
@@ -79,21 +79,57 @@
   }
 }
 
-template <int NTC>
+template <int NTC, int NTR = NTC>
 __device__ __forceinline__ void combine_body(const TailArgs &a, const scae_loss_extras &x,
                                              const Ws &ws, float *out, float *smem) {
+  static_assert(NTC % NTR == 0 && NTR % 64 == 0, "whole waves of the NTC form per thread");
+  constexpr int R = NTC / NTR, NW = NTC / 64;
   const int B = a.B, O = a.O, tid = threadIdx.x;
   float *col = smem, *red = smem + 2 * O;
   float v[6] = {0.f, 0.f, 0.f, 0.f, 0.f, 0.f};
-  for (int b = tid; b < B; b += NTC) {
-    const float4 p = *reinterpret_cast<const float4 *>(ws.part + (size_t)b * 8);
-    v[0] += p.x, v[1] += p.y, v[2] += p.z, v[3] += p.w;
-    v[4] += ws.part[(size_t)b * 8 + 4];
-  }
-  if (x.rec_sums)
-    for (int i = tid; i < x.n_rec; i += NTC) v[5] += x.rec_sums[i];
-  column_sums<NTC>(a, ws, col, tid, true);
-  scae::block_sum<6, NTC>(v, red);
+  if (R == 1) {
+    for (int b = tid; b < B; b += NTC) {
+      const float4 p = *reinterpret_cast<const float4 *>(ws.part + (size_t)b * 8);
+      v[0] += p.x, v[1] += p.y, v[2] += p.z, v[3] += p.w;
+      v[4] += ws.part[(size_t)b * 8 + 4];
+    }
+    if (x.rec_sums)
+      for (int i = tid; i < x.n_rec; i += NTC) v[5] += x.rec_sums[i];
+    column_sums<NTC>(a, ws, col, tid, true);
+    scae::block_sum<6, NTC>(v, red);
+  } else {
+    float u[R][6];
+#pragma unroll
+    for (int r = 0; r < R; ++r) {
+#pragma unroll
+      for (int i = 0; i < 6; ++i) u[r][i] = 0.f;
+      for (int b = tid + r * NTR; b < B; b += NTC) {
+        const float4 p = *reinterpret_cast<const float4 *>(ws.part + (size_t)b * 8);
+        u[r][0] += p.x, u[r][1] += p.y, u[r][2] += p.z, u[r][3] += p.w;
+        u[r][4] += ws.part[(size_t)b * 8 + 4];
+      }
+      if (x.rec_sums)
+        for (int i = tid + r * NTR; i < x.n_rec; i += NTC) u[r][5] += x.rec_sums[i];
+    }
+    column_sums<NTR>(a, ws, col, tid, true);
+#pragma unroll
+    for (int r = 0; r < R; ++r)
+#pragma unroll
+      for (int i = 0; i < 6; ++i) {
+        const float s = scae::wave_sum(u[r][i]);
+        if ((tid & 63) == 0) red[i * NW + r * (NTR / 64) + (tid >> 6)] = s;
+      }
+    __syncthreads();
+    if (tid == 0) {
+#pragma unroll
+      for (int i = 0; i < 6; ++i) {
+        float s = 0.f;
+        for (int w = 0; w < NW; ++w) s += red[i * NW + w];
+        v[i] = s;
+      }
+    }
+    __syncthreads();
+  }
   if (tid >= 64) return;
   float pb = 0.f, qb = 0.f;
   if (a.sparsity_on) {
@@ -109,6 +145,156 @@
                      a.w_qb * qb + xe1 + xe2 - rec + x.w_reg * reg;
   out[0] = loss;
   if (x.loss) x.loss[0] = loss;
+}
+
+__device__ __forceinline__ float ent_term_grad(float p, float k) {
+  const float q = p * k;
+  return q < scae::kLogSafeEps ? 1e8f : -(logf(q) + 1.f);
+}
+
+
+__device__ __forceinline__ void sparsity_grad(const float *x, const float *col, float r, int B,
+                                              int O, int type, float cw, float cb, float gw,
+                                              float gb, float *g, int lane) {
+  if (type == 0) {
+    for (int o = lane; o < O; o += 64)
+      g[o] = gw * 2.f * (r - cw) / B + gb * 2.f * (col[o] - cb) / O;
+    return;
+  }
+  const float k = type == 2 ? (float)O : 1.f;
+  float tot = 0.f;
+  for (int o = 0; o < O; ++o) tot += col[o];
+  const float tinv = 1.f / (tot + 1e-8f), rinv = 1.f / (r + 1e-8f);
+  float dot_b = 0.f, dot_w = 0.f;
+  for (int o = lane; o < O; o += 64) {
+    dot_b += ent_term_grad(col[o] * tinv, k) * col[o] * tinv;
+    dot_w += ent_term_grad(x[o] * rinv, k) * x[o] * rinv;
+  }
+  dot_b = scae::wave_sum(dot_b);
+  dot_w = scae::wave_sum(dot_w);
+  for (int o = lane; o < O; o += 64) {
+    const float dw = (ent_term_grad(x[o] * rinv, k) - dot_w) * rinv / B;
+    const float db = -(ent_term_grad(col[o] * tinv, k) - dot_b) * tinv;
+    g[o] = gw * dw + gb * db;
+  }
+}
+
+__device__ __forceinline__ void tail_upstream(const float *gout ,
+                                              const scae_loss_extras &x, float (&go)[12]) {
+#pragma unroll
+  for (int i = 0; i < 12; ++i) go[i] = gout ? gout[i] : 0.f;
+  if (x.g_loss) go[0] += x.g_loss[0];
+}
+__device__ __forceinline__ float rec_upstream(const float (&go)[12], int B) {
+  return (-go[0] + go[8] - go[9]) / B;
+}
+
+template <int NT>
+__device__ __forceinline__ void tail_bwd_cls_body(const TailArgs &a, const Ws &ws,
+                                                  const float (&go)[12], float *g_w, float *g_b,
+                                                  int blk) {
+  const int B = a.B, O = a.O, tid = threadIdx.x;
+  const float g0 = go[0];
+  if (!(a.label && g_w)) return;
+  const float g_x1 = (g0 + go[6]) / B, g_x2 = (g0 + go[7]) / B;
+  const int nout = a.ncls * O + a.ncls;
+  const int out = blk * (NT / 4) + (tid >> 2), part = tid & 3;
+  float t = 0.f;
+  if (out < a.ncls * O) {
+    const int cc = out / O, o = out - cc * O;
+    float t0 = 0.f, t1 = 0.f, t2 = 0.f, t3 = 0.f;
+    int b = part;
+    for (; b + 12 < B; b += 16) {
+#define SCAE_TERM(bb)                                                                  \
+  (ws.gl[((size_t)(bb) * 2) * a.ncls + cc] * g_x1 * a.cp[(size_t)(bb) * O + o] +      \
+   ws.gl[((size_t)(bb) * 2 + 1) * a.ncls + cc] * g_x2 * ws.mass[(size_t)(bb) * O + o])
+      const float u0 = SCAE_TERM(b), u1 = SCAE_TERM(b + 4), u2 = SCAE_TERM(b + 8),
+                  u3 = SCAE_TERM(b + 12);
+      t0 += u0, t1 += u1, t2 += u2, t3 += u3;
+    }
+    for (; b < B; b += 4) t0 += SCAE_TERM(b);
+#undef SCAE_TERM
+    t = (t0 + t1) + (t2 + t3);
+  } else if (out < nout) {
+    const int cc = out - a.ncls * O;
+#pragma unroll 4
+    for (int b = part; b < B; b += 4)
+      t += ws.gl[((size_t)b * 2) * a.ncls + cc] * g_x1 +
+           ws.gl[((size_t)b * 2 + 1) * a.ncls + cc] * g_x2;
+  }
+  t += scae::xor1_f(t);
+  t += scae::xor2_f(t);
+  if (part == 0 && out < nout) {
+    if (out < a.ncls * O)
+      g_w[out] = t;
+    else
+      g_b[out - a.ncls * O] = t;
+  }
+}
+
+template <int NT>
+__device__ __forceinline__ void tail_bwd_image_body(const TailArgs &a, const scae_loss_extras &x,
+                                                    const Ws &ws, const float (&go)[12],
+                                                    float *g_lpp, float *g_post, float *g_cp,
+                                                    float *smem, int b) {
+  const int B = a.B, O = a.O, M = a.M, tid = threadIdx.x;
+  const float g0 = go[0];
+  const float g_lp = (-a.w_ll * g0 + go[1] - go[10]) / B;
+  for (int m = tid; m < M; m += NT) g_lpp[(size_t)b * M + m] = g_lp;
+  if (x.g_rec_sums) {
+    const float gr = rec_upstream(go, B);
+    const int per = (x.n_rec + B - 1) / B, i1 = min(x.n_rec, (b + 1) * per);
+    for (int i = b * per + tid; i < i1; i += NT) x.g_rec_sums[i] = gr;
+  }
+  if (x.g_reg && b == 0 && tid == 0) x.g_reg[0] = x.w_reg * g0 + go[11];
+  float *s_cp = smem, *s_mass = s_cp + O, *col = s_mass + O, *gc = col + 2 * O, *gm = gc + O;
+  for (int o = tid; o < O; o += NT) {
+    s_cp[o] = a.cp[(size_t)b * O + o];
+    s_mass[o] = ws.mass[(size_t)b * O + o] / M;
+    if (!x.defer_combine) {
+      col[o] = ws.col[o];
+      col[O + o] = ws.col[O + o];
+    }
+    gc[o] = gm[o] = 0.f;
+  }
+  if (x.defer_combine) column_sums<NT>(a, ws, col, tid, false);
+  __syncthreads();
+  if (a.sparsity_on && tid < 64) {
+    const float *p = ws.part + (size_t)b * 8;
+    sparsity_grad(s_cp, col, p[5], B, O, a.prior_type, a.l2_within_const, a.l2_between_const,
+                  a.w_pw * g0 + go[2], a.w_pb * g0 + go[3], gc, tid);
+    sparsity_grad(s_mass, col + O, p[6], B, O, a.post_type, a.l2_within_const_post,
+                  a.l2_between_const_post, a.w_qw * g0 + go[4], a.w_qb * g0 + go[5], gm, tid);
+  }
+  __syncthreads();
+  for (int o = tid; o < O; o += NT) g_cp[(size_t)b * O + o] = gc[o];
+  float *gp = g_post + (size_t)b * (O + 1) * M;
+  if ((M & 3) == 0) {
+    const int M4 = M / 4;
+    for (int e = tid; e < (O + 1) * M4; e += NT) {
+      const int o = e / M4;
+      const float v = o < O ? gm[o] / M : 0.f;
+      reinterpret_cast<float4 *>(gp)[e] = make_float4(v, v, v, v);
+    }
+  } else {
+    for (int e = tid; e < (O + 1) * M; e += NT) {
+      const int o = e / M;
+      gp[e] = o < O ? gm[o] / M : 0.f;
+    }
+  }
+}
+
+template <int NT>
+__device__ __forceinline__ void tail_bwd_body(const TailArgs &a, const scae_loss_extras &x,
+                                              const Ws &ws, const float *gout ,
+                                              float *g_lpp, float *g_post, float *g_cp,
+                                              float *g_w, float *g_b, float *smem) {
+  float go[12];
+  tail_upstream(gout, x, go);
+  if ((int)blockIdx.x >= a.B)
+    tail_bwd_cls_body<NT>(a, ws, go, g_w, g_b, (int)blockIdx.x - a.B);
+  else
+    tail_bwd_image_body<NT>(a, x, ws, go, g_lpp, g_post, g_cp, smem, blockIdx.x);
 }
 
 
@@ -214,4 +400,24 @@
               int ncls, int n_classes_cfg, int prior_type, int post_type, int sparsity_on,
               const float *weights , float within_const);
 int fill_train_log(TrainLogArgs &g, const scae_train_log_desc &d, int B);
-}
+
+constexpr int NTRIDE = 256;
+struct TailRide {
+  TailArgs a;
+  scae_loss_extras x;
+  Ws ws;
+  const float *gout;
+  float *g_lpp, *g_post, *g_cp, *g_w, *g_b;
+  int n_cls;
+  int has_log;
+  TrainLogArgs log;
+};
+inline int cls_blocks(const TailArgs &a, int nt) {
+  return a.label ? (a.ncls * a.O + a.ncls + nt / 4 - 1) / (nt / 4) : 0;
+}
+inline size_t ride_lds(int O) {
+  return 6 * O * sizeof(float) > combine_lds(O) ? 6 * O * sizeof(float) : combine_lds(O);
+}
+int fill_ride(TailRide &r, const scae_loss_tail_ride_desc &t, bool &rides);
+int launch_ride_alone(const scae_loss_tail_ride_desc &t, void *stream);
+}
diff --git a/torch_scae_amd/csrc/render_bwd_likelihood.hip b/torch_scae_amd/csrc/render_bwd_likelihood.hip
--- a/torch_scae_amd/csrc/render_bwd_likelihood.hip
+++ b/torch_scae_amd/csrc/render_bwd_likelihood.hip
@@ -1,5 +1,6 @@
 #include "common.h"
 #include "capsule_likelihood_dev.h"
+#include "loss_tail_dev.h"
 #include "render_gmm_wave_dev.h"
 
 namespace {
@@ -33,6 +34,109 @@
                                  g_scalar_partial, chunk_rows, max_items, item_budget, smem, k, b);
 }
 
+template <typename T>
+__device__ __forceinline__ const T *handed_over(const T *p) {
+  asm volatile("" : "+r"(p));
+  return p;
+}
+
+__device__ __forceinline__ bool riders(const LkBwd &lk, int n_lk, const scae_tail::TailRide &t,
+                                       float *smem, int &id) {
+  using namespace scae_tail;
+  if (id == 0) {
+    combine_body<NT_SMALL, NTRIDE>(t.a, t.x, t.ws, t.x.out12, smem);
+    if (t.has_log) {
+      __syncthreads();
+      train_log_epilogue<NTRIDE>(t.log, t.x.out12, t.x.out12, nullptr);
+    }
+    return true;
+  }
+  id -= 1;
+  if (id < n_lk) {
+    float go[12];
+    tail_upstream(t.gout, t.x, go);
+    tail_bwd_image_body<NTRIDE>(t.a, t.x, t.ws, go, t.g_lpp, t.g_post, t.g_cp, smem, id);
+    __threadfence_block();
+    __syncthreads();
+    scae_lk::likelihood_bwd_body<false, 256>(
+        lk.a, lk.winner_idx, handed_over(lk.g_lpp), lk.g_winner, lk.g_winner_presence,
+        lk.g_soft_winner, lk.g_soft_winner_presence, handed_over(lk.g_posterior), lk.g_mlp,
+        lk.g_mlogit, lk.gvote, lk.gscale, lk.gvp, lk.gx, lk.gpresence, lk.gdummy, smem, id, n_lk);
+    return true;
+  }
+  id -= n_lk;
+  if (id < t.n_cls) {
+    float go[12];
+    tail_upstream(t.gout, t.x, go);
+    tail_bwd_cls_body<NTRIDE>(t.a, t.ws, go, t.g_w, t.g_b, id);
+    return true;
+  }
+  id -= t.n_cls;
+  return false;
+}
+
+template <int C>
+__global__ __launch_bounds__(256, 5) void bwd_cell_likelihood_tail_kernel(
+    scae_decoder_desc d, const float *__restrict__ x, const float *__restrict__ lse_post,
+    const float *__restrict__ lse_prior, int lp_tiles, int lp_ppb,
+    float *__restrict__ g_templates, float *__restrict__ g_alpha_partial,
+    float *__restrict__ g_pose, float *__restrict__ g_presence, float *__restrict__ g_bg_image,
+    float *__restrict__ g_scalar_partial, int chunk_rows, int max_items, int item_budget,
+    LkBwd lk, int n_lk, scae_tail::TailRide t) {
+  extern __shared__ __attribute__((aligned(16))) float smem[];
+  int id = blockIdx.x;
+  if (riders(lk, n_lk, t, smem, id)) return;
+  const int K = d.M + 1, b = id / K, k = id - b * K;
+  float go[12];
+  scae_tail::tail_upstream(t.gout, t.x, go);
+  scae_k1::bwd_cell_body<C, 256, true>(d, x, lse_post, lse_prior, nullptr, nullptr, lp_tiles,
+                                       lp_ppb, g_templates, g_alpha_partial, g_pose, g_presence,
+                                       g_bg_image, g_scalar_partial, chunk_rows, max_items,
+                                       item_budget, smem, k, b,
+                                       scae_tail::rec_upstream(go, t.a.B));
+}
+
+__global__ __launch_bounds__(256) void tail_likelihood_kernel(LkBwd lk, int n_lk,
+                                                              scae_tail::TailRide t) {
+  extern __shared__ __attribute__((aligned(16))) float smem[];
+  int id = blockIdx.x;
+  riders(lk, n_lk, t, smem, id);
+}
+
+template <int C>
+int launch_tail(const scae_decoder_desc *d, const scae_k1::CellGeom &g,
+                const scae_k1::LpTiling &lt, const float *x, const float *lse_post,
+                const float *lse_prior, float *g_templates, float *g_alpha_partial,
+                float *g_pose, float *g_presence, float *g_bg_image, float *g_scalar_partial,
+                const LkBwd &lk, const scae_tail::TailRide &t, hipStream_t st) {
+  if (g.lds > 48 * 1024) {
+    hipError_t e =
+        hipFuncSetAttribute(reinterpret_cast<const void *>(bwd_cell_likelihood_tail_kernel<C>),
+                            hipFuncAttributeMaxDynamicSharedMemorySize, (int)g.lds);
+    if (e != hipSuccess) return (int)e;
+  }
+  const int n_lk = lk.a.B;
+  scae::launch((bwd_cell_likelihood_tail_kernel<C>),
+               dim3(1 + n_lk + t.n_cls + (d->M + 1) * d->B), dim3(256), g.lds, st, *d, x,
+               lse_post, lse_prior, lt.tiles, lt.ppb, g_templates, g_alpha_partial, g_pose,
+               g_presence, g_bg_image, g_scalar_partial, g.chunk_rows, g.max_items,
+               g.item_budget, lk, n_lk, t);
+  return scae_launch_status();
+}
+
+int launch_tail_likelihood(const LkBwd &lk, const scae_tail::TailRide &t, hipStream_t st) {
+  const size_t lds_k = scae_lk::lk_lds(lk.a.O, lk.a.M, true), lds_t = scae_tail::ride_lds(lk.a.O);
+  const size_t lds = lds_k > lds_t ? lds_k : lds_t;
+  if (lds > 48 * 1024) {
+    hipError_t e = hipFuncSetAttribute(reinterpret_cast<const void *>(tail_likelihood_kernel),
+                                       hipFuncAttributeMaxDynamicSharedMemorySize, (int)lds);
+    if (e != hipSuccess) return (int)e;
+  }
+  scae::launch(tail_likelihood_kernel, dim3(1 + lk.a.B + t.n_cls), dim3(256), lds, st, lk,
+               lk.a.B, t);
+  return scae_launch_status();
+}
+
 template <int C>
 int launch(const scae_decoder_desc *d, const scae_k1::CellGeom &g, const scae_k1::LpTiling &lt,
            const float *x, const float *lse_post, const float *lse_prior, const float *g_tile,
@@ -62,11 +166,30 @@
     const scae_likelihood_bwd_desc *k, void *stream) {
   SCAE_REQUIRE(d && k);
   const char *e = getenv("SCAE_FUSE_K1_K4_BWD");
+  const char *et = getenv("SCAE_FUSE_TAIL_BWD");
   const scae_k1::CellGeom g = scae_k1::cell_geom(d);
-  const bool fits = !(e && *e == '0') && g.lds && (d->C == 1 || d->C == 3) && k->O <= 64 &&
-                    scae_lk::lk_lds(k->O, k->M, true) <= g.lds && k->B > 0 && k->O > 0 &&
-                    k->M > 0 && d->template_repeat <= 1;
-  if (!fits) {
+  const bool shapes = g.lds && (d->C == 1 || d->C == 3) && k->O <= 64 &&
+                      scae_lk::lk_lds(k->O, k->M, true) <= g.lds && k->B > 0 && k->O > 0 &&
+                      k->M > 0 && d->template_repeat <= 1;
+  const bool fits = !(e && *e == '0') && shapes;
+  scae_tail::TailRide t;
+  bool ride = false;
+  if (k->tail) {
+    const scae_loss_tail_ride_desc &r = *k->tail;
+    int rc = scae_tail::fill_ride(t, r, ride);
+    if (rc) return rc;
+    ride = ride && shapes && !(et && *et == '0') && scae_tail::ride_lds(r.O) <= g.lds &&
+           g.lds + 64 <= 64 * 1024 &&
+           r.B == k->B && r.O == k->O && r.M == k->M && r.B == d->B &&
+           r.g_lpp == k->g_lpp && r.g_posterior == k->g_posterior &&
+           r.extras.g_rec_sums == g_tile_sums &&
+           (int64_t)r.extras.n_rec == (int64_t)d->B * scae_k1::lp_tiling(d).tiles;
+    if (!ride) {
+      rc = scae_tail::launch_ride_alone(r, stream);
+      if (rc) return rc;
+    }
+  }
+  if (!fits && !ride) {
     int rc = scae_render_gmm_sums_bwd_f32(d, x, lse_post, lse_prior, g_tile_sums, g_templates,
                                           g_alpha_partial, g_pose, g_presence, g_bg_image,
                                           g_scalar_partial, stream);
@@ -102,6 +225,18 @@
            k->gpresence,
            k->gdummy_partial};
   hipStream_t st = (hipStream_t)stream;
+  if (ride && !fits) {
+    int rc = launch_tail_likelihood(lk, t, st);
+    if (rc) return rc;
+    return scae_render_gmm_sums_bwd_f32(d, x, lse_post, lse_prior, g_tile_sums, g_templates,
+                                        g_alpha_partial, g_pose, g_presence, g_bg_image,
+                                        g_scalar_partial, stream);
+  }
+#define SCAE_TAIL(CC)                                                                     \
+  launch_tail<CC>(d, g, lt, x, lse_post, lse_prior, g_templates, g_alpha_partial, g_pose, \
+                  g_presence, g_bg_image, g_scalar_partial, lk, t, st)
+  if (ride) return d->C == 1 ? SCAE_TAIL(1) : SCAE_TAIL(3);
+#undef SCAE_TAIL
   return d->C == 1 ? launch<1>(d, g, lt, x, lse_post, lse_prior, g_tile_sums, g_templates,
                                g_alpha_partial, g_pose, g_presence, g_bg_image, g_scalar_partial,
                                lk, st)
diff --git a/torch_scae_amd/csrc/render_gmm_wave_dev.h b/torch_scae_amd/csrc/render_gmm_wave_dev.h
--- a/torch_scae_amd/csrc/render_gmm_wave_dev.h
+++ b/torch_scae_amd/csrc/render_gmm_wave_dev.h
@@ -227,7 +227,7 @@
 
 __device__ __forceinline__ int fdiv(int n, float inv) { return (int)(((float)n + 0.5f) * inv); }
 
-template <int C, int NTB>
+template <int C, int NTB, bool UNI = false>
 __device__ __forceinline__ void bwd_cell_body(
     const scae_decoder_desc &d, const float *__restrict__ x, const float *__restrict__ lse_post,
     const float *__restrict__ lse_prior, const float *__restrict__ g_logprob,
@@ -235,7 +235,7 @@
     float *__restrict__ g_templates, float *__restrict__ g_alpha_partial,
     float *__restrict__ g_pose, float *__restrict__ g_presence,
     float *__restrict__ g_bg_image, float *__restrict__ g_scalar_partial, int chunk_rows,
-    int max_items, int item_budget, float *smem, int k, int b) {
+    int max_items, int item_budget, float *smem, int k, int b, float g_uni = 0.f) {
   constexpr int TX = TexelOf<C>::TX, NV = C + 1, RS = RecOf<C>::RS, NM = 4 * NV;
   const int tid = threadIdx.x;
   const int M = d.M, K = M + 1, W = d.W, H = d.H, HW = H * W, tw = d.tw, th = d.th;
@@ -265,7 +265,9 @@
 #pragma unroll
       for (int c = 0; c < C; ++c) {
         const size_t o = ((size_t)b * C + c) * HW + p;
-        const float gc = g_tile ? g_tile[b * lp_tiles + fdiv(p, inv_ppb)] : g_logprob[o];
+        const float gc = UNI      ? g_uni
+                         : g_tile ? g_tile[b * lp_tiles + fdiv(p, inv_ppb)]
+                                  : g_logprob[o];
         const float tv = d.bg_image ? d.bg_image[o] : sc.bg_val;
         const float diff = x[o] - tv;
         const float w = __expf(fmaf(diff * diff, -hvar, knorm) + sc.bg_ml - lse_post[o]);
@@ -369,12 +371,12 @@
       }
       const float mlv2 = kLog2e * (v[C] + lsp);
       const float sp = ex2(fmaf(-kLog2e, lse_prior[(size_t)b * HW + p], mlv2));
-      const float gct = g_tile ? g_tile[b * lp_tiles + fdiv(p, inv_ppb)] : 0.f;
+      const float gct = UNI ? g_uni : g_tile ? g_tile[b * lp_tiles + fdiv(p, inv_ppb)] : 0.f;
       float gtt[C], gml = 0.f;
 #pragma unroll
       for (int c = 0; c < C; ++c) {
         const size_t o = ((size_t)b * C + c) * HW + p;
-        const float gc = g_tile ? gct : g_logprob[o];
+        const float gc = UNI || g_tile ? gct : g_logprob[o];
         const float diff = x[o] - v[c];
         const float w = ex2(fmaf(diff * diff, -hvar2, fmaf(-kLog2e, lse_post[o], mlv2 + knorm2)));
         const float gw = gc * w;
diff --git a/torch_scae_amd/ops.py b/torch_scae_amd/ops.py
--- a/torch_scae_amd/ops.py
+++ b/torch_scae_amd/ops.py
@@ -61,7 +61,22 @@
     def backward(ctx, *grads):
         with step_plan.running(ctx.plan, node):
             return f(ctx, *grads)
+    backward._scae_node = node
     return staticmethod(backward)
+
+
+_VIEW_NODES = ("ViewBackward0", "ReshapeAliasBackward0", "UnsafeViewBackward0",
+               "AliasBackward0")
+
+
+def _gradient_reader(t):
+    if t is None or not t.requires_grad:
+        return ""
+    fn = t.grad_fn
+    while fn is not None and type(fn).__name__ in _VIEW_NODES:
+        fn = fn.next_functions[0][0] if fn.next_functions else None
+    cls = getattr(fn, "_forward_cls", None)
+    return getattr(getattr(cls, "backward", None), "_scae_node", None)
 
 
 def _slot(t, ctx=None):
@@ -495,6 +510,37 @@
     def launch_alone(self):
         _lib.call("scae_render_gmm_sums_bwd_f32", ctypes.byref(self.desc),
                   *self.ptrs, _stream(self.ref))
+
+
+class _PendingTailBackward:
+
+    def __init__(self, desc, keep, stream_ref):
+        self.desc, self.keep, self.ref = desc, keep, stream_ref
+        self.g_lpp, self.g_post = desc.g_lpp, desc.g_posterior
+        self.g_rec = desc.extras.g_rec_sums
+
+    def launch_alone(self):
+        d = self.desc
+        _lib.call("scae_loss_tail_bwd_f32", d.lpp, d.posterior, d.caps_presence,
+                  d.cls_w, d.cls_b, d.label, ctypes.byref(d.extras), d.gout12,
+                  d.workspace, d.g_lpp, d.g_posterior, d.g_caps_presence,
+                  d.g_cls_w, d.g_cls_b, d.B, d.O, d.M, d.ncls, d.n_classes_cfg,
+                  d.prior_type, d.post_type, d.sparsity_on, d.weights5,
+                  d.within_const, _stream(self.ref))
+
+
+_VOTE_NODES = ("_ChainVotes.backward", "_CapsuleVotes.backward")
+
+
+def _tail_readers_wait(lpp, posterior, caps_presence, rec_sums, reg):
+    lk = "_CapsuleLikelihood.backward"
+    if _gradient_reader(lpp) != lk or _gradient_reader(posterior) != lk or \
+            lpp.grad_fn is not posterior.grad_fn:
+        return False
+    if _gradient_reader(rec_sums) != "_RenderGmmLogProbSums.backward":
+        return False
+    return all(_gradient_reader(t) in ("",) + _VOTE_NODES
+               for t in (caps_presence, reg))
 
 
 class _PendingWeightGemms:
@@ -2330,6 +2376,15 @@
         vote, scale, vp, dummy_vote, x, post, widx = saved[:7]
         presence = saved[7] if ctx.has_presence else None
         B, O, M = ctx.dims
+        tail = ctx.plan.take("tail_bwd")
+        if tail is not None and (
+                g_log_prob is not None or g_lpp is None or g_post is None
+                or g_lpp.data_ptr() != tail.g_lpp
+                or g_post.data_ptr() != tail.g_post
+                or not (g_lpp.is_contiguous() and g_post.is_contiguous())
+                or tail.ref.device != vote.device):
+            tail.launch_alone()
+            tail = None
         if g_log_prob is not None:
             spread = (g_log_prob / B).expand(B, M)
             g_lpp = spread if g_lpp is None else g_lpp + spread
@@ -2341,6 +2396,13 @@
         gin = [_c(g) for g in (g_lpp, g_w, g_wp, g_s, g_sp, g_post, g_mlp,
                                g_mlogit)]
         pending = ctx.plan.take("k1_bwd")
+        if tail is not None and not (
+                pending is not None and pending.ref.device == vote.device
+                and pending.ptrs[3] is not None
+                and pending.ptrs[3].value == tail.g_rec
+                and not any(g is not None for g in (g_w, g_wp, g_s, g_sp))):
+            tail.launch_alone()
+            tail = None
         if pending is not None and any(
                 g is not None for g in (g_w, g_wp, g_s, g_sp)):
             pending.launch_alone()
@@ -2358,6 +2420,9 @@
                      *gin, gvote, gscale, gvp, gx, gpres, gdummy)):
                 setattr(k, name, None if t is None else t.data_ptr())
             k.B, k.O, k.M = B, O, M
+            if tail is not None:
+                k.tail = ctypes.pointer(tail.desc)
+                k._keep = tail.keep
             _lib.call("scae_render_gmm_sums_bwd_likelihood_f32",
                       ctypes.byref(pending.desc), *pending.ptrs,
                       ctypes.byref(k), _stream(vote))
@@ -2401,7 +2466,7 @@
         O = O1 - 1
         ncls = 0 if cls_w is None else cls_w.shape[0]
         (n_classes_cfg, prior_type, post_type, sparsity_on, weights,
-         within_const, w_reg) = cfg
+         within_const, w_reg, readers_wait) = cfg
         w5 = (ctypes.c_float * 5)(*weights)
         ints = (B, O, M, ncls, int(n_classes_cfg or 0), prior_type, post_type,
                 int(sparsity_on))
@@ -2457,6 +2522,7 @@
         ctx.call = (ints, tuple(weights), wc, float(w_reg))
         ctx.set_materialize_grads(False)
         ctx.deferred = None
+        ctx.parkable = bool(defer and readers_wait and B <= 1024)
         if defer:
             ctx.deferred = _PendingCombine(
                 tail, (lpp, posterior, caps_presence, cls_w, cls_b, label,
@@ -2503,6 +2569,29 @@
             ex.train_log = pend.keep[-1].train_log
         w5 = (ctypes.c_float * 5)(*weights)
         lab = None if label is None else ctypes.c_void_p(label.data_ptr())
+        plan = ctx.plan
+        if ctx.parkable and plan.parking and plan.carry_tail_bwd and \
+                ex.defer_combine and has_rec and \
+                (cls_w is None or (_in_slot(g_w) and _in_slot(g_b))):
+            gout = _c(gout)
+            d = _lib.LossTailRideDesc()
+            for name, t in zip(
+                    ("lpp", "posterior", "caps_presence", "cls_w", "cls_b",
+                     "label", "gout12", "workspace", "g_lpp", "g_posterior",
+                     "g_caps_presence", "g_cls_w", "g_cls_b"),
+                    (lpp, posterior, cp, cls_w, cls_b, label, gout, ws, g_lpp,
+                     g_post, g_cp, g_w, g_b)):
+                setattr(d, name, None if t is None else t.data_ptr())
+            d.extras = ex
+            (d.B, d.O, d.M, d.ncls, d.n_classes_cfg, d.prior_type, d.post_type,
+             d.sparsity_on) = ints
+            d.weights5 = w5
+            d.within_const = wc
+            plan.park("tail_bwd", _PendingTailBackward(
+                d, (lpp, posterior, cp, cls_w, cls_b, label, rec_sums, reg, ws,
+                    gout, g_loss, g_lpp, g_post, g_cp, g_rec, g_reg, ex,
+                    None if pend is None else pend.keep), lpp))
+            return g_lpp, g_post, g_cp, g_w, g_b, None, g_rec, g_reg, None
         _lib.call("scae_loss_tail_bwd_f32", _p(lpp), _p(posterior), _p(cp),
                   _p(cls_w), _p(cls_b), lab, ctypes.byref(ex),
                   _p(_c(gout)), _p(ws), _p(g_lpp), _p(g_post), _p(g_cp),
@@ -2515,9 +2604,12 @@
                      within_const=None, rec_sums=None, reg=None, w_reg=0.):
     if label is None:
         cls_w = cls_b = None
+    plan = _plan()
     cfg = (n_classes, _SPARSITY_TYPES[prior_type], _SPARSITY_TYPES[post_type],
            bool(sparsity_on), [float(w) for w in weights], within_const,
-           float(w_reg))
+           float(w_reg),
+           plan.fused and plan.carry_tail_bwd and rec_sums is not None
+           and _tail_readers_wait(lpp, posterior, caps_presence, rec_sums, reg))
     return _LossTail.apply(lpp, posterior, caps_presence, cls_w, cls_b, label,
                            rec_sums, reg, cfg)
 
@@ -2779,13 +2871,15 @@
             job["defer"] and all(_in_slot(o) for o in job["outs"])
             for job in jobs)
     if g_tile is not None and park:
-        plan.flush_scope("deferring")
+        plan.flush(*[k for k, r in step_plan.RIDES.items()
+                     if r.scope == "deferring" and k != "tail_bwd"])
         addr = lambda t: None if t is None else t.data_ptr()
         plan.park("k1_bwd", _PendingK1Backward(
             d, ctx_tensors, (x, lse_post, lse_prior, g_tile),
             (addr(g_templates), g_alpha_p, addr(g_pose), addr(g_presence),
              addr(g_bg_image), g_scal), templates))
     elif g_tile is not None:
+        _plan().flush("tail_bwd")
         _lib.call("scae_render_gmm_sums_bwd_f32", ctypes.byref(d), _p(x),
                   _p(lse_post), _p(lse_prior), _p(g_tile), _p(g_templates),
                   _p(g_alpha_p), _p(g_pose), _p(g_presence), _p(g_bg_image),
diff --git a/torch_scae_amd/step_plan.py b/torch_scae_amd/step_plan.py
--- a/torch_scae_amd/step_plan.py
+++ b/torch_scae_amd/step_plan.py
@@ -38,6 +38,13 @@
         "the loss tail's batch combine (one workgroup)",
         carriers=("_LossTail.backward",), scope="fusing",
         abi="scae_loss_tail_bwd_f32 (scae_loss_extras.defer_combine)")),
+    ("tail_bwd", Ride(
+        "the loss tail's backward (K6): image rows, classifier gradients, the "
+        "deferred combine",
+        carriers=("_CapsuleLikelihood.backward",
+                  "_RenderGmmLogProbSums.backward"), readers=ANY,
+        abi="scae_render_gmm_sums_bwd_likelihood_f32 "
+            "(scae_likelihood_bwd_desc.tail)")),
     ("k1_bwd", Ride(
         "the reconstruction likelihood's backward (K1)",
         carriers=("_CapsuleLikelihood.backward",), readers=ANY,
@@ -76,6 +83,7 @@
         self.prologue = prologue
         self.bf16 = False
         self.carry_trunk_bwd = True
+        self.carry_tail_bwd = True
         self.noise = {}
         self.noise_salt = 0
         self.side_stream = None
```

New measurement: 274,600, median of 4. 1.2% higher.
